# csiro-crop-informatics/biokanga

Hardware: AMD Instinct MI355X
Metric: aligned reads/s (SAM-identical) on 100 bp SE vs GRCh38, 1->8 MI355X (higher is better)
Workload: dtype u8

## Files before the change

### biokanga_amd/csrc/bk_ctx_int.h

```cpp
#pragma once
#include <atomic>
#include <thread>
#include <hip/hip_runtime.h>

#include <cstdio>
#include <string>
#include <vector>

#include "bk_device.h"
#include "bk_devbuf.h"

#define HIP_TRY(expr)                                                                              \
    do {                                                                                           \
        hipError_t e__ = (expr);                                                                   \
        if (e__ != hipSuccess) {                                                                   \
            fprintf(stderr, "biokanga_amd: %s failed: %s (%s:%d)\n", #expr, hipGetErrorString(e__), __FILE__, __LINE__); \
            return e__ == hipErrorOutOfMemory ? BK_ERR_MEM : BK_ERR_INTERNAL;                      \
        }                                                                                          \
    } while (0)

namespace bk {
struct BatchBufs {
    DevBuf<uint64_t> rd4, rd2, iv_first;
    DevBuf<uint2> iv2, iv32;
    DevBuf<uint32_t> iv_n, rmeta;
    DevBuf<uint32_t> act[2], heavy, wave, wave_work;
    DevBuf<uint32_t> stage[3], stripe_cnt;
    DevBuf<uint32_t> slist, slist_stage;
    DevBuf<uint32_t> sort[3];
    DevBuf<uint8_t> sort_tmp, scan_tmp;
    DevBuf<bk_seg2> seg2;
    DevBuf<uint8_t> in_bases;
    DevBuf<uint64_t> in_offs;
    DevBuf<uint32_t> in_lens;
    DevBuf<bk_hit> in_out;
    DevBuf<uint16_t> in_lens16;
    DevBuf<uint32_t> in_words;
    DevBuf<bk_nbase> in_exc;
    DevBuf<bk_snp_site> snp_sites;
    DevBuf<uint8_t> chrom_accept;
    DevBuf<unsigned long long> htab;
    DevBuf<uint32_t> slot_epoch;
};
struct ImageBufs {
    DevBuf<uint64_t> tgt4, tgt2, tgt2s;
    DevBuf<uint32_t> sa_lo, isa;
    DevBuf<uint8_t> sa_hi, nflag;
    DevBuf<uint64_t> ent_start, ent_end;
    DevBuf<uint32_t> ent_id, id2idx;
    DevBuf<uint8_t> ktab;
    DevBuf<uint64_t> ktab_hi;
    DevBuf<uint32_t> k2, kx[kMoreKeys];
    DevBuf<uint8_t> swin;
    DevBuf<uint32_t> swmap;
    DevBuf<uint32_t> grow_kx[kMoreKeys];
    DevBuf<uint8_t> grow_ktab2;
};
struct FixedBufs {
    DevBuf<uint32_t> small;
    DevBuf<PhaseCtl> ctl;
    DevBuf<unsigned long long> seq_counts, ctr, ctr_aux, snp_tot;
    DevBuf<unsigned long long> seq_global;
    DevBuf<uint32_t> snp_planes;
};
}

struct bk_ctx {
    int device = 0;
    hipStream_t stream = nullptr;
    bk_align_params params{};
    bk::DevAlignCfg cfg{};
    bk::DevIndex ix{};
    bk::ImageBufs image;
    bk::FixedBufs fixed;
    void release_image_buffers() { image = bk::ImageBufs{}; fixed = bk::FixedBufs{}; }
    uint64_t n_tgt4_words = 0;
    uint32_t cap_rd2w = 0;
    int use_tgt2 = 2;
    int sort_lists = 7;
    bool sort_lists_set = false;
    int sort_shift = 0;
    int use_k2 = 1;
    int use_k3 = bk::kMoreKeys;
    bool grow_enabled = false, grow_wait = false;
    uint64_t grow_after = 5 * BK_POLICY_MIN_READS, grow_seen = 0;
    std::atomic<int> grow_state{0};
    std::thread grow_thread;
    bk::DevIndex grow_ix{};
    bool grow_want_ktab2 = false;
    bool grow_elem = false, grow_want_elem = false;
    int use_ktab2 = 1;
    bool ktab_is2 = false;
    int use_iv32 = 1;
    uint32_t wave_waves = 256u * 8u * 4u;
    int use_isa = 1;
    int use_swin = 1;
    uint64_t swin_budget = 0;
    int swin_skip_short = 0;
    int swin_w = 0;
    uint64_t swin_bytes = 0;
    double swin_setup_s = 0;
    double swin_covered = 0;
    bool swin_denied = false;
    bool swin_rebuilt = false;
    int iv_poison = 0;
    int use_wave = 1;
    int lazy_search = 1;
    bool ktab64 = false;
    int ktab_wide = 0;
    int k_req = -1;
    int use_ktab = 1;
    uint32_t el_size = 4;
    uint64_t tot_seq_len = 0;
    std::string dataset;
    std::vector<bk_entry_info> entries;
    std::vector<bk_snp_site> snp_sites;

    bk::BatchBufs buf;
    void release_batch_buffers() { buf = bk::BatchBufs{}; }
    uint32_t cap_reads = 0, cap_wpr = 0, cap_iv_cores = 0;
    uint32_t *h_small = nullptr;
    bk::PhaseCtl *h_ctl = nullptr;
    hipEvent_t ev_ctl = nullptr;
    bool ctl_pending = false, hist_valid = false;
    uint32_t ctl_pending_reads = 0, ctl_pending_maxlen = 0;
    int ctl_pending_phases = 0;
    double hist_slist[bk::kMaxPhases] = {0}, hist_wave[bk::kMaxPhases] = {0};
    int async_error = 0;
    int async_phases = 1;
    bool force_rccl = false;
    uint64_t rccl_allreduces = 0;
    int rccl_ranks = 0;
    bk::HeavyScratch hs{};
    int max_read_len = 500;
    uint32_t last_maxlen = 0;
    int dbg_stop_phase = -1, dbg_phase = 0, dbg_cur = 0;
    uint32_t dbg_n = 0, dbg_ivc = 0;
    bool dbg_valid = false;
    bool debug = false;
    uint32_t chunk_reads = 64u << 20;

    hipEvent_t ev_wait = nullptr;
    bool entries_set = false, tgt2_built = false;
    bool tables_built = false;
    bool tables_under_way = false;
    void *sam_text[2] = {nullptr, nullptr};
    uint64_t sam_text_cap = 0;
    uint32_t n_chrom_accept = 0;
    bk_timing timing{};
    std::vector<hipEvent_t> ev_pool;
    std::vector<uint64_t> loci_offs;
    std::vector<bk_loci> loci;
    std::vector<bk_loci_trims> loci_trims;
    std::vector<bk_seg2> seg2;
};


namespace bk {
struct DevReads {
    const uint8_t *bases = nullptr;
    const uint64_t *offs = nullptr;
    const uint32_t *lens = nullptr;
    const uint32_t *words = nullptr;
    const bk_nbase *exc = nullptr;
    uint64_t n_exc = 0;
};
int engine_align_device(bk_ctx *c, const DevReads &in, uint32_t nreads, bk_hit *d_out, hipStream_t s, uint32_t maxlen_known = 0);
void release_swin(bk_ctx *c);
void drop_swin(bk_ctx *c);
int engine_pair_device(bk_ctx *c, const DevReads &in, uint32_t n_pairs, bk_hit *d_hits, uint32_t maxlen, const bk_pe_params *pe, hipStream_t s,
                       bk_seg2 *seg2_host = nullptr, bk_seg2 *seg2_dev = nullptr);
int engine_prepare_packed(bk_ctx *c, const uint16_t *d_lens16, uint32_t nreads, uint64_t n_words, const bk_nbase *d_exc, uint64_t n_exc,
                          uint32_t *d_lens32, uint64_t *d_offs, uint32_t *maxlen, hipStream_t s);
}

namespace bk {
hipError_t dev_malloc_bytes(void **p, size_t bytes);
hipError_t dev_zero_now(void *p, size_t bytes);
template <class T> inline hipError_t dev_malloc(T **p, size_t bytes) { return dev_malloc_bytes(reinterpret_cast<void **>(p), bytes); }
int upload_host(void *d_dst, const void *h_src, size_t bytes, int device);
int upload_file(void *d_dst, int fd, uint64_t file_ofs, size_t bytes, int device);
bool host_is_pinned(const void *p);
}
```

### biokanga_amd/csrc/bk_device.h

```cpp
#pragma once
#include <hip/hip_runtime.h>
#include <stdint.h>

#include "../../include/biokanga_amd.h"

namespace bk {

constexpr int kMoreKeys = 2;
constexpr int kK2Levels = 7;

__host__ __device__ __forceinline__ uint64_t k2s_pad(uint64_t words) { return (words + 15) & ~15ULL; }
__host__ __device__ __forceinline__ uint64_t k2s_count(uint64_t n, int j) { return (n + (1ULL << (4 * j)) - 1) >> (4 * j); }
__host__ __device__ __forceinline__ uint64_t k2s_start(uint64_t n, int j)
{
    uint64_t o = k2s_pad(n) + 16;
    for (int i = 1; i < j; i++) o += k2s_pad(k2s_count(n, i)) + 16;
    return o;
}


constexpr int kListStripes = 64;
struct StripeSet {
    uint32_t *cnt;
    uint32_t *stage[3];
    uint32_t cap;
};
constexpr int kCtrStripes = 64;
constexpr int kNwLong = 20;
constexpr int kNwLongest = 32;
constexpr int kPackedPadWords = 32;
constexpr int kMaxCoresFast = 16;
constexpr int kWave = 64;
constexpr int kMaxReadLenAbs = 2000;
constexpr uint32_t kNodeCap = 1024000;
constexpr uint64_t kEosWord = 0x7777777777777777ULL;
constexpr int kSwBases = 192, kSwPre = 92, kSwLen = 100;
template <int E> struct SwGeo { static constexpr int bases = 64 * E, pre = E == 3 ? 92 : 32 * E; };
template <int E> __host__ __device__ inline uint64_t sw_word_at(uint64_t idx, int q) { return (idx >> 5) * (32ULL * E) + (uint64_t)q * 32 + (idx & 31); }
constexpr int kSwBlkShift = 5;
constexpr uint32_t kSwNone = 0xFFFFFFFFu;
constexpr uint32_t kSwMinRun = 65, kSwHead = 192;
constexpr int kSwLevels = 8;
constexpr uint32_t kReadHasN = 1u << 15;
constexpr uint32_t kReadLenMask = kReadHasN - 1;

struct DevIndex {
    const uint64_t *tgt4;
    const uint64_t *tgt2;
    const uint64_t *tgt2s;
    const uint8_t *nflag;
    int flag_shift;
    uint32_t nflag_bytes;
    const uint32_t *sa_lo;
    const uint8_t *sa_hi;
    const uint64_t *ent_start;
    const uint64_t *ent_end;
    const uint32_t *ent_id;
    const uint32_t *id2idx;
    uint32_t max_id;
    const uint32_t *ktab32;
    const uint64_t *ktab64;
    const uint64_t *ktab_hi;
    const uint2 *ktab2;
    int ktab2_elem;
    const uint32_t *k2;
    const uint32_t *kx[kMoreKeys];
    const uint32_t *isa;
    const uint4 *swin;
    int sw_words;
    const uint32_t *swmap;
    uint64_t n;
    uint32_t n_ent;
    int k;
};

struct DevAlignCfg {
    int max_subs, mm_delta, align_strand, max_ns, max_hits;
    int min_core_len, slides_per100, max_iter;
    int heavy_thresh;
};

struct DevBatch {
    const uint8_t *bases;
    const uint64_t *offs;
    const uint32_t *lens;
    const uint32_t *pk_words;
    const bk_nbase *pk_exc;
    uint64_t pk_nexc;
    uint32_t pk_read0;
    uint64_t *rd4;
    uint64_t *rd2;
    uint32_t *rmeta;
    uint64_t *iv_first;
    uint32_t *iv_n;
    uint2 *iv2;
    uint32_t iv_stride;
    const uint32_t *act;
    uint32_t *wave_work;
    uint2 *iv32;
    bk_hit *out;
    unsigned long long *seq_counts;
    unsigned long long *ctr;
    uint32_t wpr;
    uint32_t n_reads;
    uint32_t nw;
    uint32_t iv_cores;
};

struct PhaseCtl {
    uint32_t n_act;
    uint32_t cmax;
    uint32_t n_slist;
    uint32_t n_wave;
    uint32_t n_heavy;
    uint32_t wave_cursor, heavy_cursor;
    uint32_t pad[9];
};
constexpr int kMaxPhases = 72;

struct HeavyScratch {
    unsigned long long *htab;
    uint32_t *slot_epoch;
    uint32_t tab_size;
    uint32_t n_slots;
};

struct ReadPlan {
    int len, max_tot_mm, core_len, core_delta, max_slides, n_loop, n_phases;
};

__host__ __device__ inline ReadPlan make_plan(int len, const DevAlignCfg &c)
{
    ReadPlan p;
    p.len = len;
    int m = c.max_subs == 0 ? 0 : (int)(0.5 + (double)(len * c.max_subs) / 100.0);
    if (c.max_subs != 0 && m < 1) m = 1;
    if (m > 63) m = 63;
    p.max_tot_mm = m;
    int cl = len / (c.mm_delta == 1 ? m + 1 : m + 2);
    p.core_len = cl > c.min_core_len ? cl : c.min_core_len;
    int ms = (c.slides_per100 * len + 99) / 100;
    p.max_slides = ms > 1 ? ms : 1;
    int cd = len / p.max_slides - 1;
    p.core_delta = cd > p.core_len ? cd : p.core_len;
    p.n_loop = 0;
    int has_final = 1;
    if (m > 0) {
        int a;
        for (a = 0; a <= m; a++) {
            if (len / (a + c.mm_delta) <= p.core_len) break;
            p.n_loop++;
        }
        has_final = a <= m;
    }
    p.n_phases = p.n_loop + has_final;
    return p;
}

__host__ __device__ inline void phase_params(const ReadPlan &p, const DevAlignCfg &c, int phase, int &mm, int &cl, int &cd)
{
    if (phase < p.n_loop) {
        mm = phase;
        cl = p.len / (phase + c.mm_delta);
        cd = cl;
    } else {
        mm = p.max_tot_mm;
        cl = p.core_len;
        cd = p.core_delta;
    }
}

__host__ __device__ inline int core_offsets(int plen, int cl, int cd, int max_slides, int *ofs, int maxn)
{
    int cur = cd, o = 0, n = 0;
    while (n < max_slides && o <= plen - cl && cur > cl / 3) {
        if (o + cl + cur > plen) cur = plen - (o + cl);
        n++;
        o += cur;
    }
    const int last = plen - cl;
    for (int i = 0; i < maxn; i++) {
        int v = i * cd;
        ofs[i] = v < last ? v : last;
    }
    return n;
}

}
```

### biokanga_amd/csrc/bk_engine.cpp

```cpp
#include "bk_engine_int.h"

namespace bk {
int size_heavy_scratch(bk_ctx *c)
{
    int slides = std::max(1, (c->cfg.slides_per100 * c->max_read_len + 99) / 100);
    uint64_t worst = c->cfg.max_iter ? (uint64_t)slides * (uint64_t)c->cfg.max_iter : kNodeCap;
    if (worst > kNodeCap) worst = kNodeCap;
    uint32_t ts = 1024;
    while (ts < 2 * worst) ts <<= 1;
    uint32_t slots = 4096;
    while ((uint64_t)slots * ts * 8 > (16ULL << 30) && slots > 64) slots >>= 1;
    if (c->hs.htab && c->hs.tab_size == ts && c->hs.n_slots == slots) return BK_OK;
    BatchBufs &m = c->buf;
    m.htab.reset();
    m.slot_epoch.reset();
    c->hs = HeavyScratch{};
    HIP_TRY(m.htab.ensure((size_t)slots * ts));
    HIP_TRY(m.slot_epoch.ensure(slots));
    launch_fill_u64(m.htab.get(), (uint64_t)slots * ts, 0ULL, c->stream);
    HIP_TRY(hipGetLastError());
    HIP_TRY(hipMemsetAsync(m.slot_epoch.get(), 0, (size_t)slots * 4, c->stream));
    HIP_TRY(hipStreamSynchronize(c->stream));
    c->hs = HeavyScratch{m.htab.get(), m.slot_epoch.get(), ts, slots};
    return BK_OK;
}


int ensure_batch_scratch(bk_ctx *c, uint32_t n_reads, uint32_t wpr, uint32_t rd2w, uint32_t iv_cores)
{
    if (n_reads <= c->cap_reads && wpr <= c->cap_wpr && rd2w <= c->cap_rd2w && iv_cores <= c->cap_iv_cores) return BK_OK;
    const size_t nr = std::max(n_reads, c->cap_reads), w = std::max(wpr, c->cap_wpr), w2 = std::max(rd2w, c->cap_rd2w);
    const size_t ivc = std::max(iv_cores, c->cap_iv_cores);
    BatchBufs &m = c->buf;
    m.rd4.reset(); m.iv_first.reset(); m.iv_n.reset(); m.rd2.reset(); m.iv2.reset(); m.rmeta.reset();
    m.act[0].reset(); m.act[1].reset(); m.heavy.reset(); m.wave.reset(); m.iv32.reset(); m.wave_work.reset();
    for (auto &st : m.stage) st.reset();
    c->cap_reads = 0;
    HIP_TRY(m.rd4.ensure(nr * 2 * w));
    if (w2) HIP_TRY(m.rd2.ensure(nr * 2 * w2 + 8));
    HIP_TRY(m.rmeta.ensure((nr + 2) / 2 * 2));
    if (c->image.sa_hi.get() == nullptr && c->ix.n < (1ULL << 32))
        HIP_TRY(m.iv2.ensure(nr * 2 * ivc));
    else {
        HIP_TRY(m.iv_first.ensure(nr * 2 * ivc));
        HIP_TRY(m.iv_n.ensure(nr * 2 * ivc));
    }
    HIP_TRY(m.act[0].ensure(nr));
    HIP_TRY(m.act[1].ensure(nr));
    HIP_TRY(m.heavy.ensure(nr));
    HIP_TRY(m.wave.ensure(nr));
    for (auto &st : m.stage) HIP_TRY(st.ensure(nr + (kListStripes + 2) * 1024));
    if (!m.stripe_cnt.get()) {
        HIP_TRY(m.stripe_cnt.ensure((size_t)2 * kListStripes * 16));
        HIP_TRY(dev_zero_now(m.stripe_cnt.get(), (size_t)2 * kListStripes * 16 * 4));
    }
    if (m.iv2.get()) HIP_TRY(m.iv32.ensure(nr * 2));
    HIP_TRY(m.wave_work.ensure(nr));
    c->cap_reads = (uint32_t)nr;
    c->cap_wpr = (uint32_t)w;
    c->cap_rd2w = (uint32_t)w2;
    c->cap_iv_cores = (uint32_t)ivc;
    return BK_OK;
}

int ensure_slist(bk_ctx *c, uint64_t lanes, hipStream_t s)
{
    BatchBufs &m = c->buf;
    if (m.slist_stage.get() && lanes <= m.slist.cap()) return BK_OK;
    HIP_TRY(hipStreamSynchronize(s));
    m.slist.reset();
    m.slist_stage.reset();
    HIP_TRY(m.slist.ensure(lanes));
    HIP_TRY(m.slist_stage.ensure(lanes + (kListStripes + 2) * 1024));
    return BK_OK;
}

int ensure_in_reads(bk_ctx *c, uint32_t n, bool packed)
{
    BatchBufs &m = c->buf;
    if (n > m.in_out.cap()) {
        m.in_offs.reset(); m.in_lens.reset(); m.in_out.reset(); m.in_lens16.reset();
        HIP_TRY(m.in_offs.ensure(n));
        HIP_TRY(m.in_lens.ensure(n));
        HIP_TRY(m.in_out.ensure(n));
    }
    if (packed) HIP_TRY(m.in_lens16.ensure(m.in_out.cap()));
    return BK_OK;
}

HostExtent host_extent(const uint64_t *offs, const uint32_t *lens, uint32_t nreads)
{
    HostExtent x;
    for (uint32_t i = 0; i < nreads; i++) {
        x.lo = std::min(x.lo, offs[i]);
        x.hi = std::max(x.hi, offs[i] + lens[i]);
        x.maxlen = std::max(x.maxlen, lens[i]);
    }
    x.rel.resize(nreads);
    for (uint32_t i = 0; i < nreads; i++) x.rel[i] = offs[i] - x.lo;
    return x;
}

static int stage_host_batch(bk_ctx *c, const uint8_t *bases, const uint64_t *offs, const uint32_t *lens, uint32_t nreads, HostExtent &x, DevReads &in)
{
    x = host_extent(offs, lens, nreads);
    if (x.maxlen > (uint32_t)kMaxReadLenAbs) return BK_ERR_PARAMS;
    const uint64_t nbytes = x.hi - x.lo;
    BatchBufs &m = c->buf;
    HIP_TRY(m.in_bases.ensure(nbytes + 16));
    int rc = ensure_in_reads(c, nreads, false);
    if (rc) return rc;
    HIP_TRY(hipMemcpyAsync(m.in_bases.get(), bases + x.lo, nbytes, hipMemcpyHostToDevice, c->stream));
    HIP_TRY(hipMemcpyAsync(m.in_offs.get(), x.rel.data(), (size_t)nreads * 8, hipMemcpyHostToDevice, c->stream));
    HIP_TRY(hipMemcpyAsync(m.in_lens.get(), lens, (size_t)nreads * 4, hipMemcpyHostToDevice, c->stream));
    in.bases = m.in_bases.get(); in.offs = m.in_offs.get(); in.lens = m.in_lens.get();
    return BK_OK;
}

static DevBatch make_batch(bk_ctx *c, const DevReads &in, uint32_t first, uint32_t n, uint32_t wpr, uint32_t iv_cores, bk_hit *d_out)
{
    const BatchBufs &m = c->buf;
    DevBatch b{};
    b.bases = in.bases; b.offs = in.offs + first; b.lens = in.lens + first;
    b.pk_words = in.words; b.pk_exc = in.exc; b.pk_nexc = in.words ? in.n_exc : 0; b.pk_read0 = first;
    b.rd4 = m.rd4.get(); b.iv_first = m.iv_first.get(); b.iv_n = m.iv_n.get(); b.iv2 = m.iv2.get();
    b.rmeta = m.rmeta.get();
    b.out = d_out; b.seq_counts = c->fixed.seq_counts.get(); b.ctr = c->fixed.ctr.get();
    b.wpr = wpr; b.n_reads = n; b.iv_cores = iv_cores;
    return b;
}

enum class Span { Search, Extend, Heavy, Other, SearchA, SearchSort, SearchB, Prep };

struct EvTimer {
    bk_ctx *c;
    bool on = true;
    std::vector<std::pair<Span, std::pair<hipEvent_t, hipEvent_t>>> spans;
    size_t next_ev = 0;
    hipEvent_t get()
    {
        if (!on) return nullptr;
        if (next_ev == c->ev_pool.size()) {
            hipEvent_t e;
            (void)hipEventCreate(&e);
            c->ev_pool.push_back(e);
        }
        return c->ev_pool[next_ev++];
    }
    hipEvent_t begin(hipStream_t s)
    {
        hipEvent_t e = get();
        if (e) (void)hipEventRecord(e, s);
        return e;
    }
    void end(Span kind, hipEvent_t b, hipStream_t s)
    {
        hipEvent_t e = get();
        if (!e) return;
        (void)hipEventRecord(e, s);
        spans.push_back({kind, {b, e}});
    }
};

int ensure_sort_scratch(bk_ctx *c, uint32_t n, hipStream_t s)
{
    BatchBufs &m = c->buf;
    if (m.sort_tmp.get() && n <= m.sort[2].cap()) return BK_OK;
    HIP_TRY(hipStreamSynchronize(s));
    for (auto &p : m.sort) p.reset();
    m.sort_tmp.reset();
    const uint64_t cap = (uint64_t)n + n / 4;
    for (auto &p : m.sort) HIP_TRY(p.ensure(cap));
    size_t tb = 0;
    if (sort_list_by_key(nullptr, nullptr, nullptr, nullptr, (uint32_t)cap, nullptr, &tb, s)) return BK_ERR_INTERNAL;
    HIP_TRY(m.sort_tmp.ensure(tb));
    return BK_OK;
}

int sort_work(bk_ctx *c, const uint32_t *list, uint32_t n, hipStream_t s, const uint32_t **out)
{
    const BatchBufs &m = c->buf;
    size_t tb = m.sort_tmp.cap();
    if (sort_list_by_key(m.sort[0].get(), m.sort[1].get(), list, m.sort[2].get(), n, m.sort_tmp.get(), &tb, s)) return BK_ERR_INTERNAL;
    *out = m.sort[2].get();
    return BK_OK;
}

struct LociChunk {
    bk_ctx *c;
    uint32_t n;
    hipStream_t s;
    DevBuf<unsigned long long> cnt, offs;
    DevBuf<uint8_t> tmp;
    DevBuf<bk_loci> loci;
    DevBuf<bk_loci_trims> trims;
    size_t base = 0;
    uint64_t loci_base = 0, total = 0;
    int begin()
    {
        HIP_TRY(cnt.ensure((size_t)n + 1));
        HIP_TRY(offs.ensure((size_t)n + 1));
        HIP_TRY(hipMemsetAsync(cnt.get(), 0, ((size_t)n + 1) * 8, s));
        return BK_OK;
    }
    int scan()
    {
        size_t tb = 0;
        if (scan_counts_u64(nullptr, nullptr, n + 1, nullptr, &tb, s)) return BK_ERR_INTERNAL;
        HIP_TRY(tmp.ensure(tb ? tb : 16));
        if (scan_counts_u64(cnt.get(), offs.get(), n + 1, tmp.get(), &tb, s)) return BK_ERR_INTERNAL;
        base = c->loci_offs.empty() ? 0 : c->loci_offs.size() - 1;
        loci_base = c->loci.size();
        if (c->loci_offs.empty()) c->loci_offs.push_back(0);
        c->loci_offs.resize(base + n + 1);
        HIP_TRY(hipMemcpyAsync(c->loci_offs.data() + base, offs.get(), ((size_t)n + 1) * 8, hipMemcpyDeviceToHost, s));
        HIP_TRY(hipStreamSynchronize(s));
        total = c->loci_offs[base + n];
        HIP_TRY(loci.ensure((size_t)total));
        return BK_OK;
    }
    int finish()
    {
        if (total) {
            c->loci.resize(loci_base + total);
            HIP_TRY(hipMemcpyAsync(c->loci.data() + loci_base, loci.get(), (size_t)total * sizeof(bk_loci), hipMemcpyDeviceToHost, s));
            if (trims.get()) {
                c->loci_trims.resize(loci_base + total);
                HIP_TRY(hipMemcpyAsync(c->loci_trims.data() + loci_base, trims.get(), (size_t)total * sizeof(bk_loci_trims), hipMemcpyDeviceToHost, s));
            }
            HIP_TRY(hipStreamSynchronize(s));
        }
        if (loci_base)
            for (size_t i = 0; i <= n; i++) c->loci_offs[base + i] += loci_base;
        return BK_OK;
    }
};

int collect_loci(bk_ctx *c, const DevBatch &b, uint32_t n, uint32_t maxlen, hipStream_t s)
{
    bk_seg2 *d_seg2 = c->params.min_chimeric_len > 0 ? c->buf.seg2.get() : nullptr;
    LociChunk lc{c, n, s};
    int rc = lc.begin();
    if (rc) return rc;
    launch_loci_count(b.out, n, c->params.clamp_ml ? c->cfg.max_hits : 0, lc.cnt.get(), s);
    rc = lc.scan();
    if (rc) return rc;
    uint32_t n_multi = 0;
    if (lc.total) {
        uint32_t *sm = c->fixed.small.get();
        if (d_seg2) {
            HIP_TRY(lc.trims.ensure((size_t)lc.total));
            HIP_TRY(clear_dev(lc.trims.get(), (size_t)lc.total * sizeof(bk_loci_trims), s));
        }
        HIP_TRY(hipMemsetAsync(sm, 0, 16 * 4, s));
        uint32_t *list = c->buf.act[0].get();
        launch_loci_single(b.out, n, lc.offs.get(), lc.loci.get(), list, sm + 0, d_seg2, lc.trims.get(), s);
        HIP_TRY(hipMemcpyAsync(c->h_small, sm, 16 * 4, hipMemcpyDeviceToHost, s));
        HIP_TRY(hipStreamSynchronize(s));
        n_multi = c->h_small[0];
        if (n_multi) {
            rc = size_heavy_scratch(c);
            if (rc) return rc;
            launch_loci_enum(c->ix, c->cfg, b, c->hs, list, n_multi, sm + 1, lc.offs.get(), lc.loci.get(), sm + 2, d_seg2 ? c->params.min_chimeric_len : 0,
                             maxlen > 512 ? 1 : 0, d_seg2, lc.trims.get(), s);
            HIP_TRY(hipGetLastError());
            HIP_TRY(hipMemcpyAsync(c->h_small, sm, 16 * 4, hipMemcpyDeviceToHost, s));
        }
    }
    rc = lc.finish();
    if (rc) return rc;
    if (n_multi && c->h_small[2] != 0) {
        fprintf(stderr, "bk: loci replay disagreed with LowHitInstances for %u reads\n", c->h_small[2]);
        return BK_ERR_INTERNAL;
    }
    return BK_OK;
}

int best_matches_chunk(bk_ctx *c, const DevBatch &b, uint32_t n, const uint32_t *d_list, uint32_t n_list, hipStream_t s)
{
    const uint32_t width = (uint32_t)c->cfg.max_hits;
    DevBuf<bk_loci> dense;
    LociChunk lc{c, n, s};
    int rc = lc.begin();
    if (rc) return rc;
    HIP_TRY(dense.ensure((size_t)n * width));
    rc = size_heavy_scratch(c);
    if (rc) return rc;
    uint32_t *sm = c->fixed.small.get();
    HIP_TRY(hipMemsetAsync(sm + 4, 0, 4, s));
    launch_best(c->ix, c->cfg, b, c->hs, d_list, n_list, sm + 4, lc.cnt.get(), dense.get(), s);
    HIP_TRY(hipGetLastError());
    rc = lc.scan();
    if (rc) return rc;
    if (lc.total) {
        launch_loci_compact(dense.get(), width, lc.offs.get(), n, lc.loci.get(), s);
        HIP_TRY(hipGetLastError());
    }
    return lc.finish();
}

int align_chunk(bk_ctx *c, const DevReads &in, uint32_t first, uint32_t n, uint32_t maxlen, bk_hit *d_out, hipStream_t s, EvTimer &tm)
{
    uint32_t *sm = c->fixed.small.get(), *hm = c->h_small;
    HIP_TRY(hipMemsetAsync(sm, 0, 16 * 4, s));
    const uint32_t wpr = words_per_read(maxlen);
    const bool reg_path = c->use_wave && maxlen <= 16u * (uint32_t)kNwLongest;
    const int nw16 = maxlen <= 128 ? 8 : (maxlen <= 256 ? 16 : (maxlen <= 16u * (uint32_t)kNwLong ? kNwLong : kNwLongest));
    const bool two_bit = reg_path && c->ix.tgt2 != nullptr;
    const uint32_t ivc = iv_cores_for(c, maxlen);
    int rc = ensure_batch_scratch(c, n, wpr, two_bit ? (uint32_t)(nw16 / 2) : 0u, ivc);
    if (rc && c->image.swin.get()) {
        (void)hipGetLastError();
        bk::release_swin(c);
        rc = ensure_batch_scratch(c, n, wpr, two_bit ? (uint32_t)(nw16 / 2) : 0u, ivc);
    }
    if (rc) return rc;

    BatchBufs &m = c->buf;
    uint32_t *const d_act[2] = {m.act[0].get(), m.act[1].get()}, *const d_heavy = m.heavy.get(), *const d_wave = m.wave.get();
    uint32_t *const d_stage[3] = {m.stage[0].get(), m.stage[1].get(), m.stage[2].get()}, *const d_stripe_cnt = m.stripe_cnt.get();
    DevBatch b = make_batch(c, in, first, n, wpr, ivc, d_out);
    b.rd2 = two_bit ? m.rd2.get() : nullptr;
    b.wave_work = (reg_path && c->cfg.heavy_thresh <= 100) ? m.wave_work.get() : nullptr;
    b.iv32 = (c->use_iv32 && c->ix.k2) ? m.iv32.get() : nullptr;
    b.nw = reg_path ? (uint32_t)nw16 : 0u;
    const int nstr = c->cfg.align_strand == 0 ? 2 : 1;

    PhaseCtl *ctl = c->fixed.ctl.get();
    HIP_TRY(hipMemsetAsync(ctl, 0, sizeof(PhaseCtl) * (kMaxPhases + 2), s));
    auto P = [&](int ph) { return reinterpret_cast<uint32_t *>(ctl + ph); };
    int max_phases = 0, cmax_bound[kMaxPhases + 1] = {0};
    bool cores_fit = true;
    for (uint32_t len = 1; len <= maxlen; len++) {
        const ReadPlan p = make_plan((int)len, c->cfg);
        max_phases = std::max(max_phases, p.n_phases);
        for (int ph = 0; ph < p.n_phases && ph <= kMaxPhases; ph++) {
            int mm, cl, cd, dummy[1];
            phase_params(p, c->cfg, ph, mm, cl, cd);
            const int nc = core_offsets((int)len, cl, cd, p.max_slides, dummy, 0);
            if (nc > kMaxCoresFast) cores_fit = false;
            cmax_bound[ph] = std::max(cmax_bound[ph], std::min(nc, (int)kMaxCoresFast));
        }
    }
    if (max_phases > kMaxPhases) return BK_ERR_INTERNAL;
    const bool no_readback = reg_path && c->cfg.heavy_thresh <= 100 && c->ix.k2 != nullptr && cores_fit && !c->params.best_matches &&
                             !c->debug && c->async_phases;
    const bool check_maxlen = !tm.on;
    if (check_maxlen) launch_max_len(b.lens, n, P(kMaxPhases + 1) + 0, s);
    hipEvent_t e0 = tm.begin(s);
    launch_prep(c->cfg, b, d_act[0], P(0) + 0, P(0) + 1, d_stage[0], d_stripe_cnt, s);
    HIP_TRY(hipGetLastError());
    tm.end(Span::Prep, e0, s);
    uint32_t n_act = n;
    int cmax = cmax_bound[0];
    auto read_ctl = [&](int ph) -> int {
        HIP_TRY(hipMemcpyAsync(hm, ctl + ph, 2 * sizeof(PhaseCtl), hipMemcpyDeviceToHost, s));
        HIP_TRY(hipStreamSynchronize(s));
        return BK_OK;
    };
    if (!no_readback) {
        int rr = read_ctl(0);
        if (rr) return rr;
        n_act = hm[0];
        cmax = (int)hm[1];
    }
    int cur = 0;
    if (c->params.best_matches) {
        hipEvent_t eb = tm.begin(s);
        int rb = best_matches_chunk(c, b, n, d_act[0], n_act, s);
        if (rb) return rb;
        tm.end(Span::Heavy, eb, s);
        n_act = 0;
    }
    b.iv_stride = n;
    if (no_readback && c->ix.isa == nullptr) { int rh = size_heavy_scratch(c); if (rh) return rh; }
    for (int phase = 0; no_readback ? phase < max_phases : n_act > 0; phase++) {
        const uint32_t *ext_list = d_act[cur];
        b.act = ext_list;
        if (no_readback) cmax = cmax_bound[phase];
        const uint32_t n_bound = n_act;
        uint32_t *ctl_p = P(phase), *ctl_n = P(phase + 1);
        const int lazy = (reg_path && c->lazy_search) ? 1 : 0;
        if (cmax > 0) {
            hipEvent_t e1 = tm.begin(s);
            if (c->ix.k2) {
                const uint64_t lanes = (uint64_t)n_bound * (uint64_t)(cmax * nstr);
                { int rs = ensure_slist(c, lanes, s); if (rs) return rs; }
                uint32_t *const d_slist = m.slist.get();
                if (c->iv_poison) launch_clear_iv(b, ctl_p + 0, n_bound, cmax, c->cfg.align_strand == 2 ? 1 : 0, c->cfg.align_strand == 1 ? 0 : 1, 0xFFFFFFFFu, s);
                hipEvent_t ea = tm.begin(s);
                launch_search_a(c->ix, c->cfg, b, d_act[cur], ctl_p + 0, n_bound, phase, cmax, nstr, lazy, d_slist, ctl_p + 2,
                                m.slist_stage.get(), d_stripe_cnt, s);
                HIP_TRY(hipGetLastError());
                tm.end(Span::SearchA, ea, s);
                uint64_t n_slist_bound = lanes;
                uint32_t n_sort = 0;
                if (!no_readback) {
                    HIP_TRY(hipMemcpyAsync(hm + 2, ctl_p + 2, 4, hipMemcpyDeviceToHost, s));
                    HIP_TRY(hipStreamSynchronize(s));
                    n_slist_bound = hm[2];
                    n_sort = hm[2];
                } else {
                    const double f = c->hist_valid ? c->hist_slist[phase] * 1.05 : 0.30;
                    n_sort = (uint32_t)std::min<uint64_t>({(uint64_t)(f * n) + 4096, lanes, (uint64_t)0x7FFFFFF0});
                }
                if (no_readback && m.sort[2].cap() >= 4096) n_sort = (uint32_t)std::min<uint64_t>(n_sort, m.sort[2].cap());
                const uint32_t *sorted = nullptr;
                if ((c->sort_lists & 1) && n_sort >= 4096) {
                    int rs = ensure_sort_scratch(c, n_sort, s);
                    if (rs) return rs;
                    hipEvent_t es = tm.begin(s);
                    launch_keys_search(b, d_slist, ctl_p + 2, n_sort, c->sort_shift, m.sort[0].get(), s);
                    rs = sort_work(c, d_slist, n_sort, s, &sorted);
                    if (rs) return rs;
                    tm.end(Span::SearchSort, es, s);
                } else
                    n_sort = 0;
                if (n_slist_bound) {
                    hipEvent_t eb = tm.begin(s);
                    launch_search_b(c->ix, c->cfg, b, phase, lazy, d_slist, sorted, n_sort, ctl_p + 2, n_slist_bound, s);
                    tm.end(Span::SearchB, eb, s);
                }
            } else
                launch_search(c->ix, c->cfg, b, d_act[cur], n_act, phase, cmax, nstr, lazy, s);
            HIP_TRY(hipGetLastError());
            tm.end(Span::Search, e1, s);
        }
        if (phase == c->dbg_stop_phase) {
            c->dbg_n = n; c->dbg_ivc = ivc; c->dbg_cur = cur; c->dbg_phase = phase; c->dbg_valid = true;
            break;
        }
        hipEvent_t e2 = tm.begin(s);
        DevAlignCfg cfg_lane = c->cfg;
        if (c->ix.n > (1ULL << 32)) cfg_lane.heavy_thresh = 0;
        if (n_bound == 0) {}
        else if (reg_path && c->cfg.heavy_thresh <= 100)
            launch_flat(c->ix, c->cfg, b, ext_list, ctl_p + 0, n_bound, phase, nstr * std::max(cmax, 1), d_act[cur ^ 1], ctl_n + 0, d_heavy, ctl_p + 4,
                        d_wave, ctl_p + 3, ctl_n + 1, d_stage, d_stripe_cnt, nw16, s);
        else
            launch_extend(c->ix, cfg_lane, b, ext_list, n_act, phase, d_act[cur ^ 1], ctl_n + 0, d_heavy, ctl_p + 4, ctl_n + 1, s);
        HIP_TRY(hipGetLastError());
        tm.end(Span::Extend, e2, s);
        uint32_t n_heavy = 0, n_wave = n_bound;
        if (!no_readback) {
            int rr = read_ctl(phase);
            if (rr) return rr;
            n_heavy = hm[4];
            n_wave = hm[3];
        }
        if (n_wave) {
            hipEvent_t e3 = tm.begin(s);
            const uint32_t *wsorted = nullptr;
            uint32_t n_sort = n_wave;
            if (no_readback) {
                const double f = c->hist_valid ? c->hist_wave[phase] * 1.05 : 0.25;
                n_sort = (uint32_t)std::min<uint64_t>((uint64_t)(f * n) + 4096, n_wave);
                if (m.sort[2].cap() >= 4096) n_sort = (uint32_t)std::min<uint64_t>(n_sort, m.sort[2].cap());
            }
            if ((c->sort_lists & 2) && n_sort >= 4096) {
                int rs = ensure_sort_scratch(c, n_sort, s);
                if (rs) return rs;
                launch_keys_wave(c->cfg, b, phase, d_wave, ctl_p + 3, n_sort, (c->sort_lists & 4) ? -1 : c->sort_shift, m.sort[0].get(), b.wave_work, s);
                rs = sort_work(c, d_wave, n_sort, s, &wsorted);
                if (rs) return rs;
            } else
                n_sort = 0;
            if (!no_readback && c->ix.isa == nullptr) { int rh = size_heavy_scratch(c); if (rh) return rh; }
            launch_wave(c->ix, c->cfg, b, c->hs, d_wave, wsorted, n_sort, ctl_p + 3, n_wave, phase, ctl_p + 5, d_act[cur ^ 1], ctl_n + 0, ctl_n + 1,
                        nw16, c->wave_waves, s);
            HIP_TRY(hipGetLastError());
            tm.end(Span::Heavy, e3, s);
        }
        if (n_heavy) {
            hipEvent_t e3 = tm.begin(s);
            { int rh = size_heavy_scratch(c); if (rh) return rh; }
            launch_heavy(c->ix, c->cfg, b, c->hs, d_heavy, n_heavy, phase, ctl_p + 6, d_act[cur ^ 1], ctl_n + 0, ctl_n + 1, s);
            HIP_TRY(hipGetLastError());
            tm.end(Span::Heavy, e3, s);
        }
        if (!no_readback) {
            if (n_wave || n_heavy) { int rr = read_ctl(phase); if (rr) return rr; }
            if (c->debug)
                fprintf(stderr, "bk: phase %d n_act %u cmax %d n_heavy %u n_wave %u -> next n_act %u cmax %u\n", phase, n_act, cmax, n_heavy, n_wave, hm[16], hm[17]);
            n_act = hm[16];
            cmax = (int)hm[17];
        }
        cur ^= 1;
        if (phase > 70) return BK_ERR_INTERNAL;
    }
    if (c->dbg_stop_phase >= 0 && !c->dbg_valid) {
        c->dbg_n = n; c->dbg_ivc = ivc; c->dbg_cur = cur; c->dbg_phase = kMaxPhases; c->dbg_valid = true;
    }
    if (no_readback) {
        HIP_TRY(hipMemcpyAsync(c->h_ctl, ctl, sizeof(PhaseCtl) * (kMaxPhases + 2), hipMemcpyDeviceToHost, s));
        HIP_TRY(hipEventRecord(c->ev_ctl, s));
        c->ctl_pending = true;
        c->ctl_pending_reads = n;
        c->ctl_pending_phases = max_phases;
        c->ctl_pending_maxlen = check_maxlen ? maxlen : 0;
    }
    if (c->params.micro_indel_len > 0 || c->params.splice_junct_len > 0 || c->params.min_chimeric_len > 0) {
        hipEvent_t ei = tm.begin(s);
        { int r2 = ensure_seg2(c, n); if (r2) return r2; }
        bk_seg2 *d_seg2 = m.seg2.get();
        hipError_t eh = clear_dev(d_seg2, (size_t)n * sizeof(bk_seg2), s);
        int rc2 = BK_OK;
        if (eh == hipSuccess && (c->params.micro_indel_len > 0 || c->params.splice_junct_len > 0)) {
            eh = hipMemsetAsync(sm, 0, 16 * 4, s);
            if (eh == hipSuccess) {
                launch_indel(c->ix, c->cfg, b, n, c->params.micro_indel_len, c->params.splice_junct_len, c->params.min_chimeric_len > 0 ? 1 : 0, d_act[0], sm + 0,
                             hm + 0, sm + 1, d_seg2, s);
                eh = hipGetLastError();
            }
        }
        if (eh == hipSuccess && c->params.min_chimeric_len > 0) {
            rc2 = size_heavy_scratch(c);
            if (rc2 == BK_OK) {
                eh = hipMemsetAsync(sm, 0, 16 * 4, s);
                if (eh == hipSuccess) {
                    launch_unaligned_list(b.out, n, d_act[0], sm + 0, s);
                    eh = hipMemcpyAsync(hm, sm, 4, hipMemcpyDeviceToHost, s);
                }
                if (eh == hipSuccess) eh = hipStreamSynchronize(s);
                if (eh == hipSuccess && hm[0]) {
                    launch_chimeric(c->ix, c->cfg, b, c->hs, d_act[0], hm[0], c->params.min_chimeric_len, maxlen > 512 ? 1 : 0, sm + 1, d_seg2, s);
                    eh = hipGetLastError();
                }
            }
        }
        const size_t at = c->seg2.size();
        c->seg2.resize(at + n);
        if (eh == hipSuccess && rc2 == BK_OK) eh = hipMemcpyAsync(c->seg2.data() + at, d_seg2, (size_t)n * sizeof(bk_seg2), hipMemcpyDeviceToHost, s);
        if (eh == hipSuccess) eh = hipStreamSynchronize(s);
        if (rc2 != BK_OK) return rc2;
        if (eh != hipSuccess) return BK_ERR_INTERNAL;
        if (c->params.min_chimeric_len > 0 && c->cfg.max_hits > 1)
            for (size_t i = at; i < at + n; i++)
                if (c->seg2[i].flags == 0x40) c->seg2[i] = bk_seg2{};
        tm.end(Span::Heavy, ei, s);
    }
    hipEvent_t e4 = tm.begin(s);
    launch_count_seqs(d_out, n, c->image.id2idx.get(), c->ix.n_ent, c->fixed.seq_counts.get(), s);
    HIP_TRY(hipGetLastError());
    tm.end(Span::Other, e4, s);
    if (c->cfg.max_hits > 1 && !c->params.best_matches) {
        int rl = collect_loci(c, b, n, maxlen, s);
        if (rl) return rl;
    }
    return BK_OK;
}


int take_phase_history(bk_ctx *c, bool wait)
{
    if (!c->ctl_pending) return BK_OK;
    if (wait) HIP_TRY(bk::wait_event(c->ev_ctl));
    else if (hipEventQuery(c->ev_ctl) != hipSuccess) { (void)hipGetLastError(); return BK_OK; }
    c->ctl_pending = false;
    const PhaseCtl *h = c->h_ctl;
    const double n = (double)std::max<uint32_t>(c->ctl_pending_reads, 1);
    for (int ph = 0; ph < kMaxPhases; ph++) {
        c->hist_slist[ph] = ph < c->ctl_pending_phases ? (double)h[ph].n_slist / n : 0.0;
        c->hist_wave[ph] = ph < c->ctl_pending_phases ? (double)h[ph].n_wave / n : 0.0;
        if (h[ph].n_heavy) {
            fprintf(stderr, "biokanga_amd: %u reads of phase %d were left for the general kernel by a schedule that does not run it\n", h[ph].n_heavy, ph);
            c->async_error = BK_ERR_INTERNAL;
        }
    }
    if (c->ctl_pending_maxlen && h[kMaxPhases + 1].n_act > c->ctl_pending_maxlen) {
        fprintf(stderr, "biokanga_amd: a batch held a read of %u bases, its caller had promised at most %u\n", h[kMaxPhases + 1].n_act, c->ctl_pending_maxlen);
        c->async_error = BK_ERR_PARAMS;
    }
    c->hist_valid = true;
    if (c->async_error && wait) { const int e = c->async_error; c->async_error = 0; return e; }
    return BK_OK;
}

int align_device(bk_ctx *c, const DevReads &in, uint32_t nreads, bk_hit *d_out, hipStream_t s, uint32_t maxlen_known, bool enqueue_only)
{
    grow_tick(c, nreads);
    const uint32_t *d_lens = in.lens;
    if (enqueue_only) {
        const uint32_t ml = maxlen_known;
        const bool plain = c->cfg.max_hits == 1 && !c->params.best_matches && !c->params.micro_indel_len && !c->params.splice_junct_len && !c->params.min_chimeric_len;
        const bool fits = ml >= 1 && ml <= 16u * (uint32_t)kNwLongest && nreads <= c->cap_reads && nreads <= c->chunk_reads && words_per_read(ml) <= c->cap_wpr &&
                          iv_cores_for(c, ml) <= c->cap_iv_cores && rd2w_for(ml) <= c->cap_rd2w &&
                          (uint64_t)nreads * iv_cores_for(c, ml) * (c->cfg.align_strand == 0 ? 2u : 1u) <= c->buf.slist.cap() && (c->ix.isa != nullptr || c->hs.htab != nullptr);
        const bool main_path = c->use_wave && c->cfg.heavy_thresh <= 100 && c->ix.k2 != nullptr && c->ix.tgt2 != nullptr && !c->debug && c->async_phases;
        if (!plain || !fits || !main_path) return BK_ERR_PARAMS;
    }
    EvTimer tm{c};
    tm.on = !enqueue_only;
    hipEvent_t t0 = tm.begin(s);
    c->loci_offs.clear();
    c->loci.clear();
    c->loci_trims.clear();
    c->seg2.clear();
    uint32_t maxlen = maxlen_known;
    if (!maxlen) {
        HIP_TRY(hipMemsetAsync(c->fixed.small.get(), 0, 16 * 4, s));
        launch_max_len(d_lens, nreads, c->fixed.small.get() + 5, s);
        HIP_TRY(hipMemcpyAsync(c->h_small, c->fixed.small.get(), 16 * 4, hipMemcpyDeviceToHost, s));
        HIP_TRY(hipStreamSynchronize(s));
        maxlen = c->h_small[5];
    }
    if (maxlen > (uint32_t)kMaxReadLenAbs) return BK_ERR_PARAMS;
    c->last_maxlen = maxlen;
    (void)take_phase_history(c, false);
    if ((int)maxlen > c->max_read_len) {
        c->max_read_len = (int)maxlen;
    }
    if (!enqueue_only) { int rw = maybe_build_swin(c, maxlen, nreads, s); if (rw) return rw; }
    uint32_t chunk = c->chunk_reads;
    if (!(std::min(chunk, nreads) <= c->cap_reads && words_per_read(maxlen) <= c->cap_wpr && iv_cores_for(c, maxlen) <= c->cap_iv_cores &&
          rd2w_for(maxlen) <= std::max(c->cap_rd2w, 1u) && !c->params.best_matches)) {
        const uint64_t per_read = scratch_bytes_per_read(words_per_read(maxlen), rd2w_for(maxlen), iv_cores_for(c, maxlen));
        size_t free_b = 0, total_b = 0;
        HIP_TRY(hipMemGetInfo(&free_b, &total_b));
        const uint64_t have = (uint64_t)c->cap_reads * scratch_bytes_per_read(c->cap_wpr, c->cap_rd2w, c->cap_iv_cores);
        uint64_t fit = ((uint64_t)free_b + have) / 4 * 3 / per_read;
        if (fit < 65536) fit = 65536;
        if (fit < chunk) chunk = (uint32_t)fit;
        if (chunk > (1u << 27)) chunk = 1u << 27;
        if (c->params.best_matches) {
            const uint64_t lim = std::max<uint64_t>(1024, (4ULL << 30) / (sizeof(bk_loci) * (uint64_t)c->cfg.max_hits));
            if (lim < chunk) chunk = (uint32_t)lim;
        }
    }
    for (uint32_t done = 0; done < nreads;) {
        uint32_t n = std::min(chunk, nreads - done);
        int rc = align_chunk(c, in, done, n, maxlen, d_out + done, s, tm);
        if (rc) return rc;
        done += n;
    }
    if (enqueue_only) return BK_OK;
    hipEvent_t t1 = tm.begin(s);
    HIP_TRY(bk::wait_stream(s, c->ev_wait));
    { int rh = take_phase_history(c, true); if (rh) return rh; }
    float ms = 0;
    (void)hipEventElapsedTime(&ms, t0, t1);
    c->timing.ms_total += ms;
    for (auto &sp : tm.spans) {
        float m = 0;
        (void)hipEventElapsedTime(&m, sp.second.first, sp.second.second);
        switch (sp.first) {
        case Span::Search: c->timing.ms_search += m; c->timing.n_search_launches++; break;
        case Span::Extend: c->timing.ms_extend += m; c->timing.n_extend_launches++; break;
        case Span::Heavy: c->timing.ms_heavy += m; c->timing.n_heavy_launches++; break;
        case Span::SearchA: c->timing.ms_search_a += m; break;
        case Span::SearchSort: c->timing.ms_search_sort += m; break;
        case Span::SearchB: c->timing.ms_search_b += m; c->timing.n_search_b_launches++; break;
        case Span::Prep: c->timing.ms_prep += m; c->timing.ms_other += m; break;
        case Span::Other: c->timing.ms_other += m; break;
        }
    }
    return BK_OK;
}


}

using namespace bk;

int bk::engine_align_device(bk_ctx *c, const DevReads &in, uint32_t nreads, bk_hit *d_out, hipStream_t s, uint32_t maxlen_known)
{
    return align_device(c, in, nreads, d_out, s, maxlen_known);
}

namespace {
struct CastU64 {
    __host__ __device__ unsigned long long operator()(const uint32_t &v) const { return (unsigned long long)v; }
};
}

int bk::engine_prepare_packed(bk_ctx *c, const uint16_t *d_lens16, uint32_t nreads, uint64_t n_words, const bk_nbase *d_exc, uint64_t n_exc,
                              uint32_t *d_lens32, uint64_t *d_offs, uint32_t *maxlen, hipStream_t s)
{
    launch_widen_lens(d_lens16, nreads, d_lens32, (unsigned long long *)d_offs, s);
    HIP_TRY(hipGetLastError());
    size_t need = 0;
    HIP_TRY(bk::prim::exclusive_sum(nullptr, need, (unsigned long long *)d_offs, (unsigned long long *)d_offs, (size_t)nreads, s));
    if (need > c->buf.scan_tmp.cap()) {
        HIP_TRY(hipStreamSynchronize(s));
        HIP_TRY(c->buf.scan_tmp.ensure(need + 256));
    }
    size_t tb = c->buf.scan_tmp.cap();
    HIP_TRY(bk::prim::exclusive_sum(c->buf.scan_tmp.get(), tb, (unsigned long long *)d_offs, (unsigned long long *)d_offs, (size_t)nreads, s));
    HIP_TRY(hipMemsetAsync(c->fixed.ctr_aux.get(), 0, 32, s));
    launch_packed_extent(d_offs, d_lens32, nreads, c->fixed.ctr_aux.get(), s);
    launch_check_exc(d_exc, n_exc, d_lens32, nreads, reinterpret_cast<uint32_t *>(c->fixed.ctr_aux.get() + 2), s);
    HIP_TRY(hipGetLastError());
    unsigned long long h[3] = {0, 0, 0};
    HIP_TRY(hipMemcpyAsync(h, c->fixed.ctr_aux.get(), 24, hipMemcpyDeviceToHost, s));
    HIP_TRY(hipStreamSynchronize(s));
    if (h[0] != n_words || h[1] > (unsigned long long)kMaxReadLenAbs || (uint32_t)h[2] != 0) return BK_ERR_PARAMS;
    *maxlen = (uint32_t)h[1];
    return BK_OK;
}

int bk::engine_pair_device(bk_ctx *c, const DevReads &in, uint32_t n_pairs, bk_hit *d_hits, uint32_t maxlen, const bk_pe_params *pe, hipStream_t s,
                           bk_seg2 *seg2_host, bk_seg2 *seg2_dev)
{
    const uint32_t nreads = 2 * n_pairs;
    const uint32_t wpr = words_per_read(maxlen);
    const uint32_t ivc = c->cap_iv_cores ? c->cap_iv_cores : iv_cores_for(c, maxlen);
    int rc = ensure_batch_scratch(c, nreads, wpr, 0, ivc);
    if (rc && c->image.swin.get()) {
        (void)hipGetLastError();
        bk::release_swin(c);
        rc = ensure_batch_scratch(c, nreads, wpr, 0, ivc);
    }
    if (rc) return rc;
    const DevBatch b = make_batch(c, in, 0, nreads, wpr, c->cap_iv_cores, d_hits);
    if (c->params.min_chimeric_len > 0 && !seg2_host && !seg2_dev) return BK_ERR_PARAMS;
    bk_seg2 *d_seg2 = seg2_dev;
    if (!d_seg2 && seg2_host) {
        rc = ensure_seg2(c, nreads);
        if (rc) return rc;
        d_seg2 = c->buf.seg2.get();
        HIP_TRY(hipMemcpyAsync(d_seg2, seg2_host, (size_t)nreads * sizeof(bk_seg2), hipMemcpyHostToDevice, s));
    }
    HIP_TRY(hipMemsetAsync(c->fixed.small.get(), 0, 16 * 4, s));
    launch_pe(c->ix, c->cfg, b, pe->pe_mode, pe->pair_min_len, pe->pair_max_len, pe->pair_strand ? 1 : 0, d_hits, n_pairs,
              c->buf.heavy.get(), c->fixed.small.get(), c->h_small, d_seg2, c->params.min_chimeric_len, maxlen > 512 ? 1 : 0, c->buf.chrom_accept.get(), c->n_chrom_accept, s);
    HIP_TRY(hipGetLastError());
    if (seg2_host && !seg2_dev) HIP_TRY(hipMemcpyAsync(seg2_host, d_seg2, (size_t)nreads * sizeof(bk_seg2), hipMemcpyDeviceToHost, s));
    HIP_TRY(hipStreamSynchronize(s));
    return BK_OK;
}


extern "C" {


int bk_batch_seg2(bk_ctx *c, const bk_seg2 **seg2, uint64_t *n)
{
    if (!c || !seg2 || !n) return BK_ERR_PARAMS;
    *seg2 = c->seg2.empty() ? nullptr : c->seg2.data();
    *n = c->seg2.size();
    return BK_OK;
// ... 355 lines not shown
```

### biokanga_amd/csrc/bk_engine_int.h

```cpp
#pragma once
#include <hip/hip_runtime.h>
#include <fcntl.h>
#include <unistd.h>
#include "bk_prim.h"

#include <algorithm>
#include <cstdio>
#include <cstdlib>
#include <ctime>
#include <cstring>
#include <map>
#include <mutex>
#include <string>
#include <atomic>
#include <thread>
#include <type_traits>
#include <vector>

#include <dlfcn.h>
#include <rccl/rccl.h>

#include "bk_ctx_int.h"
#include "bk_cpus.h"
#include "bk_wait.h"
#include "bk_env.h"
#include "sfx_file.h"


namespace bk {
void launch_pack_target(const uint8_t *seq, uint64_t n, uint64_t *tgt4, uint64_t nwords, hipStream_t s);
void launch_pack_target2(const uint64_t *tgt4, uint64_t nwords4, uint64_t *tgt2, unsigned int *nflag32, int flag_shift, hipStream_t s);
void launch_split_sa5(const uint8_t *sa5, uint64_t n, uint32_t *lo, uint8_t *hi, hipStream_t s);
void launch_build_ktab(const DevIndex &ix, void *tab, int k, bool tab64, hipStream_t s, uint64_t i0 = 0, uint64_t i1 = 0, unsigned long long *starts = nullptr, bool pairs = false);
void launch_fill_ktab2_y(void *tab2, const uint32_t *k2, uint64_t n_entries, hipStream_t s, const uint32_t *sa_elem = nullptr);
void launch_max_len(const uint32_t *lens, uint32_t n, uint32_t *out, hipStream_t s);
void launch_widen_lens(const uint16_t *lens16, uint32_t n, uint32_t *lens32, unsigned long long *nwords, hipStream_t s);
void launch_check_exc(const bk_nbase *exc, uint64_t n_exc, const uint32_t *lens, uint32_t n_reads, uint32_t *bad, hipStream_t s);
void launch_packed_extent(const uint64_t *offs, const uint32_t *lens, uint32_t n, unsigned long long *out, hipStream_t s);
void launch_snp_pileup(const DevIndex &ix, const uint8_t *bases, const uint64_t *offs, const uint32_t *id2idx, const bk_snp_aln *alns, uint64_t n_alns,
                       uint32_t *planes, hipStream_t s);
void launch_snp_gather(const DevIndex &ix, const uint32_t *planes, uint64_t g0, uint32_t n, uint32_t *out, hipStream_t s);
void launch_snp_centroids(const DevIndex &ix, const uint32_t *planes, uint64_t g0, uint32_t chrom_len, uint32_t min_reads, uint32_t *hist, hipStream_t s);
void launch_snp_sites(const DevIndex &ix, const uint32_t *planes, uint64_t g0, uint32_t chrom_len, uint32_t min_reads, double min_prop,
                      bk_snp_site *sites, uint32_t cap, uint32_t *n_sites, unsigned long long *totals, hipStream_t s);
void launch_count_seqs(const bk_hit *out, uint32_t n, const uint32_t *id2idx, uint32_t n_ent, unsigned long long *counts, hipStream_t s);
void launch_fill_u64(unsigned long long *p, uint64_t n, unsigned long long v, hipStream_t s);
void launch_prep(const DevAlignCfg &cfg, const DevBatch &b, uint32_t *act, uint32_t *act_cnt, uint32_t *cmax, uint32_t *stage,
                 uint32_t *stripe_cnt, hipStream_t s);
void launch_search(const DevIndex &ix, const DevAlignCfg &cfg, const DevBatch &b, const uint32_t *act, uint32_t n_act,
                   int phase, int cmax, int nstr, int lazy, hipStream_t s);
void launch_extend(const DevIndex &ix, const DevAlignCfg &cfg, const DevBatch &b, const uint32_t *act, uint32_t n_act,
                   int phase, uint32_t *next_act, uint32_t *next_cnt, uint32_t *heavy, uint32_t *heavy_cnt,
                   uint32_t *cmax_next, hipStream_t s);
void launch_build_isa(const uint32_t *sa, uint64_t n, uint32_t *isa, hipStream_t s, uint64_t i0 = 0, uint64_t i1 = 0);
void launch_build_swin(const DevIndex &ix, void *swin, int words, hipStream_t s);
void launch_swin_breaks(const DevIndex &ix, const int *w, int n_levels, unsigned long long *const *brk, uint64_t a, uint64_t e, uint64_t n_words,
                        const unsigned long long *starts, hipStream_t s);
void launch_swin_cover(const unsigned long long *brk, uint64_t n, uint32_t max_run, uint32_t min_run, uint32_t *flags, uint64_t n_blocks, int first_level, hipStream_t s);
void launch_pack_ktab64(const uint64_t *tab, uint64_t n_entries, uint32_t *off, uint64_t *hi, uint32_t *overflow, hipStream_t s);
void launch_count_nonzero(const uint32_t *flags, uint64_t n, unsigned long long *count, hipStream_t s);
void launch_swin_map(const uint32_t *flags, const uint32_t *incl, uint64_t n_blocks, uint32_t cap_blocks, uint32_t *used, uint32_t *map, hipStream_t s);
void launch_swin_fill(const DevIndex &ix, const uint32_t *map, void *swin, int words, uint64_t a, uint64_t e, hipStream_t s);
void launch_build_k2(const DevIndex &ix, uint32_t *k2, uint32_t *k3, uint32_t *k4, unsigned long long *bad, hipStream_t s, uint64_t i0 = 0, uint64_t i1 = 0, bool write_k2 = true);
void launch_build_k2_levels(uint32_t *k2, uint64_t n, hipStream_t s);
void launch_make_ktab2(const uint32_t *tab, const uint32_t *k2, uint64_t n_entries, uint64_t n, void *out, hipStream_t s, const uint32_t *sa_elem = nullptr);
void launch_search_a(const DevIndex &ix, const DevAlignCfg &cfg, const DevBatch &b, const uint32_t *act, const uint32_t *p_n_act, uint32_t n_act_bound,
                     int phase, int cmax, int nstr, int lazy, uint32_t *list, uint32_t *list_cnt, uint32_t *stage, uint32_t *stripe_cnt,
                     hipStream_t s);
void launch_search_b(const DevIndex &ix, const DevAlignCfg &cfg, const DevBatch &b, int phase, int lazy, const uint32_t *list, const uint32_t *sorted,
                     uint32_t n_sorted, const uint32_t *p_n_list, uint64_t n_bound, hipStream_t s);
void launch_clear_iv(const DevBatch &b, const uint32_t *p_n_act, uint32_t n_act_bound, int cmax, int st0, int st1, uint32_t word, hipStream_t s);
void launch_pe(const DevIndex &ix, const DevAlignCfg &cfg, const DevBatch &b, int pe_mode, int min_len, int max_len, int pair_strand,
               bk_hit *hits, uint32_t n_pairs, uint32_t *orphans, uint32_t *counters, uint32_t *h_count, bk_seg2 *seg2, int min_chim,
               int long_reads, const uint8_t *accept, uint32_t n_accept, hipStream_t s);
void launch_flat(const DevIndex &ix, const DevAlignCfg &cfg, const DevBatch &b, const uint32_t *act, const uint32_t *p_n_act, uint32_t n_act_bound, int phase,
                 int slots_max, uint32_t *next_act, uint32_t *next_cnt, uint32_t *heavy, uint32_t *heavy_cnt, uint32_t *wave,
                 uint32_t *wave_cnt, uint32_t *cmax_next, uint32_t *const *stage, uint32_t *stripe_cnt, int nw, hipStream_t s);
void launch_wave(const DevIndex &ix, const DevAlignCfg &cfg, const DevBatch &b, const HeavyScratch &hs, const uint32_t *list, const uint32_t *sorted,
                 uint32_t n_sorted, const uint32_t *p_n_list, uint32_t n_bound, int phase, uint32_t *cursor, uint32_t *next_act, uint32_t *next_cnt,
                 uint32_t *cmax_next, int nw, uint32_t max_waves, hipStream_t s);
void launch_heavy(const DevIndex &ix, const DevAlignCfg &cfg, const DevBatch &b, const HeavyScratch &hs, const uint32_t *list,
                  uint32_t n_list, int phase, uint32_t *cursor, uint32_t *next_act, uint32_t *next_cnt, uint32_t *cmax_next,
                  hipStream_t s);
int build_sa_device(const uint8_t *d_seq, uint64_t n, void *d_sa_out, int el_size, hipStream_t s);
int scan_counts_u64(const unsigned long long *in, unsigned long long *out, uint32_t n, void *tmp, size_t *tmp_bytes, hipStream_t s);
void launch_loci_count(const bk_hit *out, uint32_t n, int clamp_to, unsigned long long *cnt, hipStream_t s);
void launch_best(const DevIndex &ix, const DevAlignCfg &cfg, const DevBatch &b, const HeavyScratch &hs, const uint32_t *list,
                 uint32_t n_list, uint32_t *cursor, unsigned long long *cnt, bk_loci *dense, hipStream_t s);
void launch_indel(const DevIndex &ix, const DevAlignCfg &cfg, const DevBatch &b, uint32_t n, int max_indel, int max_junct, int keep_state, uint32_t *list,
                  uint32_t *list_cnt_dev, uint32_t *list_cnt_host, uint32_t *cursor, bk_seg2 *seg2, hipStream_t s);
void launch_unaligned_list(const bk_hit *out, uint32_t n, uint32_t *list, uint32_t *cnt, hipStream_t s);
void launch_chimeric(const DevIndex &ix, const DevAlignCfg &cfg, const DevBatch &b, const HeavyScratch &hs, const uint32_t *list, uint32_t n_list,
                     int min_pct, int long_reads, uint32_t *cursor, bk_seg2 *seg2, hipStream_t s);
void launch_loci_compact(const bk_loci *dense, uint32_t width, const unsigned long long *offs, uint32_t n, bk_loci *out, hipStream_t s);
void launch_loci_single(const bk_hit *out, uint32_t n, const unsigned long long *offs, bk_loci *loci, uint32_t *list, uint32_t *list_cnt,
                        const bk_seg2 *seg2, bk_loci_trims *trims, hipStream_t s);
void launch_loci_enum(const DevIndex &ix, const DevAlignCfg &cfg, const DevBatch &b, const HeavyScratch &hs, const uint32_t *list,
                      uint32_t n_list, uint32_t *cursor, const unsigned long long *offs, bk_loci *loci, uint32_t *err, int min_pct, int long_reads,
                      bk_seg2 *seg2, bk_loci_trims *trims, hipStream_t s);
int sort_list_by_key(const uint32_t *keys_in, uint32_t *keys_out, const uint32_t *vals_in, uint32_t *vals_out, uint32_t n,
                     void *tmp, size_t *tmp_bytes, hipStream_t s);
void launch_keys_search(const DevBatch &b, const uint32_t *list, const uint32_t *p_n, uint32_t n_sort, int shift, uint32_t *keys, hipStream_t s);
void launch_keys_wave(const DevAlignCfg &cfg, const DevBatch &b, int phase, const uint32_t *list, const uint32_t *p_n, uint32_t n_sort, int shift, uint32_t *keys,
                      const uint32_t *work_of, hipStream_t s);

struct StageClock {
    bool on = env::timing();
    double t0 = now();
    static double now() { timespec ts; clock_gettime(CLOCK_MONOTONIC, &ts); return (double)ts.tv_sec + 1e-9 * (double)ts.tv_nsec; }
    static double wall() { timespec ts; clock_gettime(CLOCK_REALTIME, &ts); return (double)(ts.tv_sec % 60) + 1e-9 * (double)ts.tv_nsec; }
    void lap(const char *what) { if (!on) return; const double t = now(); fprintf(stderr, "bk timing: %-28s %7.1f ms   (done at :%06.3f)\n", what, 1e3 * (t - t0), wall()); t0 = t; }
};


inline uint32_t words_per_read(uint32_t maxlen)
{
    return ((maxlen + 15) / 16 + 2) & ~1u;
}

inline uint32_t iv_cores_for(const bk_ctx *c, uint32_t maxlen)
{
    const uint32_t ms = std::max(1u, ((uint32_t)c->cfg.slides_per100 * maxlen + 99) / 100);
    return std::min<uint32_t>(ms, kMaxCoresFast);
}

inline uint32_t rd2w_for(uint32_t maxlen)
{
    return maxlen <= 128 ? 4u : (maxlen <= 256 ? 8u : (maxlen <= 16u * (uint32_t)kNwLong ? (uint32_t)kNwLong / 2 : (uint32_t)kNwLongest / 2));
}

inline uint64_t scratch_bytes_per_read(uint32_t wpr, uint32_t rd2w = 8, uint32_t iv_cores = kMaxCoresFast)
{
    return 2ULL * wpr * 8 + 2ULL * rd2w * 8 + 2ULL * iv_cores * (12 + 8) + 52 + 24;
}


int derive_cfg(bk_ctx *c);
hipError_t clear_dev(void *p, size_t bytes, hipStream_t s);
struct TablePlan {
    bool ktab = false, k2 = false, isa = false;
    bool ktab2 = false;
    int kx = 0;
    int k = 0;
    DevBuf<unsigned long long> d_bad;
};

int tables_begin(bk_ctx *c, TablePlan &tp);
int tables_range(bk_ctx *c, const TablePlan &tp, uint64_t i0, uint64_t i1, unsigned long long *bucket_starts = nullptr);
int tables_end(bk_ctx *c, TablePlan &tp);
int build_tables(bk_ctx *c);
int build_tgt2(bk_ctx *c);
void publish_index(bk_ctx *c);
void grow_take_in(bk_ctx *c);
void grow_drop(bk_ctx *c);
void grow_tick(bk_ctx *c, uint64_t nreads, bool now = false);
int setup_entries(bk_ctx *c, const bk_entry_info *entries, uint32_t n_entries);
int finish_ctx(bk_ctx *c, const bk_entry_info *entries, uint32_t n_entries);
int new_ctx(bk_ctx **out, int device_id, const bk_align_params *p, bk_ctx **pc);
int adopt_device_image(bk_ctx *c, const uint8_t *d_seq, uint64_t n, const uint8_t *d_sa, int el);
int maybe_build_swin(bk_ctx *c, uint32_t maxlen, uint32_t nreads, hipStream_t s);
int size_heavy_scratch(bk_ctx *c);
int ensure_batch_scratch(bk_ctx *c, uint32_t n_reads, uint32_t wpr, uint32_t rd2w = 0, uint32_t iv_cores = kMaxCoresFast);
int ensure_sort_scratch(bk_ctx *c, uint32_t n, hipStream_t s);
int ensure_slist(bk_ctx *c, uint64_t lanes, hipStream_t s);
inline int ensure_seg2(bk_ctx *c, uint32_t n) { HIP_TRY(c->buf.seg2.ensure(n)); return BK_OK; }
struct HostExtent {
    uint64_t lo = ~0ULL, hi = 0;
    uint32_t maxlen = 0;
    std::vector<uint64_t> rel;
};
HostExtent host_extent(const uint64_t *offs, const uint32_t *lens, uint32_t nreads);
int align_device(bk_ctx *c, const DevReads &in, uint32_t nreads, bk_hit *d_out, hipStream_t s, uint32_t maxlen_known = 0, bool enqueue_only = false);
}
```

### biokanga_amd/csrc/bk_extend.hip

```cpp
#include "bk_dev_window.h"
#include "bk_dev_prof.h"

namespace bk {


template <bool WIDE>
__global__ void __launch_bounds__(256) k_extend(DevIndex ix, DevAlignCfg cfg, DevBatch b, const uint32_t *__restrict__ act,
                                                uint32_t n_act, int phase, uint32_t *__restrict__ next_act,
                                                uint32_t *__restrict__ next_cnt, uint32_t *__restrict__ heavy,
                                                uint32_t *__restrict__ heavy_cnt, uint32_t *__restrict__ cmax_next)
{
    __shared__ LdsEntries s_le;
    lds_entries_load(s_le, ix);
    uint32_t a = blockIdx.x * blockDim.x + threadIdx.x;
    unsigned long long n_search = 0, n_cand = 0, n_lcm = 0;
    if (a < n_act) {
        uint32_t r = act[a];
        int len = (int)b.lens[r];
        ReadPlan p = make_plan(len, cfg);
        int mm, cl, cd, ofs[kMaxCoresFast];
        phase_params(p, cfg, phase, mm, cl, cd);
        int nc = core_offsets(len, cl, cd, p.max_slides, ofs, kMaxCoresFast);
        int s0 = cfg.align_strand == 2 ? 1 : 0, s1 = cfg.align_strand == 1 ? 0 : 1;
        bool is_heavy = nc > kMaxCoresFast;
        if (!is_heavy)
            for (int st = s0; st <= s1; st++)
                for (int c = 0; c < nc; c++)
                    if (iv_count(b, iv_slot(b, a, st, c)) > (uint32_t)cfg.heavy_thresh) is_heavy = true;
        if (is_heavy) {
            heavy[atomicAdd(heavy_cnt, 1u)] = r;
        } else {
            n_lcm = 1;
            const int init = mm + cfg.mm_delta + 1;
            int low_inst = 0, low_mm = init, nxt = init;
            uint64_t hit_left = 0;
            int hit_ent = -1, hit_strand = '?';
            bool done = false;
            for (int st = s0; st <= s1 && !done; st++) {
                const uint64_t *rdw = b.rd4 + ((uint64_t)r * 2 + st) * b.wpr;
                for (int c = 0; c < nc && !done; c++) {
                    n_search++;
                    uint64_t slot = iv_slot(b, a, st, c);
                    uint32_t n;
                    uint64_t first;
                    iv_get(b, slot, first, n);
                    for (uint32_t j = 0; j < n; j++) {
                        uint64_t loci = sa_get<WIDE>(ix, first + j);
                        if (loci < (uint64_t)ofs[c]) continue;
                        uint64_t t = loci - (uint64_t)ofs[c];
                        int e = find_entry_lds(s_le, ix, t);
                        if (e < 0 || t + (uint64_t)len - 1 > ix.ent_end[e]) continue;
                        bool dup = false;
                        for (int c2 = 0; c2 < c && !dup; c2++) {
                            uint64_t q0 = nib16(rdw, ofs[c2]) & top_mask(cl);
                            dup = cmp_core(rdw, ofs[c2], cl, q0, ix.tgt4, t + (uint64_t)ofs[c2]) == 0;
                        }
                        if (dup) continue;
                        n_cand++;
                        int lim = mm < nxt - 1 ? mm : nxt - 1;
                        int cm = hamming(rdw, len, ix.tgt4, t, lim);
                        if (cm > lim) continue;
                        if (cm < low_mm) {
                            low_inst = 1; nxt = low_mm; low_mm = cm;
                            hit_left = t; hit_ent = e; hit_strand = st ? '-' : '+';
                        } else if (cm == low_mm)
                            low_inst++;
                        else
                            nxt = cm;
                        if (low_inst > cfg.max_hits && low_mm == 0) { done = true; break; }
                    }
                }
            }
            int rslt = classify(low_inst, low_mm, nxt, init, cfg.mm_delta, cfg.max_hits);
            if (rslt != BK_HR_NONE)
                write_result(ix, cfg, b, r, len, rslt, low_inst, low_mm, nxt, hit_left, hit_ent, hit_strand, phase << 1);
            else if (phase + 1 < p.n_phases) {
                int mm2, cl2, cd2, dummy[1];
                phase_params(p, cfg, phase + 1, mm2, cl2, cd2);
                int nc2 = core_offsets(len, cl2, cd2, p.max_slides, dummy, 0);
                if (nc2 <= kMaxCoresFast) atomicMax(cmax_next, (uint32_t)nc2);
                next_act[atomicAdd(next_cnt, 1u)] = r;
            }
        }
    }
    for (int off = 32; off > 0; off >>= 1) {
        n_search += __shfl_down(n_search, off);
        n_cand += __shfl_down(n_cand, off);
        n_lcm += __shfl_down(n_lcm, off);
    }
    if ((threadIdx.x & 63) == 0) {
        if (n_search) atomicAdd(&b.ctr[ctr_stripe() + 0], n_search);
        if (n_cand) atomicAdd(&b.ctr[ctr_stripe() + 1], n_cand);
        if (n_lcm) atomicAdd(&b.ctr[ctr_stripe() + 2], n_lcm);
    }
}


constexpr uint32_t kLdsEntries = 128;
constexpr uint32_t kFlatCap = 8192;
constexpr uint8_t kRecSkip = 255;

template <bool WIDE> struct FlatEntT { typedef uint64_t type; };
template <> struct FlatEntT<false> { typedef uint32_t type; };
__host__ __device__ constexpr bool flat_caches_first(bool wide, int bs, int slots_max)
{
    return !wide && slots_max <= 16 && bs * slots_max * 6 <= 24576;
}

__host__ __device__ constexpr bool flat_rows_in_lds(bool wide, int nw, int bs) { return false; }
__host__ __device__ constexpr bool flat_small_pass(bool wide, int nw, int bs) { return !wide && nw <= 8 && bs <= 256; }

template <bool WIDE, int NW, int BS>
__global__ void __launch_bounds__(BS) k_flat(DevIndex ix, DevAlignCfg cfg, DevBatch b, const uint32_t *__restrict__ act,
                                              const uint32_t *__restrict__ p_n_act, int phase, int slots_max, StripeSet out, int have_wave)
{
    const uint32_t n_act = *p_n_act;
    if ((uint64_t)blockIdx.x * BS >= n_act) return;
    constexpr bool ROWS = flat_rows_in_lds(WIDE, NW, BS);
#ifdef BK_FLAT_KB
    constexpr int KB = BK_FLAT_KB;
#else
    constexpr int KB = 1;
#endif
    constexpr int NBLK = NW / 4 + 1;
    constexpr bool SMALL = flat_small_pass(WIDE, NW, BS);
    constexpr uint32_t CAP = (SMALL ? kFlatCap / 4 : kFlatCap) * BS / 256;
    constexpr int SPEC = 8;
    extern __shared__ uint32_t s_dyn[];
    const bool cf = flat_caches_first(WIDE, BS, slots_max);
    uint32_t *s_first = s_dyn;
    uint16_t *s_sp = reinterpret_cast<uint16_t *>(s_dyn + (cf ? BS * slots_max : 0));
    __shared__ uint32_t s_lazy[BS];
    __shared__ uint32_t s_off[BS + 1];
    __shared__ uint32_t s_r[BS];
    __shared__ uint32_t s_geo[BS];
    __shared__ uint8_t s_hasn[BS];
    __shared__ uint32_t s_k1[BS], s_c2[BS], s_nx[BS];
    __shared__ uint8_t s_mm[BS];
    __shared__ alignas(16) uint8_t s_rec[CAP];
    __shared__ uint4 s_row[ROWS ? BS * 2 * (NW / 4) : 1];
    __shared__ alignas(16) uint32_t s_key[WIDE ? CAP : 1];
    __shared__ uint32_t s_t[SMALL ? CAP : 1];
    __shared__ uint32_t s_wsum[BS / 64];
    __shared__ uint32_t s_cnt[4], s_base[4], s_cmax;
    __shared__ unsigned long long s_ctr[3];
    using EntT = typename FlatEntT<WIDE>::type;
    __shared__ EntT s_es[kLdsEntries], s_ee[kLdsEntries];
    const uint32_t t = threadIdx.x;
#if defined(BK_PROF) && BK_PROF == 1
    PROF_BEGIN;
#endif
    const int lane = t & 63, wid = t >> 6;
    if (t < 4) s_cnt[t] = 0;
    if (t == 4) s_cmax = 0;
    if (t >= 8 && t < 11) s_ctr[t - 8] = 0;
    const bool ent_lds = ix.n_ent <= kLdsEntries;
    uint64_t es_v = 0, ee_v = 0;
    if (ent_lds && t < ix.n_ent) { es_v = ix.ent_start[t]; ee_v = ix.ent_end[t]; }

    const uint32_t a = blockIdx.x * blockDim.x + t;
    const int s0 = cfg.align_strand == 2 ? 1 : 0, s1 = cfg.align_strand == 1 ? 0 : 1;
    const int cmaxs = slots_max / (s1 - s0 + 1);
    const bool two_bit = b.rd2 != nullptr;
    uint32_t n_search = 0, n_cand = 0, n_lcm = 0;
    int dest = 0;
    uint32_t r = 0, my_cmax = 0, my_total = 0;
    int len = 0, mm = 0, cl = 1, cd = 1, nc = 0, n_phases = 0;
    bool mine = false;
    if (a < n_act) {
        r = act[a];
        const uint32_t len_v = b.rmeta[r];
        const bool spec = !WIDE && slots_max <= SPEC;
        uint2 sv[SPEC];
        if (!WIDE) {
#pragma unroll
            for (int u = 0; u < SPEC; u++) {
                sv[u] = make_uint2(0, 0);
                if (spec && u < slots_max) {
                    const int sti = u >= cmaxs ? 1 : 0;
                    sv[u] = b.iv2[iv_slot(b, a, s0 + sti, u - sti * cmaxs)];
                }
            }
        }
        uint4 rb00 = make_uint4(0, 0, 0, 0), rb01 = rb00, rb10 = rb00, rb11 = rb00;
        if (ROWS && two_bit) {
            const uint4 *__restrict__ rp = reinterpret_cast<const uint4 *>(b.rd2 + (uint64_t)r * 2 * (NW / 2));
            rb00 = rp[0]; rb01 = rp[1]; rb10 = rp[2]; rb11 = rp[3];
        }
        len = (int)(len_v & kReadLenMask);
        ReadPlan p = make_plan(len, cfg);
        n_phases = p.n_phases;
        int dummy[1];
        phase_params(p, cfg, phase, mm, cl, cd);
        nc = core_offsets(len, cl, cd, p.max_slides, dummy, 0);
        const bool fits = nc <= kMaxCoresFast && len <= 16 * NW && nc <= cmaxs;
        bool is_heavy = !fits;
        if (fits) {
            uint32_t run = 0, lazy_bits = 0, work = 0;
            if (!WIDE && spec) {
#pragma unroll
                for (int u = 0; u < SPEC; u++)
                    if (u < slots_max) {
                        const int c = u >= cmaxs ? u - cmaxs : u;
                        const uint32_t raw = c < nc ? sv[u].y : 0u;
                        if (raw & kLazyFlag) lazy_bits |= 1u << u;
                        if (raw & kElemFlag) lazy_bits |= 0x10000u << u;
                        const uint32_t cnt = raw & ~kIvFlags;
                        if (cnt > (uint32_t)cfg.heavy_thresh) is_heavy = true;
                        run += is_heavy ? 0 : cnt;
                        work = work + cnt < work ? 0xFFFFFFFFu : work + cnt;
                        if (cf) s_first[t * slots_max + u] = sv[u].x;
                        s_sp[t * slots_max + u] = (uint16_t)run;
                    }
            } else
                for (int q = 0; q < slots_max; q++) {
                    const int sti = q >= cmaxs ? 1 : 0, c = q - sti * cmaxs;
                    uint64_t f64 = 0;
                    uint32_t cnt = 0;
                    if (c < nc) iv_get(b, iv_slot(b, a, s0 + sti, c), f64, cnt);
                    if (cnt & kLazyFlag) lazy_bits |= 1u << (q & 31);
                    if ((cnt & kElemFlag) && cf) lazy_bits |= 0x10000u << q;
                    cnt &= ~kIvFlags;
                    if (cnt > (uint32_t)cfg.heavy_thresh) is_heavy = true;
                    run += is_heavy ? 0 : cnt;
                    work = work + cnt < work ? 0xFFFFFFFFu : work + cnt;
                    if (cf) s_first[t * slots_max + q] = (uint32_t)f64;
                    s_sp[t * slots_max + q] = (uint16_t)run;
                }
            s_lazy[t] = lazy_bits;
            if (run > CAP) is_heavy = true;
            my_total = is_heavy ? 0 : run;
            if (is_heavy && have_wave && b.wave_work != nullptr) b.wave_work[a] = work;
        }
        if (is_heavy) dest = (fits && have_wave) ? 2 : 3;
        else { mine = true; n_lcm = 1; }
        if (ROWS && two_bit) { s_row[t * 4 + 0] = rb00; s_row[t * 4 + 1] = rb01; s_row[t * 4 + 2] = rb10; s_row[t * 4 + 3] = rb11; }
        s_hasn[t] = (len_v & kReadHasN) ? 1 : 0;
    }
    PROF(0);
    if (ent_lds && t < ix.n_ent) { s_es[t] = (EntT)es_v; s_ee[t] = (EntT)ee_v; }
    s_k1[t] = 0xFFFFFFFFu; s_c2[t] = 0; s_nx[t] = 0xFFFFFFFFu;
    s_mm[t] = (uint8_t)(mm < 255 ? mm : 255);
    s_r[t] = r; s_geo[t] = (uint32_t)len | ((uint32_t)cl << 10) | ((uint32_t)cd << 20);
    {
        uint32_t v = my_total;
        for (int off = 1; off < 64; off <<= 1) { uint32_t u = __shfl_up(v, off); if (lane >= off) v += u; }
        if (lane == 63) s_wsum[wid] = v;
        __syncthreads();
        uint32_t add = 0;
        for (int w = 0; w < wid; w++) add += s_wsum[w];
        s_off[t] = add + v - my_total;
        if (t == BS - 1) s_off[BS] = add + v;
    }
    __syncthreads();
    PROF(1);

    const int init = mm + cfg.mm_delta + 1;
    int low_inst = 0, low_mm = init, nxt = init;
    int best_q = -1;
    uint32_t best_j = 0, best_x = 0, my_hit_t = 0;
    constexpr uint32_t kNone = 0xFFFFFFFFu, kOffStart = 1u << 18, kLazyBit = 1u << 16;

    for (uint32_t start = 0; start < BS;) {
        const uint32_t base = s_off[start];
        uint32_t lo = start + 1, hi = BS;
        while (lo < hi) {
            uint32_t mid = (lo + hi + 1) >> 1;
            if (s_off[mid] - base <= CAP) lo = mid; else hi = mid - 1;
        }
        const uint32_t end = lo;
        const uint32_t total = s_off[end] - base;
        for (uint32_t f0 = 0; f0 < total; f0 += KB * BS) {
            uint64_t tv[KB];
            uint32_t meta[KB];
#pragma unroll
            for (int i = 0; i < KB; i++) {
                const uint32_t f = f0 + (uint32_t)i * BS + t;
                meta[i] = kNone;
                tv[i] = 0;
                if (f < total) {
                    const uint32_t g = base + f;
                    uint32_t l2 = start, h2 = end - 1;
                    while (l2 < h2) {
                        uint32_t mid = (l2 + h2 + 1) >> 1;
                        if (s_off[mid] <= g) l2 = mid; else h2 = mid - 1;
                    }
                    const uint32_t ri = l2;
                    const uint32_t local = g - s_off[ri];
                    const uint16_t *sp = s_sp + ri * slots_max;
                    int q = 0;
                    while (sp[q] <= local) q++;
                    const uint32_t j = local - (q ? sp[q - 1] : 0);
                    uint64_t iv_f;
                    bool lazy, elem;
                    if (cf) { iv_f = s_first[ri * slots_max + q]; lazy = ((s_lazy[ri] >> q) & 1) != 0; elem = ((s_lazy[ri] >> (16 + q)) & 1) != 0; }
                    else {
                        const int sti = q >= cmaxs ? 1 : 0;
                        uint32_t iv_c;
                        iv_get(b, iv_slot(b, blockIdx.x * blockDim.x + ri, s0 + sti, q - sti * cmaxs), iv_f, iv_c);
                        lazy = (iv_c & kLazyFlag) != 0;
                        elem = (iv_c & kElemFlag) != 0;
                    }
                    tv[i] = elem ? iv_f : sa_get<WIDE>(ix, iv_f + j);
                    meta[i] = ri | ((uint32_t)q << 10) | (lazy ? kLazyBit : 0u);
                }
            }
            uint4 wv[KB][NBLK];
            uint4 rowv[KB][NW / 4];
            uint8_t fb0[KB], fb1[KB];
#pragma unroll
            for (int i = 0; i < KB; i++) {
                fb0[i] = 0; fb1[i] = 0;
#pragma unroll
                for (int u = 0; u < NBLK; u++) wv[i][u] = make_uint4(0, 0, 0, 0);
                if (meta[i] != kNone) {
                    const uint32_t ri = meta[i] & 1023u;
                    const int q = (int)((meta[i] >> 10) & 63u);
                    const int c = q >= cmaxs ? q - cmaxs : q;
                    const uint32_t geo = s_geo[ri];
                    const int c_len = (int)(geo & 1023u), c_cl = (int)((geo >> 10) & 1023u), c_cd = (int)(geo >> 20);
                    const int last = c_len - c_cl;
                    const int ofs = c * c_cd < last ? c * c_cd : last;
                    if (tv[i] >= (uint64_t)ofs) {
                        const uint64_t t0 = tv[i] - (uint64_t)ofs;
                        tv[i] = t0;
                        if (two_bit) {
                            const uint64_t g0 = t0 >> ix.flag_shift, g1 = (t0 + (uint64_t)c_len - 1) >> ix.flag_shift;
                            fb0[i] = ix.nflag[g0 >> 3];
                            fb1[i] = ix.nflag[g1 >> 3];
                            window2_load<NW>(ix.tgt2, ix.tgt2s, t0, c_len, wv[i]);
                            if (!ROWS && NW <= 8) {
                                const int sti = q >= cmaxs ? 1 : 0;
                                const uint4 *__restrict__ rp = reinterpret_cast<const uint4 *>(b.rd2 + ((uint64_t)s_r[ri] * 2 + (uint64_t)(s0 + sti)) * (NW / 2));
#pragma unroll
                                for (int u = 0; u < NW / 4; u++) rowv[i][u] = rp[u];
                            }
                        }
                    } else
                        meta[i] |= kOffStart;
                }
            }
#pragma unroll
            for (int i = 0; i < KB; i++) {
                if (meta[i] == kNone) continue;
                const uint32_t f = f0 + (uint32_t)i * BS + t;
                uint8_t rec = kRecSkip;
                if (!(meta[i] & kOffStart)) {
// ... 17 lines not shown
                        if (ROWS) {
#pragma unroll
                            for (int u = 0; u < NW / 4; u++) {
                                const uint4 v = s_row[(ri * 2 + st) * (NW / 4) + u];
                                r2w[2 * u] = ((uint64_t)v.y << 32) | v.x;
                                r2w[2 * u + 1] = ((uint64_t)v.w << 32) | v.z;
                            }
                        } else if (NW <= 8) {
#pragma unroll
                            for (int u = 0; u < NW / 4; u++) {
                                r2w[2 * u] = ((uint64_t)rowv[i][u].y << 32) | rowv[i][u].x;
                                r2w[2 * u + 1] = ((uint64_t)rowv[i][u].w << 32) | rowv[i][u].z;
                            }
                        } else
                            load_read_words2<NW>(b.rd2 + ((uint64_t)cr * 2 + st) * (NW / 2), r2w);
#pragma unroll
                        for (int u = 0; u < NW / 4; u++) rnm[u] = 0;
                        window2_compare<NW>(r2w, rnm, c_len, t0, wv[i], w);
                    }
                    if (flg) eval_window_rare<NW>(read_row(b, cr, st, s_hasn[ri] != 0), c_len, ix.tgt4, t0, w);
                    bool skip = w.eos || (lazy && !core_clean<NW>(w, ofs, c_cl));
#pragma unroll 1
                    for (int c2 = 0; c2 < c; c2++) skip |= core_clean<NW>(w, c2 * c_cd, c_cl);
                    if (!skip) rec = (uint8_t)(w.mm < 127 ? w.mm : 127);
                    if (WIDE) s_key[f] = (uint32_t)t0;
                    if (SMALL) s_t[f] = (uint32_t)t0;
                    if (!WIDE && rec != kRecSkip) {
                        atomicAdd(&s_c2[ri], 1u << 16);
                        if (rec <= s_mm[ri]) atomicMin(&s_k1[ri], ((uint32_t)rec << 16) | (base + f - s_off[ri]));
                    }
                }
                s_rec[f] = rec;
            }
        }
        PROF(2);
        __syncthreads();
        PROF(3);
        auto replay_sequential = [&]() __attribute__((always_inline)) {
            const uint16_t *sp = s_sp + t * slots_max;
            const uint32_t rb = s_off[t] - base;
            bool done = false;
            uint32_t prev = 0;
            for (int q = 0; q < slots_max && !done; q++) {
                if ((q >= cmaxs ? q - cmaxs : q) >= nc) continue;
                n_search++;
                const uint32_t upto = sp[q];
                for (uint32_t x = prev; x < upto; x++) {
                    const int cm = s_rec[rb + x];
                    if (cm == kRecSkip) continue;
                    n_cand++;
                    if (cm > mm || cm >= nxt) continue;
                    if (cm < low_mm) {
                        low_inst = 1; nxt = low_mm; low_mm = cm;
                        best_q = q; best_j = x - prev; best_x = x;
                    } else if (cm == low_mm)
                        low_inst++;
                    else
                        nxt = cm;
                    if (low_inst > cfg.max_hits && low_mm == 0) { done = true; break; }
                }
                prev = upto;
            }
        };
        if (WIDE) {
            for (uint32_t f = t; f < total; f += BS) {
                if (s_rec[f] == kRecSkip) continue;
                const uint32_t g = base + f;
                uint32_t l2 = start, h2 = end - 1;
                while (l2 < h2) {
                    uint32_t mid = (l2 + h2 + 1) >> 1;
                    if (s_off[mid] <= g) l2 = mid; else h2 = mid - 1;
                }
                const uint32_t rb = s_off[l2] - base, local = f - rb;
                const uint32_t second = (s1 > s0) ? (uint32_t)s_sp[l2 * slots_max + cmaxs - 1] : 0xFFFFFFFFu;
                const uint32_t from = local >= second ? second : 0u;
                const uint32_t kx = s_key[f];
                bool seen = false;
                uint32_t i = rb + from;
                const uint32_t i1 = rb + local;
                for (; i < i1 && (i & 3) != 0; i++) seen |= s_rec[i] != kRecSkip && s_key[i] == kx;
                for (; i + 4 <= i1 && !seen; i += 4) {
                    const uint4 k4 = *reinterpret_cast<const uint4 *>(&s_key[i]);
                    const uint32_t r4 = *reinterpret_cast<const uint32_t *>(&s_rec[i]);
                    seen = (k4.x == kx && (r4 & 0xffu) != kRecSkip) || (k4.y == kx && ((r4 >> 8) & 0xffu) != kRecSkip) ||
                           (k4.z == kx && ((r4 >> 16) & 0xffu) != kRecSkip) || (k4.w == kx && (r4 >> 24) != kRecSkip);
                }
                for (; i < i1 && !seen; i++) seen = s_rec[i] != kRecSkip && s_key[i] == kx;
                if (seen) s_rec[f] = kRecSkip;
            }
            __syncthreads();
            for (uint32_t f = t; f < total; f += BS) {
                const uint8_t rec = s_rec[f];
                if (rec == kRecSkip) continue;
                const uint32_t g = base + f;
                uint32_t l2 = start, h2 = end - 1;
                while (l2 < h2) {
                    uint32_t mid = (l2 + h2 + 1) >> 1;
                    if (s_off[mid] <= g) l2 = mid; else h2 = mid - 1;
                }
                atomicAdd(&s_c2[l2], 1u << 16);
                if (rec <= s_mm[l2]) atomicMin(&s_k1[l2], ((uint32_t)rec << 16) | (g - s_off[l2]));
            }
            __syncthreads();
        }
        {
            for (uint32_t f = t; f < total; f += BS) {
                const int cm = s_rec[f];
                if (cm == kRecSkip) continue;
                const uint32_t g = base + f;
                uint32_t l2 = start, h2 = end - 1;
                while (l2 < h2) {
                    uint32_t mid = (l2 + h2 + 1) >> 1;
                    if (s_off[mid] <= g) l2 = mid; else h2 = mid - 1;
                }
                if (cm > (int)s_mm[l2]) continue;
                if ((uint32_t)cm == (s_k1[l2] >> 16)) atomicAdd(&s_c2[l2], 1u);
                else atomicMin(&s_nx[l2], (uint32_t)cm);
            }
            __syncthreads();
            if (mine && t >= start && t < end) {
                const uint32_t k1 = s_k1[t], c2 = s_c2[t];
                if (k1 != 0xFFFFFFFFu && (k1 >> 16) == 0 && (int)(c2 & 0xFFFFu) > cfg.max_hits)
                    replay_sequential();
                else {
                    n_search += (uint32_t)((s1 - s0 + 1) * nc);
                    n_cand += c2 >> 16;
                    if (k1 != 0xFFFFFFFFu) {
                        low_mm = (int)(k1 >> 16);
                        low_inst = (int)(c2 & 0xFFFFu);
                        const uint32_t nx = s_nx[t];
                        nxt = nx < (uint32_t)init ? (int)nx : init;
                        const uint32_t local = k1 & 0xFFFFu;
                        const uint16_t *sp = s_sp + t * slots_max;
                        int q = 0;
                        while (sp[q] <= local) q++;
                        best_q = q;
                        best_j = local - (q ? sp[q - 1] : 0);
                        best_x = local;
                    }
                }
                if (SMALL && best_q >= 0) my_hit_t = s_t[s_off[t] - base + best_x];
            }
        }
        PROF(4);
        __syncthreads();
        PROF(5);
        start = end;
    }

    int rslt = BK_HR_NONE;
    if (mine) {
        rslt = classify(low_inst, low_mm, nxt, init, cfg.mm_delta, cfg.max_hits);
        if (rslt == BK_HR_NONE && phase + 1 < n_phases) {
            ReadPlan p = make_plan(len, cfg);
            int mm2, cl2, cd2, dummy[1];
            phase_params(p, cfg, phase + 1, mm2, cl2, cd2);
            int nc2 = core_offsets(len, cl2, cd2, p.max_slides, dummy, 0);
            if (nc2 <= kMaxCoresFast) my_cmax = (uint32_t)nc2;
            dest = 1;
        }
    }
    const uint64_t lt_mask = (1ULL << lane) - 1;
    for (int off = 32; off > 0; off >>= 1) {
        n_search += __shfl_down(n_search, off);
        n_cand += __shfl_down(n_cand, off);
        n_lcm += __shfl_down(n_lcm, off);
        uint32_t m = __shfl_down(my_cmax, off);
        my_cmax = m > my_cmax ? m : my_cmax;
    }
    uint32_t my_off = 0;
#pragma unroll
    for (int d = 1; d <= 3; d++) {
        uint64_t m = __ballot(dest == d);
        if (m) {
            uint32_t w = 0;
            if (lane == 0) w = atomicAdd(&s_cnt[d], (uint32_t)__popcll(m));
            w = __builtin_amdgcn_readfirstlane(w);
            if (dest == d) my_off = w + (uint32_t)__popcll(m & lt_mask);
        }
    }
    if (lane == 0) {
        if (my_cmax) atomicMax(&s_cmax, my_cmax);
        if (n_search) atomicAdd(&s_ctr[0], (unsigned long long)n_search);
        if (n_cand) atomicAdd(&s_ctr[1], (unsigned long long)n_cand);
        if (n_lcm) atomicAdd(&s_ctr[2], (unsigned long long)n_lcm);
    }
    PROF(6);
    __syncthreads();
    PROF(7);
    if (t >= 1 && t <= 3 && s_cnt[t]) s_base[t] = stripe_reserve(out, (int)t - 1, s_cnt[t]);
    if (t == 4 && s_cmax) stripe_max(out, s_cmax);
    if (t >= 8 && t < 11 && s_ctr[t - 8]) atomicAdd(&b.ctr[ctr_stripe() + t - 8], s_ctr[t - 8]);
    __syncthreads();
    PROF(8);
    if (dest) stripe_put(out, dest - 1, s_base[dest] + my_off, dest == 2 ? a : r);
    if (mine && rslt != BK_HR_NONE) {
        uint64_t hit_left = 0;
        int hit_strand = '?', e = -1;
        if (low_inst >= 1) {
            const int sti = best_q >= cmaxs ? 1 : 0, c = best_q - sti * cmaxs, st = s0 + sti;
            const int last = len - cl;
            const int ofs = c * cd < last ? c * cd : last;
            const uint64_t bf = cf ? (uint64_t)s_first[t * slots_max + best_q] : iv_start(b, iv_slot(b, a, st, c));
            const bool belem = cf ? ((s_lazy[t] >> (16 + best_q)) & 1) != 0 : (iv_count(b, iv_slot(b, a, st, c)) & kElemFlag) != 0;
            hit_left = SMALL ? (uint64_t)my_hit_t : (belem ? bf : sa_get<WIDE>(ix, bf + best_j)) - (uint64_t)ofs;
            hit_strand = st ? '-' : '+';
            if (ent_lds) {
                int lo = 0, hi = (int)ix.n_ent - 1;
                while (lo <= hi) {
                    int mid = (lo + hi) >> 1;
                    if (hit_left < (uint64_t)s_es[mid]) hi = mid - 1;
                    else if (hit_left > (uint64_t)s_ee[mid]) lo = mid + 1;
                    else { e = mid; break; }
                }
            } else
                e = find_entry(ix, hit_left);
        }
        write_result(ix, cfg, b, r, len, rslt, low_inst, low_mm, nxt, hit_left, e, hit_strand, phase << 1);
    }
#if defined(BK_PROF) && BK_PROF == 1
    PROF(9);
    PROF_END;
#endif
}

void launch_extend(const DevIndex &ix, const DevAlignCfg &cfg, const DevBatch &b, const uint32_t *act, uint32_t n_act,
                   int phase, uint32_t *next_act, uint32_t *next_cnt, uint32_t *heavy, uint32_t *heavy_cnt,
                   uint32_t *cmax_next, hipStream_t s)
{
    unsigned blocks = (n_act + 255) / 256;
    if (ix.sa_hi) hipLaunchKernelGGL(k_extend<true>, dim3(blocks), dim3(256), 0, s, ix, cfg, b, act, n_act, phase, next_act, next_cnt, heavy, heavy_cnt, cmax_next);
    else hipLaunchKernelGGL(k_extend<false>, dim3(blocks), dim3(256), 0, s, ix, cfg, b, act, n_act, phase, next_act, next_cnt, heavy, heavy_cnt, cmax_next);
}

void launch_flat(const DevIndex &ix, const DevAlignCfg &cfg, const DevBatch &b, const uint32_t *act, const uint32_t *p_n_act, uint32_t n_act_bound, int phase,
                 int slots_max, uint32_t *next_act, uint32_t *next_cnt, uint32_t *heavy, uint32_t *heavy_cnt, uint32_t *wave,
                 uint32_t *wave_cnt, uint32_t *cmax_next, uint32_t *const *stage, uint32_t *stripe_cnt, int nw, hipStream_t s)
{
    constexpr int bs = 256;
    nw &= 0xff;
    bool wide = ix.sa_hi != nullptr;
    if (!n_act_bound) return;
    unsigned blocks = (n_act_bound + (unsigned)bs - 1) / (unsigned)bs;
    if (slots_max < 1) slots_max = 1;
    size_t lds = (size_t)bs * slots_max * (flat_caches_first(wide, bs, slots_max) ? 6 : 2);
    StripeSet out;
    out.cnt = stripe_cnt;
    for (int i = 0; i < 3; i++) out.stage[i] = stage[i];
    out.cap = stripe_cap(blocks, (unsigned)bs);
    const int have_wave = wave != nullptr;
#define BK_FLAT(W, N) hipLaunchKernelGGL((k_flat<W, N, 256>), dim3(blocks), dim3(256), lds, s, ix, cfg, b, act, p_n_act, phase, slots_max, out, have_wave)
    if (nw <= 8) { if (wide) BK_FLAT(true, 8); else BK_FLAT(false, 8); }
    else if (nw <= 16) { if (wide) BK_FLAT(true, 16); else BK_FLAT(false, 16); }
    else if (nw <= kNwLong) { if (wide) BK_FLAT(true, kNwLong); else BK_FLAT(false, kNwLong); }
    else { if (wide) BK_FLAT(true, kNwLongest); else BK_FLAT(false, kNwLongest); }
#undef BK_FLAT
    uint32_t *dense[3] = {next_act, have_wave ? wave : heavy, heavy}, *total[3] = {next_cnt, have_wave ? wave_cnt : heavy_cnt, heavy_cnt};
    launch_compact(out, dense, total, 3, cmax_next, s);
}

#ifdef BK_PROF
int prof_read_flat(unsigned long long *out16) { return prof_read(out16); }
#endif

}
```

### biokanga_amd/csrc/bk_image.cpp

```cpp
#include "bk_engine_int.h"

#define SW_TRY(x) do { hipError_t e_ = (x); if (e_ != hipSuccess) { (void)hipGetLastError(); return e_ == hipErrorOutOfMemory ? BK_ERR_MEM : BK_ERR_INTERNAL; } } while (0)

namespace bk {
hipError_t dev_zero_now(void *p, size_t bytes)
{
    hipError_t e = hipMemset(p, 0, bytes);
    if (e == hipSuccess) e = hipStreamSynchronize(nullptr);
    return e;
}

hipError_t dev_malloc_bytes(void **p, size_t bytes)
{
    const int poison = env::poison();
    const bool timing = env::timing();
    timespec ta, tb;
    if (timing) clock_gettime(CLOCK_MONOTONIC, &ta);
    hipError_t e = hipMalloc(p, bytes);
    if (timing) {
        clock_gettime(CLOCK_MONOTONIC, &tb);
        const double ms = 1e3 * (double)(tb.tv_sec - ta.tv_sec) + 1e-6 * (double)(tb.tv_nsec - ta.tv_nsec);
        if (ms > 2.0) fprintf(stderr, "bk timing: hipMalloc of %.2f GB took %.1f ms\n", (double)bytes / 1e9, ms);
    }
    if (e == hipSuccess && poison >= 0 && bytes) {
// ... 842 lines not shown
    const int fd = ::open(sfx_path, O_RDONLY);
    if (fd < 0) { bk_ctx_destroy(c); return BK_ERR_OPNFILE; }
    const uint64_t seq_ofs = (uint64_t)(f.seq - (const uint8_t *)f.map_base), sa_ofs = (uint64_t)(f.sa - (const uint8_t *)f.map_base);
    bool sent = upload_file(d_seq.get(), fd, seq_ofs, f.concat_len, device_id) == BK_OK;
    clk.lap("upload bases");
    if (sent && sa_in_place) {
        rc = adopt_device_image(c, d_seq.get(), f.concat_len, nullptr, 4);
        d_seq.reset();
        TablePlan tp;
        if (!rc) rc = tables_begin(c, tp);
        const uint64_t n = f.concat_len;
        uint64_t n_slices = std::max<uint64_t>(1, std::min<uint64_t>(16, n >> 26));
        if (const unsigned long long ts = env::table_slices()) n_slices = std::max<uint64_t>(1, std::min<uint64_t>(ts, n));
        bool swin_sliced = false;
        if (!rc && eager_swin && swin_ahead && tp.ktab && tp.k2 && tp.isa && !c->ktab64 && c->use_wave && c->use_tgt2) {
            rc = setup_entries(c, ents.data(), (uint32_t)ents.size());
            if (!rc) { c->entries_set = true; rc = build_tgt2(c); }
            if (!rc) {
                c->tgt2_built = true;
                clk.lap("entry table, 2-bit target");
                int w[kSwLevels];
                const int n_levels = swin_core_lens_k(c, 100, tp.k, w);
                sb.ent_state = 1;
                swin_sliced = swin_begin(c, sb, w, n_levels, 3, swin_ahead, n / n_slices + 128, 1, c->stream) == BK_OK;
                if (!swin_sliced) { (void)hipGetLastError(); sb.ent_state = 0; }
                else sb.alloc_ahead(device_id, swin_ahead);
            }
        }
        for (uint64_t k = 0; k < n_slices && !rc && sent; k++) {
            const uint64_t i0 = (n * k / n_slices) & ~63ULL, i1 = k + 1 == n_slices ? n : (n * (k + 1) / n_slices) & ~63ULL;
            if (i1 <= i0) continue;
            sent = upload_file(c->image.sa_lo.get() + i0, fd, sa_ofs + i0 * 4, (i1 - i0) * 4, device_id) == BK_OK;
            if (sent) rc = tables_range(c, tp, i0, i1, swin_sliced ? sb.d_starts.get() : nullptr);
            if (sent && !rc && swin_sliced) {
                DevIndex ix = c->ix;
                ix.k = tp.k;
                ix.k2 = c->image.k2.get();
                if (swin_range(c, sb, ix, i1, c->stream) != BK_OK) { (void)hipGetLastError(); swin_sliced = false; }
            }
        }
        clk.lap("upload suffix array, tables enqueued behind its slices");
        if (!rc && sent) rc = tables_end(c, tp);
        clk.lap("tables finished");
        if (!rc && sent && swin_sliced && c->ix.k2 != nullptr) {
            const int re = swin_end(c, sb, c->stream);
            if (re == BK_ERR_INTERNAL) rc = re;
            clk.lap("window array finished");
            if (clk.on && c->image.swin.get()) fprintf(stderr, "biokanga_amd: window array for %.1f %% of the suffix array, %.2f GB, made behind the upload\n", 100.0 * c->swin_covered, c->swin_bytes / 1e9);
        }
    } else if (sent) {
        sent = upload_file(d_sa.get(), fd, sa_ofs, f.concat_len * f.el_size, device_id) == BK_OK;
        clk.lap("upload suffix array");
        if (sent) rc = adopt_device_image(c, d_seq.get(), f.concat_len, d_sa.get(), (int)f.el_size);
        clk.lap("pack target, adopt");
    }
    ::close(fd);
    d_seq.reset(); d_sa.reset();
    if (!sent) { bk_ctx_destroy(c); return BK_ERR_INTERNAL; }
    if (rc) { bk_ctx_destroy(c); return rc; }
    rc = finish_ctx(c, ents.data(), (uint32_t)ents.size());
    if (rc) { bk_ctx_destroy(c); return rc; }
    clk.lap("(rest of bk_ctx_create)");
    if (eager_swin) {
        rc = maybe_build_swin(c, 100, c->chunk_reads, c->stream);
        if (rc) { bk_ctx_destroy(c); return rc; }
    }
    *out = c;
    return BK_OK;
}

int bk_ctx_create_from_device(bk_ctx **out, const void *d_seq, uint64_t concat_len, const void *d_sa, int sfx_el_size,
                              const bk_entry_info *entries, uint32_t n_entries, int device_id, const bk_align_params *p)
{
    if (!d_seq || !d_sa || !entries || !n_entries || !concat_len || (sfx_el_size != 4 && sfx_el_size != 5)) return BK_ERR_PARAMS;
    bk_ctx *c = nullptr;
    int rc = new_ctx(out, device_id, p, &c);
    if (rc) return rc;
    c->dataset = "device";
    rc = adopt_device_image(c, (const uint8_t *)d_seq, concat_len, (const uint8_t *)d_sa, sfx_el_size);
    if (!rc) rc = finish_ctx(c, entries, n_entries);
    if (rc) { bk_ctx_destroy(c); return rc; }
    *out = c;
    return BK_OK;
}

int bk_ctx_clone(bk_ctx **out, const bk_ctx *src, int device_id)
{
    if (!src) return BK_ERR_PARAMS;
    bk_ctx *c = nullptr;
    int rc = new_ctx(out, device_id, &src->params, &c);
    if (rc) return rc;
    StageClock clk;
    c->dataset = src->dataset;
    c->el_size = src->el_size;
    c->n_tgt4_words = src->n_tgt4_words;
    c->sort_shift = src->sort_shift;
    c->ktab64 = src->ktab64;
    c->ktab_wide = src->ktab_wide;
    c->ktab_is2 = src->ktab_is2;
    c->use_ktab2 = src->use_ktab2;
    c->grow_elem = src->grow_elem;
    c->use_k3 = src->use_k3;
    c->sort_lists = src->sort_lists; c->sort_lists_set = src->sort_lists_set;
    c->grow_enabled = src->grow_enabled && src->grow_state.load() != 4; c->grow_after = src->grow_after; c->grow_wait = src->grow_wait;
    c->use_ktab = src->use_ktab; c->k_req = src->k_req; c->use_k2 = src->use_k2; c->use_isa = src->use_isa; c->use_wave = src->use_wave; c->use_tgt2 = src->use_tgt2;
    c->ix.n = src->ix.n;
    c->ix.k = src->ix.k;
    c->ix.flag_shift = src->ix.flag_shift;
    c->ix.nflag_bytes = src->ix.nflag_bytes;
    bool ok = true;
    auto dup = [&](auto &dst, const auto &from) {
        if (!ok || !from.get()) return;
        if (dst.ensure(from.cap()) != hipSuccess) { ok = false; rc = BK_ERR_MEM; return; }
        const size_t bytes = from.cap() * sizeof(*from.get());
        hipError_t e = c->device == src->device ? hipMemcpyAsync(dst.get(), from.get(), bytes, hipMemcpyDeviceToDevice, c->stream)
                                                : hipMemcpyPeerAsync(dst.get(), c->device, from.get(), src->device, bytes, c->stream);
        if (e != hipSuccess) { ok = false; rc = BK_ERR_INTERNAL; }
    };
    ImageBufs &im = c->image;
    const ImageBufs &sim = src->image;
    dup(im.tgt4, sim.tgt4);
    dup(im.sa_lo, sim.sa_lo);
    dup(im.sa_hi, sim.sa_hi);
    dup(im.ktab, sim.ktab);
    dup(im.ktab_hi, sim.ktab_hi);
    dup(im.k2, sim.k2);
    for (int i = 0; i < kMoreKeys; i++) dup(im.kx[i], sim.kx[i]);
    dup(im.isa, sim.isa);
    dup(im.tgt2, sim.tgt2);
    dup(im.tgt2s, sim.tgt2s);
    dup(im.nflag, sim.nflag);
    c->use_swin = src->use_swin;
    if (ok && hipStreamSynchronize(c->stream) != hipSuccess) { ok = false; rc = BK_ERR_INTERNAL; }
    if (!ok) { bk_ctx_destroy(c); return rc; }
    publish_index(c);
    clk.lap("index image copied from the first device");
    rc = setup_entries(c, src->entries.data(), (uint32_t)src->entries.size());
    if (rc) { bk_ctx_destroy(c); return rc; }
    *out = c;
    return BK_OK;
}

void bk_ctx_destroy(bk_ctx *c)
{
    if (!c) return;
    (void)hipSetDevice(c->device);
    grow_drop(c);
    if (c->stream) (void)hipStreamSynchronize(c->stream);
    c->release_image_buffers();
    c->release_batch_buffers();
    if (c->h_small) (void)hipHostFree(c->h_small);
    for (void *&t : c->sam_text) if (t) { (void)hipHostFree(t); t = nullptr; }
    if (c->h_ctl) (void)hipHostFree(c->h_ctl);
    if (c->ev_ctl) (void)hipEventDestroy(c->ev_ctl);
    if (c->ev_wait) (void)hipEventDestroy(c->ev_wait);
    for (hipEvent_t e : c->ev_pool) (void)hipEventDestroy(e);
    if (c->stream) (void)hipStreamDestroy(c->stream);
    bk::live_contexts()--;
    delete c;
}


}
```

### biokanga_amd/csrc/bk_prep.hip

```cpp
#include "bk_dev_util.h"

namespace bk {


__global__ void __launch_bounds__(256) k_compact_lists(CompactJobs J)
{
    const int li = blockIdx.y;
    __shared__ uint32_t s_pre[kListStripes + 1];
    if (threadIdx.x < 64) {
        uint32_t run = 0;
        for (int s0 = 0; s0 < kListStripes; s0 += 64) {
            uint32_t v = J.set.cnt[(s0 + threadIdx.x) * 16 + li];
            for (int off = 1; off < 64; off <<= 1) { uint32_t u = __shfl_up(v, off); if ((int)threadIdx.x >= off) v += u; }
            s_pre[s0 + threadIdx.x + 1] = run + v;
            run += __shfl(v, 63);
        }
        if (threadIdx.x == 0) s_pre[0] = 0;
    }
    __syncthreads();
    const uint32_t tot = s_pre[kListStripes], old = *J.total[li];
    const uint32_t *__restrict__ stage = J.set.stage[li];
    uint32_t *__restrict__ dense = J.dense[li];
    for (uint32_t i = blockIdx.x * 256 + threadIdx.x; i < tot; i += gridDim.x * 256) {
        int lo = 0, hi = kListStripes - 1;
        while (lo < hi) {
            const int mid = (lo + hi + 1) >> 1;
            if (s_pre[mid] <= i) lo = mid; else hi = mid - 1;
        }
        dense[old + i] = stage[(uint64_t)lo * J.set.cap + (i - s_pre[lo])];
    }
}

__global__ void k_finish_lists(CompactJobs J)
{
    uint32_t sum[3] = {0, 0, 0}, mx = 0;
    for (int s0 = threadIdx.x; s0 < kListStripes; s0 += 64) {
        uint32_t *line = J.set.cnt + s0 * 16;
#pragma unroll
        for (int li = 0; li < 3; li++) { sum[li] += line[li]; line[li] = 0; }
        uint32_t *mline = J.set.cnt + (kListStripes + s0) * 16;
        mx = mline[0] > mx ? mline[0] : mx;
        mline[0] = 0;
    }
    for (int off = 32; off > 0; off >>= 1) {
#pragma unroll
        for (int li = 0; li < 3; li++) sum[li] += __shfl_down(sum[li], off);
        const uint32_t q = __shfl_down(mx, off);
        mx = q > mx ? q : mx;
    }
    if (threadIdx.x == 0) {
        for (int li = 0; li < J.n; li++) if (sum[li]) *J.total[li] += sum[li];
        if (J.max_out && mx > *J.max_out) *J.max_out = mx;
    }
}


struct __attribute__((packed)) Bytes16 { uint64_t lo, hi; };

__device__ __forceinline__ uint64_t pack8_msb(uint64_t y)
{
    y &= 0x0707070707070707ULL;
    y = (y | (y >> 4)) & 0x00FF00FF00FF00FFULL;
    y = (y | (y >> 8)) & 0x0000FFFF0000FFFFULL;
    y = (y | (y >> 16)) & 0x00000000FFFFFFFFULL;
    return y;
}

__device__ __forceinline__ uint64_t complement8(uint64_t x)
{
    x &= 0x0707070707070707ULL;
    return x ^ (((~x >> 2) & 0x0101010101010101ULL) * 3);
}


__device__ __forceinline__ uint32_t rev2_32(uint32_t x)
{
    x = __brev(x);
    return ((x >> 1) & 0x55555555u) | ((x & 0x55555555u) << 1);
}
__device__ __forceinline__ uint64_t rev2_64(uint64_t x)
{
    x = __brevll(x);
    return ((x >> 1) & 0x5555555555555555ULL) | ((x & 0x5555555555555555ULL) << 1);
}

__device__ __forceinline__ uint32_t packed_word16(const uint32_t *__restrict__ W, int len, int w, bool rc)
{
    const int rem = len - 16 * w;
    if (rem <= 0) return 0;
    const uint32_t keep = rem >= 16 ? 0xFFFFFFFFu : ~0u << (32 - 2 * rem);
    if (!rc) return W[w] & keep;
    const int p = len - 16 * w - 16;
    uint32_t x;
    if (p >= 0) {
        const int i = p >> 4;
        const unsigned s = (unsigned)(p & 15) << 1;
        const uint64_t c = ((uint64_t)W[i] << 32) | W[i + 1];
        x = (uint32_t)(c >> (32 - s));
    } else
        x = W[0] >> (unsigned)(2 * (-p));
    return ~rev2_32(x) & keep;
}

template <int W>
__device__ __forceinline__ void revcomp2(const uint64_t (&f)[W], int len, uint64_t (&r)[W])
{
    uint64_t v[W + 1];
#pragma unroll
    for (int i = 0; i < W; i++) v[i] = ~rev2_64(f[W - 1 - i]);
    v[W] = 0;
    const int sh = 2 * (32 * W - len), q = sh >> 6;
    const unsigned bsh = (unsigned)(sh & 63);
#pragma unroll
    for (int step = 1; step <= W; step <<= 1) {
        const bool on = (q & step) != 0;
        uint64_t nv[W + 1];
#pragma unroll
        for (int i = 0; i <= W; i++) nv[i] = on ? (i + step <= W ? v[i + step <= W ? i + step : W] : 0ULL) : v[i];
#pragma unroll
        for (int i = 0; i <= W; i++) v[i] = nv[i];
    }
#pragma unroll
    for (int i = 0; i < W; i++) r[i] = bsh ? ((v[i] << bsh) | (v[i + 1] >> (64 - bsh))) : v[i];
}

__global__ void __launch_bounds__(256) k_mark_exc(DevBatch b)
{
    const uint64_t i = (uint64_t)blockIdx.x * blockDim.x + threadIdx.x;
    if (i >= b.pk_nexc) return;
    const bk_nbase e = b.pk_exc[i];
    const uint32_t rr = e.read - b.pk_read0;
    if (rr >= b.n_reads) return;
    if (e.code == 4) atomicAdd(&b.rmeta[rr], ((uint32_t)e.run + 1u) << 16);
    else atomicOr(&b.rmeta[rr], 1u << 31);
}

__global__ void __launch_bounds__(256) k_exc_rows(DevBatch b)
{
    const uint64_t i = (uint64_t)blockIdx.x * blockDim.x + threadIdx.x;
    if (i >= b.pk_nexc) return;
    const uint32_t rd = b.pk_exc[i].read;
    const uint32_t rr = rd - b.pk_read0;
    if (rr >= b.n_reads || (i > 0 && b.pk_exc[i - 1].read == rd)) return;
    for (uint32_t st = 0; st < 2; st++)
        for (uint32_t w = 0; w < b.wpr; w++) {
            uint64_t v = 0;
            if (w < b.nw) {
                const uint64_t x = b.rd2[((uint64_t)rr * 2 + st) * (b.nw / 2) + (w >> 1)];
                v = spread2to4((w & 1) ? (uint32_t)x : (uint32_t)(x >> 32));
            }
            b.rd4[((uint64_t)rr * 2 + st) * b.wpr + w] = v;
        }
}

__global__ void __launch_bounds__(256) k_apply_exc(DevBatch b)
{
    const uint64_t i = (uint64_t)blockIdx.x * blockDim.x + threadIdx.x;
    if (i >= b.pk_nexc) return;
    const bk_nbase e = b.pk_exc[i];
    const uint32_t rr = e.read - b.pk_read0;
    if (rr >= b.n_reads) return;
    const int len = (int)b.lens[rr];
    const int lo2[2] = {(int)e.pos, len - 1 - (int)e.pos - (int)e.run}, hi2[2] = {(int)e.pos + (int)e.run, len - 1 - (int)e.pos};
    const unsigned long long code16 = 0x1111111111111111ULL * (unsigned long long)(e.code & 7);
    for (int st = 0; st < 2; st++) {
        for (int w = lo2[st] >> 4; w <= (hi2[st] >> 4); w++) {
            const int a = lo2[st] > 16 * w ? lo2[st] - 16 * w : 0, z = hi2[st] < 16 * w + 15 ? hi2[st] - 16 * w : 15;
            const unsigned long long m = (~0ULL >> (4 * a)) & (~0ULL << (60 - 4 * z));
            unsigned long long *p = reinterpret_cast<unsigned long long *>(b.rd4 + ((uint64_t)rr * 2 + st) * b.wpr + w);
            atomicAnd(p, ~m);
            atomicOr(p, code16 & m);
        }
    }
}

__global__ void __launch_bounds__(256) k_check_exc(const bk_nbase *__restrict__ exc, uint64_t n_exc, const uint32_t *__restrict__ lens, uint32_t n_reads,
                                                   uint32_t *__restrict__ bad)
{
    const uint64_t i = (uint64_t)blockIdx.x * blockDim.x + threadIdx.x;
    if (i >= n_exc) return;
    const bk_nbase e = exc[i];
    bool ok = e.read < n_reads && e.code >= 4 && e.code <= 7;
    if (ok) ok = (uint32_t)e.pos + e.run < lens[e.read];
    if (ok && i > 0) {
        const bk_nbase q = exc[i - 1];
        ok = q.read < e.read || (q.read == e.read && (uint32_t)q.pos + q.run < e.pos);
    }
    if (!ok) atomicAdd(bad, 1u);
}

__global__ void __launch_bounds__(256) k_widen_lens(const uint16_t *__restrict__ lens16, uint32_t n, uint32_t *__restrict__ lens32,
                                                    unsigned long long *__restrict__ nwords)
{
    const uint32_t i = blockIdx.x * blockDim.x + threadIdx.x;
    if (i >= n) return;
    const uint32_t l = lens16[i];
    lens32[i] = l;
    nwords[i] = (l + 15) >> 4;
}

__global__ void __launch_bounds__(256) k_packed_extent(const uint64_t *__restrict__ offs, const uint32_t *__restrict__ lens, uint32_t n,
                                                       unsigned long long *__restrict__ out)
{
    unsigned long long e = 0, l = 0;
    for (uint64_t i = (uint64_t)blockIdx.x * blockDim.x + threadIdx.x; i < n; i += (uint64_t)gridDim.x * blockDim.x) {
        const unsigned long long len = lens[i], end = offs[i] + ((len + 15) >> 4);
        e = end > e ? end : e;
        l = len > l ? len : l;
    }
    for (int off = 32; off > 0; off >>= 1) {
        const unsigned long long e2 = __shfl_down(e, off), l2 = __shfl_down(l, off);
        e = e2 > e ? e2 : e;
        l = l2 > l ? l2 : l;
    }
    if ((threadIdx.x & 63) == 0) {
        if (e) atomicMax(out + 0, e);
        if (l) atomicMax(out + 1, l);
    }
}

void launch_packed_extent(const uint64_t *offs, const uint32_t *lens, uint32_t n, unsigned long long *out, hipStream_t s)
{
    unsigned blocks = (n + 255) / 256;
    if (blocks > 2048) blocks = 2048;
    if (n) hipLaunchKernelGGL(k_packed_extent, dim3(blocks), dim3(256), 0, s, offs, lens, n, out);
}

void launch_widen_lens(const uint16_t *lens16, uint32_t n, uint32_t *lens32, unsigned long long *nwords, hipStream_t s)
{
    if (n) hipLaunchKernelGGL(k_widen_lens, dim3((n + 255) / 256), dim3(256), 0, s, lens16, n, lens32, nwords);
}

void launch_check_exc(const bk_nbase *exc, uint64_t n_exc, const uint32_t *lens, uint32_t n_reads, uint32_t *bad, hipStream_t s)
{
    if (n_exc) hipLaunchKernelGGL(k_check_exc, dim3((unsigned)((n_exc + 255) / 256)), dim3(256), 0, s, exc, n_exc, lens, n_reads, bad);
}

__global__ void __launch_bounds__(256) k_pack_reads(DevBatch b, const uint32_t *__restrict__ pairs, uint32_t n_pairs)
{
    const uint32_t wpr = b.wpr;
    const uint32_t per_read = 2 * wpr;
    const uint32_t rpb = 256 / per_read;
    const uint32_t lr = threadIdx.x / per_read;
    if (lr >= rpb) return;
    uint64_t r = (uint64_t)blockIdx.x * rpb + lr;
    if (pairs != nullptr) {
        if (r >= 2ULL * n_pairs) return;
        r = 2ULL * pairs[r >> 1] + (r & 1);
    }
    if (r >= b.n_reads) return;
    const uint32_t rem = threadIdx.x - lr * per_read;
    const uint32_t st = rem >= wpr ? 1 : 0, w = rem - st * wpr;
    int len = (int)b.lens[r];
    if (b.pk_words != nullptr) {
        b.rd4[r * per_read + rem] = spread2to4(packed_word16(b.pk_words + b.offs[r], len, (int)w, st != 0));
        return;
    }
    const uint8_t *s = b.bases + b.offs[r];
    uint64_t v = 0;
    int base0 = 16 * (int)w;
    if (base0 + 16 <= len) {
        if (st == 0) {
            Bytes16 q = *reinterpret_cast<const Bytes16 *>(s + base0);
            v = (pack8_msb(__builtin_bswap64(q.lo)) << 32) | pack8_msb(__builtin_bswap64(q.hi));
        } else {
            Bytes16 q = *reinterpret_cast<const Bytes16 *>(s + (len - 16 - base0));
            v = (pack8_msb(complement8(q.hi)) << 32) | pack8_msb(complement8(q.lo));
        }
    } else if (base0 < len) {
        int cnt = len - base0;
        if (st == 0) {
            for (int k = 0; k < cnt; k++) v |= (uint64_t)(s[base0 + k] & 7) << (60 - 4 * k);
        } else {
            for (int k = 0; k < cnt; k++) {
                uint8_t x = s[len - 1 - base0 - k] & 7;
                x = x < 4 ? (uint8_t)(3 - x) : x;
                v |= (uint64_t)x << (60 - 4 * k);
            }
        }
    }
    b.rd4[r * per_read + rem] = v;
}

#ifndef BK_PREP_TRANSPOSE
#define BK_PREP_TRANSPOSE 1
#endif
template <int NW, bool PACKED>
__global__ void __launch_bounds__(256) k_prep_fused(DevAlignCfg cfg, DevBatch b, StripeSet out)
{
    __shared__ uint32_t s_cnt, s_base, s_cmax;
    constexpr bool TR = NW == 8 && BK_PREP_TRANSPOSE;
    __shared__ uint4 s_tr[TR ? 4 : 1][TR ? 64 * (NW / 2) : 1];
    if (threadIdx.x == 0) { s_cnt = 0; s_cmax = 0; }
    __syncthreads();
    const uint32_t r = blockIdx.x * blockDim.x + threadIdx.x;
    const bool lean = b.rd2 != nullptr;
    const int wv = threadIdx.x >> 6;
    const bool wave_full = (r | 63u) < b.n_reads;
    bool go = false, has_n = false;
    uint32_t my_cmax = 0;
    int len = 0;
    uint64_t fw[PACKED ? 1 : NW], rv[PACKED ? 1 : NW];
    uint64_t f2[NW / 2], r2[NW / 2];
    bk_hit h;
    if (r < b.n_reads) {
        len = (int)b.lens[r];
        int num_ns = 0;
        bool bad = false;
        if (PACKED) {
            const uint32_t *__restrict__ W = b.pk_words + b.offs[r];
            uint32_t wv[NW];
#pragma unroll
            for (int k = 0; k < NW; k++) wv[k] = W[k];
#pragma unroll
            for (int k = 0; k < NW / 2; k++) {
                uint64_t v = ((uint64_t)wv[2 * k] << 32) | wv[2 * k + 1];
                const int rem = len - 32 * k;
                if (rem < 32) v = rem <= 0 ? 0ULL : (v & (~0ULL << (64 - 2 * rem)));
                f2[k] = v;
            }
            revcomp2<NW / 2>(f2, len, r2);
            const uint32_t pre = b.rmeta[r];
            num_ns = (int)((pre >> 16) & 0x7FFFu);
            bad = (pre >> 31) != 0;
        } else {
            const uint8_t *s = b.bases + b.offs[r];
#pragma unroll
            for (int w = 0; w < NW; w++) {
                const int base0 = 16 * w;
                uint64_t f = 0;
                if (base0 + 16 <= len) {
                    Bytes16 q = *reinterpret_cast<const Bytes16 *>(s + base0);
                    f = (pack8_msb(__builtin_bswap64(q.lo)) << 32) | pack8_msb(__builtin_bswap64(q.hi));
                } else if (base0 < len) {
                    const int cnt = len - base0;
                    for (int k = 0; k < cnt; k++) f |= (uint64_t)(s[base0 + k] & 7) << (60 - 4 * k);
                }
                fw[w] = f;
                rv[w] = 0;
            }
#pragma unroll
            for (int w = 0; w < NW; w++) {
                if (16 * w < len) {
                    uint64_t x = fw[w] & top_mask(len - 16 * w);
                    uint64_t hi = x & 0x4444444444444444ULL;
                    uint64_t lo = (x | (x >> 1)) & 0x1111111111111111ULL;
                    bad |= ((hi >> 2) & lo) != 0;
                    num_ns += __popcll(hi);
                }
            }
#pragma unroll
            for (int k = 0; k < NW / 2; k++) f2[k] = ((uint64_t)squeeze2(fw[2 * k]) << 32) | squeeze2(fw[2 * k + 1]);
            if (lean && !bad && num_ns == 0) revcomp2<NW / 2>(f2, len, r2);
            else {
#pragma unroll
                for (int w = 0; w < NW; w++) {
                    const int base0 = 16 * w;
                    uint64_t v = 0;
                    if (base0 + 16 <= len) {
                        Bytes16 p = *reinterpret_cast<const Bytes16 *>(s + (len - 16 - base0));
                        v = (pack8_msb(complement8(p.hi)) << 32) | pack8_msb(complement8(p.lo));
                    } else if (base0 < len) {
                        const int cnt = len - base0;
                        for (int k = 0; k < cnt; k++) {
                            uint8_t x = s[len - 1 - base0 - k] & 7;
                            x = x < 4 ? (uint8_t)(3 - x) : x;
                            v |= (uint64_t)x << (60 - 4 * k);
                        }
                    }
                    rv[w] = v;
                }
#pragma unroll
                for (int k = 0; k < NW / 2; k++) r2[k] = ((uint64_t)squeeze2(rv[2 * k]) << 32) | squeeze2(rv[2 * k + 1]);
            }
        }
        h.chrom_id = 0; h.match_loci = 0; h.match_len = 0; h.low_hit_instances = 0; h.rslt = 0;
        h.nar = BK_NAR_NOHIT; h.strand = '?'; h.low_mm = 0; h.nxt_low_mm = 0; h.num_hits = 0; h.mismatches = 0; h.flags = 0;
        int max_ns_seq = 0;
        if (cfg.max_ns) {
            max_ns_seq = (len * cfg.max_ns) / 100;
            if (max_ns_seq < cfg.max_ns) max_ns_seq = cfg.max_ns;
        }
        if (bad || num_ns > max_ns_seq) h.nar = BK_NAR_NS;
        has_n = bad || num_ns > 0;
        if (h.nar != BK_NAR_NS) {
            ReadPlan p = make_plan(len, cfg);
            if (p.n_phases > 0) {
                int mm, cl, cd, ofs[1];
                phase_params(p, cfg, 0, mm, cl, cd);
                int nc = core_offsets(len, cl, cd, p.max_slides, ofs, 0);
                if (nc <= kMaxCoresFast) my_cmax = (uint32_t)nc;
                go = true;
            }
        }
    }
    const int lane = threadIdx.x & 63;
    uint64_t m = __ballot(go);
    uint32_t my_off = 0;
    for (int off = 32; off > 0; off >>= 1) { uint32_t q = __shfl_down(my_cmax, off); my_cmax = q > my_cmax ? q : my_cmax; }
    if (m) {
        uint32_t w = 0;
        if (lane == 0) { w = atomicAdd(&s_cnt, (uint32_t)__popcll(m)); if (my_cmax) atomicMax(&s_cmax, my_cmax); }
        w = __builtin_amdgcn_readfirstlane(w);
        my_off = w + (uint32_t)__popcll(m & ((1ULL << lane) - 1));
    }
    __syncthreads();
    if (threadIdx.x == 0 && s_cnt) s_base = stripe_reserve(out, 0, s_cnt);
    if (threadIdx.x == 64 && s_cmax) stripe_max(out, s_cmax);
    __syncthreads();
    if (go) stripe_put(out, 0, s_base + my_off, r);
    if (r < b.n_reads) {
        b.rmeta[r] = (uint32_t)len | (has_n ? kReadHasN : 0u);
        if (PACKED ? !lean : (!lean || has_n)) {
            const uint32_t wpr = b.wpr;
            uint4 *row0 = reinterpret_cast<uint4 *>(b.rd4 + (uint64_t)r * 2 * wpr);
            uint4 *row1 = reinterpret_cast<uint4 *>(b.rd4 + ((uint64_t)r * 2 + 1) * wpr);
#pragma unroll
            for (int q = 0; q < NW / 2; q++) {
                if (2 * q < (int)wpr) {
                    uint64_t a0, a1, c0, c1;
                    if (PACKED) {
                        a0 = spread2to4((uint32_t)(f2[q] >> 32)); a1 = spread2to4((uint32_t)f2[q]);
                        c0 = spread2to4((uint32_t)(r2[q] >> 32)); c1 = spread2to4((uint32_t)r2[q]);
                    } else { a0 = fw[PACKED ? 0 : 2 * q]; a1 = fw[PACKED ? 0 : 2 * q + 1]; c0 = rv[PACKED ? 0 : 2 * q]; c1 = rv[PACKED ? 0 : 2 * q + 1]; }
                    row0[q] = make_uint4((uint32_t)a0, (uint32_t)(a0 >> 32), (uint32_t)a1, (uint32_t)(a1 >> 32));
                    row1[q] = make_uint4((uint32_t)c0, (uint32_t)(c0 >> 32), (uint32_t)c1, (uint32_t)(c1 >> 32));
                }
            }
            for (uint32_t q = NW / 2; 2 * q < wpr; q++) { row0[q] = make_uint4(0, 0, 0, 0); row1[q] = make_uint4(0, 0, 0, 0); }
        }
        if (lean && !(TR && wave_full)) {
            uint4 *t0 = reinterpret_cast<uint4 *>(b.rd2 + (uint64_t)r * 2 * (NW / 2));
            uint4 *t1 = reinterpret_cast<uint4 *>(b.rd2 + ((uint64_t)r * 2 + 1) * (NW / 2));
#pragma unroll
            for (int q = 0; q < NW / 4; q++) {
                t0[q] = make_uint4((uint32_t)f2[2 * q], (uint32_t)(f2[2 * q] >> 32), (uint32_t)f2[2 * q + 1], (uint32_t)(f2[2 * q + 1] >> 32));
                t1[q] = make_uint4((uint32_t)r2[2 * q], (uint32_t)(r2[2 * q] >> 32), (uint32_t)r2[2 * q + 1], (uint32_t)(r2[2 * q + 1] >> 32));
            }
        }
        if (!(TR && wave_full)) b.out[r] = h;
    }
    if (TR && wave_full) {
        constexpr int RW = NW / 2;
        uint4 *sr = s_tr[wv];
        if (lean) {
#pragma unroll
            for (int q = 0; q < NW / 4; q++) {
                sr[lane * RW + q] = make_uint4((uint32_t)f2[2 * q], (uint32_t)(f2[2 * q] >> 32), (uint32_t)f2[2 * q + 1], (uint32_t)(f2[2 * q + 1] >> 32));
                sr[lane * RW + NW / 4 + q] = make_uint4((uint32_t)r2[2 * q], (uint32_t)(r2[2 * q] >> 32), (uint32_t)r2[2 * q + 1], (uint32_t)(r2[2 * q + 1] >> 32));
            }
            __builtin_amdgcn_wave_barrier();
            uint4 *dst = reinterpret_cast<uint4 *>(b.rd2 + (uint64_t)(r - (uint32_t)lane) * 2 * (NW / 2));
#pragma unroll
            for (int k = 0; k < RW; k++) dst[k * 64 + lane] = sr[k * 64 + lane];
            __builtin_amdgcn_wave_barrier();
        }
        uint32_t *sh = reinterpret_cast<uint32_t *>(sr);
        const uint32_t *hw = reinterpret_cast<const uint32_t *>(&h);
#pragma unroll
        for (int k = 0; k < 5; k++) sh[lane * 5 + k] = hw[k];
        __builtin_amdgcn_wave_barrier();
        uint32_t *od = reinterpret_cast<uint32_t *>(b.out + (r - (uint32_t)lane));
#pragma unroll
        for (int k = 0; k < 5; k++) od[k * 64 + lane] = sh[k * 64 + lane];
    }
}

__global__ void __launch_bounds__(1024) k_init_reads(DevAlignCfg cfg, DevBatch b, uint32_t *__restrict__ act,
                                                      uint32_t *__restrict__ act_cnt, uint32_t *__restrict__ cmax)
{
    __shared__ uint32_t s_cnt, s_base, s_cmax;
    if (threadIdx.x == 0) { s_cnt = 0; s_cmax = 0; }
    __syncthreads();
    uint32_t r = blockIdx.x * blockDim.x + threadIdx.x;
    bool go = false;
    uint32_t my_cmax = 0;
    if (r < b.n_reads) {
        int len = (int)b.lens[r];
        bk_hit h;
        h.chrom_id = 0; h.match_loci = 0; h.match_len = 0; h.low_hit_instances = 0; h.rslt = 0;
        h.nar = BK_NAR_NOHIT; h.strand = '?'; h.low_mm = 0; h.nxt_low_mm = 0; h.num_hits = 0; h.mismatches = 0; h.flags = 0;
        int max_ns_seq = 0;
        if (cfg.max_ns) {
            max_ns_seq = (len * cfg.max_ns) / 100;
            if (max_ns_seq < cfg.max_ns) max_ns_seq = cfg.max_ns;
        }
        const uint64_t *fw = b.rd4 + (uint64_t)r * 2 * b.wpr;
        int num_ns = 0;
        bool bad = false;
        for (int w = 0; 16 * w < len; w++) {
            uint64_t x = fw[w] & top_mask(len - 16 * w);
            uint64_t hi = x & 0x4444444444444444ULL;
            uint64_t lo = (x | (x >> 1)) & 0x1111111111111111ULL;
            bad |= ((hi >> 2) & lo) != 0;
            num_ns += __popcll(hi);
        }
        if (bad || num_ns > max_ns_seq) h.nar = BK_NAR_NS;
        b.out[r] = h;
        b.rmeta[r] = (uint32_t)len | ((bad || num_ns > 0) ? kReadHasN : 0u);
        if (h.nar != BK_NAR_NS) {
            ReadPlan p = make_plan(len, cfg);
            if (p.n_phases > 0) {
                int mm, cl, cd, ofs[1];
                phase_params(p, cfg, 0, mm, cl, cd);
                int nc = core_offsets(len, cl, cd, p.max_slides, ofs, 0);
                if (nc <= kMaxCoresFast) my_cmax = (uint32_t)nc;
                go = true;
            }
        }
    }
    const int lane = threadIdx.x & 63;
    uint64_t m = __ballot(go);
    uint32_t my_off = 0;
    for (int off = 32; off > 0; off >>= 1) { uint32_t q = __shfl_down(my_cmax, off); my_cmax = q > my_cmax ? q : my_cmax; }
    if (m) {
        uint32_t w = 0;
        if (lane == 0) { w = atomicAdd(&s_cnt, (uint32_t)__popcll(m)); if (my_cmax) atomicMax(&s_cmax, my_cmax); }
        w = __builtin_amdgcn_readfirstlane(w);
        my_off = w + (uint32_t)__popcll(m & ((1ULL << lane) - 1));
    }
    __syncthreads();
    if (threadIdx.x == 0 && s_cnt) s_base = atomicAdd(act_cnt, s_cnt);
    if (threadIdx.x == 64 && s_cmax) atomicMax(cmax, s_cmax);
    __syncthreads();
    if (go) act[s_base + my_off] = r;
}

__global__ void __launch_bounds__(256) k_expand_rd4(DevBatch b, const uint32_t *__restrict__ list, uint32_t n_list)
{
    const uint32_t per_read = 2 * b.wpr;
    const uint64_t tid = (uint64_t)blockIdx.x * blockDim.x + threadIdx.x;
    const uint64_t item = tid / per_read;
    if (item >= n_list) return;
    const uint32_t rem = (uint32_t)(tid - item * per_read);
    const uint32_t r = list ? list[item] : (uint32_t)item;
    if (b.rmeta[r] & kReadHasN) return;
    const uint32_t st = rem >= b.wpr ? 1 : 0, w = rem - st * b.wpr;
    uint64_t v = 0;
    if (w < b.nw) {
        const uint64_t x = b.rd2[((uint64_t)r * 2 + st) * (b.nw / 2) + (w >> 1)];
        v = spread2to4((w & 1) ? (uint32_t)x : (uint32_t)(x >> 32));
    }
    b.rd4[((uint64_t)r * 2 + st) * b.wpr + w] = v;
}

void expand_rd4(const DevBatch &b, const uint32_t *list, uint32_t n_list, hipStream_t s)
{
    if (b.rd2 == nullptr || !n_list) return;
    const uint64_t threads = (uint64_t)n_list * 2 * b.wpr;
    hipLaunchKernelGGL(k_expand_rd4, dim3((unsigned)((threads + 255) / 256)), dim3(256), 0, s, b, list, n_list);
}

__global__ void __launch_bounds__(256) k_max_len(const uint32_t *__restrict__ lens, uint32_t n, uint32_t *__restrict__ out)
{
    __shared__ uint32_t s_max;
    if (threadIdx.x == 0) s_max = 0;
    __syncthreads();
    uint32_t v = 0;
    for (uint64_t i = (uint64_t)blockIdx.x * blockDim.x + threadIdx.x; i < n; i += (uint64_t)gridDim.x * blockDim.x) {
        uint32_t w = lens[i];
        v = w > v ? w : v;
    }
    for (int off = 32; off > 0; off >>= 1) { uint32_t w = __shfl_down(v, off); v = w > v ? w : v; }
    if ((threadIdx.x & 63) == 0 && v) atomicMax(&s_max, v);
    __syncthreads();
    if (threadIdx.x == 0 && s_max) atomicMax(out, s_max);
}

void launch_max_len(const uint32_t *lens, uint32_t n, uint32_t *out, hipStream_t s)
{
    uint32_t blocks = (n + 255) / 256;
    if (blocks > 2048) blocks = 2048;
    if (n) hipLaunchKernelGGL(k_max_len, dim3(blocks), dim3(256), 0, s, lens, n, out);
}

void launch_compact(const StripeSet &set, uint32_t *const *dense, uint32_t *const *total, int n, uint32_t *max_out, hipStream_t s)
{
    CompactJobs J;
    J.set = set;
    for (int i = 0; i < 3; i++) { J.dense[i] = dense[i < n ? i : 0]; J.total[i] = total[i < n ? i : 0]; }
    J.max_out = max_out;
    J.n = n;
    hipLaunchKernelGGL(k_compact_lists, dim3(1024, (unsigned)n), dim3(256), 0, s, J);
    hipLaunchKernelGGL(k_finish_lists, dim3(1), dim3(64), 0, s, J);
}

void launch_pack_rows(const DevBatch &b, hipStream_t s, const uint32_t *pairs, uint32_t n_pairs)
{
    const uint32_t rpb = 256 / (2 * b.wpr);
    const uint64_t n = pairs != nullptr ? 2ULL * n_pairs : b.n_reads;
    if (!n) return;
    hipLaunchKernelGGL(k_pack_reads, dim3((unsigned)((n + rpb - 1) / rpb)), dim3(256), 0, s, b, pairs, n_pairs);
    if (b.pk_words != nullptr && b.pk_nexc) hipLaunchKernelGGL(k_apply_exc, dim3((unsigned)((b.pk_nexc + 255) / 256)), dim3(256), 0, s, b);
}

void launch_prep(const DevAlignCfg &cfg, const DevBatch &b, uint32_t *act, uint32_t *act_cnt, uint32_t *cmax, uint32_t *stage,
                 uint32_t *stripe_cnt, hipStream_t s)
{
    const bool packed = b.pk_words != nullptr;
    const unsigned eblocks = (unsigned)((b.pk_nexc + 255) / 256);
    if (b.nw == 8 || b.nw == 16 || b.nw == kNwLong || b.nw == kNwLongest) {
        const unsigned blocks = (b.n_reads + 255) / 256;
        StripeSet out;
        out.cnt = stripe_cnt;
        out.stage[0] = out.stage[1] = out.stage[2] = stage;
        out.cap = stripe_cap(blocks, 256);
        if (packed) {
            launch_fill_u64(reinterpret_cast<unsigned long long *>(b.rmeta), ((uint64_t)b.n_reads + 1) / 2, 0ULL, s);
            if (eblocks) hipLaunchKernelGGL(k_mark_exc, dim3(eblocks), dim3(256), 0, s, b);
            if (b.nw == 8) hipLaunchKernelGGL((k_prep_fused<8, true>), dim3(blocks), dim3(256), 0, s, cfg, b, out);
            else if (b.nw == 16) hipLaunchKernelGGL((k_prep_fused<16, true>), dim3(blocks), dim3(256), 0, s, cfg, b, out);
            else if (b.nw == kNwLong) hipLaunchKernelGGL((k_prep_fused<kNwLong, true>), dim3(blocks), dim3(256), 0, s, cfg, b, out);
            else hipLaunchKernelGGL((k_prep_fused<kNwLongest, true>), dim3(blocks), dim3(256), 0, s, cfg, b, out);
            if (eblocks && b.rd2 != nullptr) hipLaunchKernelGGL(k_exc_rows, dim3(eblocks), dim3(256), 0, s, b);
            if (eblocks) hipLaunchKernelGGL(k_apply_exc, dim3(eblocks), dim3(256), 0, s, b);
        } else if (b.nw == 8) hipLaunchKernelGGL((k_prep_fused<8, false>), dim3(blocks), dim3(256), 0, s, cfg, b, out);
        else if (b.nw == 16) hipLaunchKernelGGL((k_prep_fused<16, false>), dim3(blocks), dim3(256), 0, s, cfg, b, out);
        else if (b.nw == kNwLong) hipLaunchKernelGGL((k_prep_fused<kNwLong, false>), dim3(blocks), dim3(256), 0, s, cfg, b, out);
        else hipLaunchKernelGGL((k_prep_fused<kNwLongest, false>), dim3(blocks), dim3(256), 0, s, cfg, b, out);
        launch_compact(out, &act, &act_cnt, 1, cmax, s);
        return;
    }
    launch_pack_rows(b, s);
    hipLaunchKernelGGL(k_init_reads, dim3((b.n_reads + 1023) / 1024), dim3(1024), 0, s, cfg, b, act, act_cnt, cmax);
}

}
```

### biokanga_amd/csrc/bk_search.hip

```cpp
#include <algorithm>

#include "bk_dev_k2.h"
#include "bk_dev_prof.h"

namespace bk {



template <bool WIDE>
__global__ void __launch_bounds__(256) k_search(DevIndex ix, DevAlignCfg cfg, DevBatch b, const uint32_t *__restrict__ act,
                                                uint32_t n_act, int phase, int cmax, int nstr, int lazy)
{
    uint64_t tid = (uint64_t)blockIdx.x * blockDim.x + threadIdx.x;
    uint32_t per_read = (uint32_t)(nstr * cmax);
    uint64_t a = tid / per_read;
    if (a >= n_act) return;
    uint32_t rem = (uint32_t)(tid - a * per_read);
    int si = (int)(rem / (uint32_t)cmax), c = (int)(rem % (uint32_t)cmax);
    uint32_t r = act[a];
    const uint32_t meta = b.rmeta[r];
    int len = (int)(meta & kReadLenMask);
    ReadPlan p = make_plan(len, cfg);
    int mm, cl, cd;
    phase_params(p, cfg, phase, mm, cl, cd);
    int cur = cd, o = 0, n = 0, my_ofs = -1;
    while (n < p.max_slides && o <= len - cl && cur > cl / 3) {
        if (o + cl + cur > len) cur = len - (o + cl);
        if (n == c) my_ofs = o;
        n++;
        o += cur;
    }
    if (my_ofs < 0 || n > kMaxCoresFast) return;
    int strand = cfg.align_strand == 2 ? 1 : si;
    const RdRow rdw = read_row(b, r, strand, (meta & kReadHasN) != 0);
    uint64_t first, count;
    uint64_t slot = iv_slot(b, (uint32_t)a, strand, c);
    if (lazy && ix.k > 0 && cl >= ix.k) {
        uint64_t p0 = rdw.nib16(my_ofs) & top_mask(cl);
        uint64_t lo, hi;
        core_range(ix, p0, cl, lo, hi);
        if (hi - lo <= kLazyBucket && !(lo == 0 && hi == ix.n)) {
            iv_put(b, slot, lo, (uint32_t)(hi - lo) | (hi > lo ? kLazyFlag : 0u));
            return;
        }
    }
    search_core<WIDE>(ix, rdw, my_ofs, cl, ~0ULL >> 1, first, count);
    iv_put(b, slot, first, count > 0x7FFFFFFFULL ? 0x7FFFFFFFu : (uint32_t)count);
}


template <int ILP>
__global__ void __launch_bounds__(256) k_search_a_ilp(DevIndex ix, DevAlignCfg cfg, DevBatch b, const uint32_t *__restrict__ act,
                                                      const uint32_t *__restrict__ p_n_act, int phase, int cmax, int nstr, int lazy,
                                                      StripeSet out)
{
    __shared__ uint32_t s_cnt, s_base;
#if defined(BK_PROF) && BK_PROF == 2
    PROF_BEGIN;
#endif
    const uint32_t n_act = *p_n_act;
    const uint32_t per_read = (uint32_t)(nstr * cmax);
    const uint64_t total = (uint64_t)n_act * per_read;
    constexpr uint64_t stride = 256;
    const int k = ix.k;
  for (uint64_t tile0 = (uint64_t)blockIdx.x * (256 * ILP); tile0 < total; tile0 += (uint64_t)gridDim.x * (256 * ILP)) {
    if (threadIdx.x == 0) s_cnt = 0;
    __syncthreads();
    bool on[ILP], push[ILP], have_code[ILP];
    uint64_t slot[ILP], p0[ILP], first[ILP], lo[ILP], hi[ILP];
    uint32_t nval[ILP], q2raw[ILP];
    int cl[ILP];
    constexpr uint32_t kNoIv32 = 0xFFFFFFFFu;
    uint32_t cix[ILP];
    uint2 cv[ILP];
    bool cached[ILP];
    uint32_t key0[ILP];
#pragma unroll
    for (int u = 0; u < ILP; u++) {
        const uint64_t tid = tile0 + threadIdx.x + (uint64_t)u * stride;
        on[u] = false; push[u] = false; have_code[u] = false; slot[u] = 0; p0[u] = 0; q2raw[u] = 0; first[u] = 0; nval[u] = 0; cl[u] = 1; lo[u] = hi[u] = 0;
        cix[u] = kNoIv32; cv[u] = make_uint2(0, kNoIv32); cached[u] = false;
        if (tid < total) {
            const uint64_t a = tid / per_read;
            const uint32_t rem = (uint32_t)(tid - a * per_read);
            const int si = (int)(rem / (uint32_t)cmax), c = (int)(rem % (uint32_t)cmax);
            const uint32_t r = act[a];
            const uint32_t meta = b.rmeta[r];
            const int len = (int)(meta & kReadLenMask);
            const int strand_c = cfg.align_strand == 2 ? 1 : si;
            if (b.iv32 != nullptr && c == 0 && phase > 0) cv[u] = b.iv32[(uint32_t)strand_c * b.n_reads + r];
            ReadPlan p = make_plan(len, cfg);
            int mm, cd, dummy[1];
            phase_params(p, cfg, phase, mm, cl[u], cd);
            const int nc = core_offsets(len, cl[u], cd, p.max_slides, dummy, 0);
            if (c < nc && nc <= kMaxCoresFast) {
                on[u] = true;
                if (b.iv32 != nullptr && c == 0 && cl[u] >= k + kK2Bases) {
                    cix[u] = (uint32_t)strand_c * b.n_reads + r;
                    cached[u] = phase > 0 && cv[u].y != kNoIv32 && (cv[u].y < (1u << kKindShift) || (lazy && (cv[u].y & kIvFlags) == kIvFlags));
                }
                const int my_ofs = c * cd < len - cl[u] ? c * cd : len - cl[u];
                const int strand = cfg.align_strand == 2 ? 1 : si;
                slot[u] = iv_slot(b, (uint32_t)a, strand, c);
                if (b.rd2 != nullptr && !(meta & kReadHasN)) {
                    const uint64_t *row = b.rd2 + ((uint64_t)r * 2 + strand) * (b.nw / 2);
                    const uint64_t x = bits64_2(row, my_ofs);
                    p0[u] = spread2to4((uint32_t)(x >> 32)) & top_mask(cl[u]);
                    q2raw[u] = k == 16 ? (uint32_t)x : (uint32_t)(bits64_2(row, my_ofs + k) >> 32);
                } else {
                    const uint64_t *rdw = b.rd4 + ((uint64_t)r * 2 + strand) * b.wpr;
                    p0[u] = nib16(rdw, my_ofs) & top_mask(cl[u]);
                    const uint64_t q4 = nib16(rdw, my_ofs + k);
                    q2raw[u] = squeeze2(q4);
                    const int rem2 = cl[u] - k;
                    if (rem2 > 0 && (q4 & 0x4444444444444444ULL & top_mask(rem2 < kK2Bases ? rem2 : kK2Bases))) p0[u] |= 0x4000000000000000ULL;
                }
            }
        }
    }
    PROFS(0);
#pragma unroll
    for (int u = 0; u < ILP; u++) {
        nval[u] = kKindFull << kKindShift;
        push[u] = on[u];
        have_code[u] = on[u] && !cached[u] && cl[u] >= k && !(p0[u] & 0x4444444444444444ULL & top_mask(k));
        key0[u] = kK2Above;
        if (have_code[u]) {
            const uint64_t code = (uint64_t)(squeeze2(p0[u]) >> (32 - 2 * k));
            if (ix.ktab2 != nullptr) {
                const uint2 e0 = ix.ktab2[code], e1 = ix.ktab2[code + 1];
                lo[u] = e0.x; hi[u] = e1.x; key0[u] = e0.y;
            } else {
                ktab_get_pair(ix, code, lo[u], hi[u]);
            }
        }
    }
    PROFS(1);
    uint32_t key[ILP][kInlineBucket];
    bool absent[ILP];
    bool carry[ILP];
#pragma unroll
    for (int u = 0; u < ILP; u++) {
        const uint64_t size = hi[u] - lo[u];
        const uint32_t m = k2_mask(cl[u] - k);
        absent[u] = have_code[u] && ix.ktab2 != nullptr && size >= 2 && ktab2_absent(key0[u], m, q2raw[u] & m);
        carry[u] = have_code[u] && lazy && ix.ktab2 != nullptr && ix.ktab2_elem && size == 1;
        const bool key_in_entry = size == 1 && ix.ktab2 != nullptr && !ix.ktab2_elem;
#pragma unroll
        for (uint32_t j = 0; j < kInlineBucket; j++)
            key[u][j] = (have_code[u] && !absent[u] && !carry[u] && size <= kInlineBucket && j < size) ? (key_in_entry ? key0[u] : ix.k2[lo[u] + j]) : kK2Above;
    }
    PROFS(2);
#pragma unroll
    for (int u = 0; u < ILP; u++) {
        uint2 leave = make_uint2(0, kNoIv32);
        if (cached[u] && (cv[u].y & kElemFlag)) {
            first[u] = cv[u].x;
            nval[u] = cv[u].y;
            push[u] = false;
        } else if (cached[u]) {
            first[u] = cv[u].x;
            const uint32_t cnt = cv[u].y;
            if (cnt == 0 || cl[u] <= k + kK2Bases) { nval[u] = cnt; push[u] = false; }
            else if (lazy && cnt <= kLazyBucket) { nval[u] = cnt | kLazyFlag; push[u] = false; }
            else nval[u] = cnt | (kKindDeep << kKindShift);
        }
        if (carry[u]) {
            first[u] = key0[u];
            nval[u] = 1u | kIvFlags;
            push[u] = false;
            leave = make_uint2(key0[u], 1u | kIvFlags);
        } else if (have_code[u]) {
            const uint64_t size = hi[u] - lo[u];
            if (size == 0 || absent[u]) { first[u] = lo[u]; nval[u] = 0; push[u] = false; leave = make_uint2((uint32_t)lo[u], 0u); }
            else if (size <= kInlineBucket) {
                const uint32_t m = k2_mask(cl[u] - k), q2 = q2raw[u] & m;
                uint32_t lb = 0, ub = 0;
                bool suspect = false;
#pragma unroll
                for (uint32_t j = 0; j < kInlineBucket; j++) {
                    const int cm = k2_cmp(key[u][j], m, q2);
                    lb += cm < 0;
                    ub += cm <= 0;
                    suspect |= cm == 0 && k2_nkind(key[u][j]);
                }
                if (suspect) {
                    first[u] = lo[u];
                    nval[u] = (uint32_t)size | (kKindK2 << kKindShift);
                } else {
                    first[u] = lo[u] + lb;
                    const uint32_t cnt = ub - lb;
                    leave = make_uint2((uint32_t)first[u], cnt);
                    if (cnt == 0 || cl[u] <= k + kK2Bases) { nval[u] = cnt; push[u] = false; }
                    else if (lazy && cnt <= kLazyBucket) { nval[u] = cnt | kLazyFlag; push[u] = false; }
                    else nval[u] = cnt | (kKindDeep << kKindShift);
                }
            } else if (size < (1ULL << kKindShift)) {
                first[u] = lo[u];
                nval[u] = (uint32_t)size | (kKindK2 << kKindShift);
            }
        }
        if (phase == 0 && cix[u] != kNoIv32) b.iv32[cix[u]] = leave;
    }
    PROFS(3);
    const int lane = threadIdx.x & 63;
    uint32_t my_off[ILP];
#pragma unroll
    for (int u = 0; u < ILP; u++) {
        my_off[u] = 0;
        const uint64_t m = __ballot(push[u]);
        if (m) {
            uint32_t w = 0;
            if (lane == 0) w = atomicAdd(&s_cnt, (uint32_t)__popcll(m));
            w = __builtin_amdgcn_readfirstlane(w);
            my_off[u] = w + (uint32_t)__popcll(m & ((1ULL << lane) - 1));
        }
    }
    PROFS(4);
    __syncthreads();
    const uint64_t tile = tile0 / (256 * ILP);
    if (threadIdx.x == 0 && s_cnt) s_base = stripe_reserve_tile(out, 0, s_cnt, tile);
    __syncthreads();
    PROFS(5);
#pragma unroll
    for (int u = 0; u < ILP; u++) {
        if (push[u]) stripe_put_tile(out, 0, s_base + my_off[u], (uint32_t)slot[u], tile);
        if (on[u]) iv_put(b, slot[u], first[u], nval[u]);
    }
    __syncthreads();
  }
#if defined(BK_PROF) && BK_PROF == 2
    PROFS(6);
    PROF_END;
#endif
}

template <bool WIDE>
__global__ void __launch_bounds__(256) k_search_b(DevIndex ix, DevAlignCfg cfg, DevBatch b, int phase, int lazy,
                                                  const uint32_t *__restrict__ list, const uint32_t *__restrict__ sorted, uint32_t n_sorted,
                                                  const uint32_t *__restrict__ p_n_list)
{
    __shared__ uint64_t s_lv[kK2Levels + 1];
    if (threadIdx.x <= (unsigned)kK2Levels) s_lv[threadIdx.x] = threadIdx.x ? k2s_start(ix.n, (int)threadIdx.x) : 0;
    __syncthreads();
    const uint32_t n_list = *p_n_list;
    const uint32_t n_grouped = sorted != nullptr ? (n_list < n_sorted ? n_list : n_sorted) : 0u;
  for (uint32_t i = blockIdx.x * blockDim.x + threadIdx.x; i < n_list; i += gridDim.x * blockDim.x) {
#ifdef BK_DIAG_B
    unsigned long long d_k2 = 0, d_deep = 0, d_sa = 0;
    struct Fin { unsigned long long &a, &b, &c; DevBatch &bb; __device__ ~Fin() { if (a + b) atomicAdd(&bb.ctr[ctr_stripe() + 5], a + b); if (c) atomicAdd(&bb.ctr[ctr_stripe() + 6], c); } } fin{d_k2, d_deep, d_sa, b};
#endif
    const uint64_t slot = i < n_grouped ? sorted[i] : list[i];
    const uint32_t r = b.act[(uint32_t)(slot % b.iv_stride)], sc = (uint32_t)(slot / b.iv_stride);
    const int strand = (int)(sc / b.iv_cores), c = (int)(sc % b.iv_cores);
    const uint32_t meta = b.rmeta[r];
    const int len = (int)(meta & kReadLenMask);
    ReadPlan p = make_plan(len, cfg);
    int mm, cl, cd;
    phase_params(p, cfg, phase, mm, cl, cd);
    const int my_ofs = c * cd < len - cl ? c * cd : len - cl;
    const RdRow rdw = read_row(b, r, strand, (meta & kReadHasN) != 0);
    uint64_t first;
    uint32_t raw;
    iv_get(b, slot, first, raw);
    const uint32_t kind = raw >> kKindShift;
    uint64_t cnt = raw & ((1u << kKindShift) - 1);
    const int k = ix.k;
    if (kind == kKindFull) {
        search_core<WIDE>(ix, rdw, my_ofs, cl, ~0ULL >> 1, first, cnt);
        iv_put(b, slot, first, cnt > 0x7FFFFFFFULL ? 0x7FFFFFFFu : (uint32_t)cnt);
        continue;
    }
    if (kind == kKindK2) {
        const uint32_t m = k2_mask(cl - k);
        const uint32_t q2 = squeeze2(rdw.nib16(my_ofs + k)) & m;
        uint64_t l1, l2;
        unsigned long long k2_lines = 0;
        k2_bounds(ix.k2, s_lv, first, cnt, m, q2, l1, l2, k2_lines);
#ifdef BK_DIAG_B
        d_k2 += 1 + (k2_lines << 32);
#endif
        {
            const int upto = cl < k + kK2Bases ? cl : k + kK2Bases;
            while (l2 > l1) {
                const uint32_t kv = ix.k2[l2 - 1];
                if (!k2_nkind(kv) || cmp_core_from(rdw, my_ofs, upto, k, ix.tgt4, sa_get<WIDE>(ix, l2 - 1)) == 0) break;
                l2--;
            }
        }
        first = l1;
        cnt = l2 - l1;
        if (!WIDE && b.iv32 != nullptr && phase == 0 && c == 0 && cl >= k + kK2Bases)
            b.iv32[(uint32_t)strand * b.n_reads + r] = make_uint2((uint32_t)first, (uint32_t)cnt);
        if (cnt == 0 || cl <= k + kK2Bases) {
            iv_put(b, slot, first, cnt > 0x7FFFFFFFULL ? 0x7FFFFFFFu : (uint32_t)cnt);
            continue;
        }
    }
    if (lazy && cnt <= kLazyBucket) {
        iv_put(b, slot, first, (uint32_t)cnt | kLazyFlag);
        continue;
    }
    int start = k + kK2Bases;
    bool settled = false;
    for (int lv = 0; lv < kMoreKeys && ix.kx[lv] != nullptr; lv++) {
        const uint32_t *__restrict__ kx = ix.kx[lv];
        const uint64_t p3 = rdw.nib16(my_ofs + start);
        if (p3 & 0x4444444444444444ULL & top_mask(cl - start < kK2Bases ? cl - start : kK2Bases)) break;
        const uint32_t m3 = k2_mask(cl - start);
        const uint32_t q3 = squeeze2(p3) & m3;
        uint64_t l1, l2;
        unsigned long long k3_lines = 0;
        k2_bounds(kx, s_lv, first, cnt, m3, q3, l1, l2, k3_lines);
#ifdef BK_DIAG_B
        d_deep += 1 + (k3_lines << 32);
#endif
        {
            const int upto = cl < start + kK2Bases ? cl : start + kK2Bases;
            while (l2 > l1) {
                const uint32_t kv = kx[l2 - 1];
                if (!k2_nkind(kv) || cmp_core_from(rdw, my_ofs, upto, start, ix.tgt4, sa_get<WIDE>(ix, l2 - 1)) == 0) break;
                l2--;
            }
        }
        first = l1;
        cnt = l2 - l1;
        start += kK2Bases;
        if (cnt == 0 || cl <= start) {
            iv_put(b, slot, first, cnt > 0x7FFFFFFFULL ? 0x7FFFFFFFu : (uint32_t)cnt);
            settled = true;
            break;
        }
        if (lazy && cnt <= kLazyBucket) {
            iv_put(b, slot, first, (uint32_t)cnt | kLazyFlag);
            settled = true;
            break;
        }
    }
    if (settled) continue;
    {
        uint64_t l1 = first, h1 = first + cnt, l2 = first, h2 = first + cnt;
        while (l1 < h1 || l2 < h2) {
            const bool a1 = l1 < h1, a2 = l2 < h2;
            const uint64_t m1 = l1 + ((h1 - l1) >> 1), m2 = l2 + ((h2 - l2) >> 1);
#ifdef BK_DIAG_B
            d_sa += (2ULL << 32) * (a1 + (a2 && m1 != m2));
#endif
            const uint64_t s1 = a1 ? sa_get<WIDE>(ix, m1) : 0, s2 = a2 ? sa_get<WIDE>(ix, m2) : 0;
            const int c1 = a1 ? cmp_core_from(rdw, my_ofs, cl, start, ix.tgt4, s1) : 0;
            const int c2 = a2 ? cmp_core_from(rdw, my_ofs, cl, start, ix.tgt4, s2) : 0;
            if (a1) { if (c1 > 0) l1 = m1 + 1; else h1 = m1; }
            if (a2) { if (c2 >= 0) l2 = m2 + 1; else h2 = m2; }
        }
        first = l1;
#ifdef BK_DIAG_B
        d_sa += 1;
#endif
        cnt = l2 - l1;
    }
    iv_put(b, slot, first, cnt > 0x7FFFFFFFULL ? 0x7FFFFFFFu : (uint32_t)cnt);
  }
}

void launch_search(const DevIndex &ix, const DevAlignCfg &cfg, const DevBatch &b, const uint32_t *act, uint32_t n_act,
                   int phase, int cmax, int nstr, int lazy, hipStream_t s)
{
    uint64_t threads = (uint64_t)n_act * (uint64_t)(cmax * nstr);
    unsigned blocks = (unsigned)((threads + 255) / 256);
    if (ix.sa_hi) hipLaunchKernelGGL(k_search<true>, dim3(blocks), dim3(256), 0, s, ix, cfg, b, act, n_act, phase, cmax, nstr, lazy);
    else hipLaunchKernelGGL(k_search<false>, dim3(blocks), dim3(256), 0, s, ix, cfg, b, act, n_act, phase, cmax, nstr, lazy);
}

__global__ void __launch_bounds__(256) k_keys_search(DevBatch b, const uint32_t *__restrict__ list, const uint32_t *__restrict__ p_n, uint32_t n_sort, int shift,
                                                     uint32_t *__restrict__ keys)
{
    const uint32_t n = *p_n;
    for (uint32_t i = blockIdx.x * blockDim.x + threadIdx.x; i < n_sort; i += gridDim.x * blockDim.x)
        keys[i] = i < n ? (uint32_t)(iv_start(b, list[i]) >> shift) : 0xFFFFFFFFu;
}

void launch_keys_search(const DevBatch &b, const uint32_t *list, const uint32_t *p_n, uint32_t n_sort, int shift, uint32_t *keys, hipStream_t s)
{
    if (!n_sort) return;
    unsigned blocks = (n_sort + 255) / 256;
    if (blocks > 16384) blocks = 16384;
    hipLaunchKernelGGL(k_keys_search, dim3(blocks), dim3(256), 0, s, b, list, p_n, n_sort, shift, keys);
}

void launch_search_a(const DevIndex &ix, const DevAlignCfg &cfg, const DevBatch &b, const uint32_t *act, const uint32_t *p_n_act, uint32_t n_act_bound,
                     int phase, int cmax, int nstr, int lazy, uint32_t *list, uint32_t *list_cnt, uint32_t *stage, uint32_t *stripe_cnt,
                     hipStream_t s)
{
    uint64_t threads = (uint64_t)n_act_bound * (uint64_t)(cmax * nstr);
    if (!threads) return;
    lazy &= 0xff;
    constexpr int ilp = 2;
    const uint64_t per = (uint64_t)256 * (uint64_t)ilp;
    const uint64_t tiles = (threads + per - 1) / per;
    const unsigned blocks = (unsigned)std::min<uint64_t>(tiles, 16384);
    StripeSet out;
    out.cnt = stripe_cnt;
    out.stage[0] = out.stage[1] = out.stage[2] = stage;
    out.cap = stripe_cap((unsigned)tiles, (unsigned)per);
    hipLaunchKernelGGL(k_search_a_ilp<2>, dim3(blocks), dim3(256), 0, s, ix, cfg, b, act, p_n_act, phase, cmax, nstr, lazy, out);
    launch_compact(out, &list, &list_cnt, 1, nullptr, s);
}

void launch_search_b(const DevIndex &ix, const DevAlignCfg &cfg, const DevBatch &b, int phase, int lazy, const uint32_t *list, const uint32_t *sorted,
                     uint32_t n_sorted, const uint32_t *p_n_list, uint64_t n_bound, hipStream_t s)
{
    if (!n_bound) return;
    unsigned blocks = (unsigned)std::min<uint64_t>((n_bound + 255) / 256, 32768);
    if (ix.sa_hi) hipLaunchKernelGGL(k_search_b<true>, dim3(blocks), dim3(256), 0, s, ix, cfg, b, phase, lazy, list, sorted, n_sorted, p_n_list);
    else hipLaunchKernelGGL(k_search_b<false>, dim3(blocks), dim3(256), 0, s, ix, cfg, b, phase, lazy, list, sorted, n_sorted, p_n_list);
}

__global__ void __launch_bounds__(256) k_clear_iv(DevBatch b, const uint32_t *__restrict__ p_n_act, int cmax, int st0, int st1, uint32_t word)
{
    const uint32_t n_act = *p_n_act;
    const uint64_t per_strand = (uint64_t)cmax * n_act, total = per_strand * (uint64_t)(st1 - st0 + 1);
    for (uint64_t i = (uint64_t)blockIdx.x * blockDim.x + threadIdx.x; i < total; i += (uint64_t)gridDim.x * blockDim.x) {
        const int st = st0 + (int)(i / per_strand);
        const uint64_t q = i % per_strand;
        const uint64_t slot = iv_slot(b, (uint32_t)(q % n_act), st, (int)(q / n_act));
        if (b.iv2) b.iv2[slot] = make_uint2(word, word);
        else { b.iv_first[slot] = word ? ~0ULL : 0ULL; b.iv_n[slot] = word; }
    }
}

void launch_clear_iv(const DevBatch &b, const uint32_t *p_n_act, uint32_t n_act_bound, int cmax, int st0, int st1, uint32_t word, hipStream_t s)
{
    const uint64_t total = (uint64_t)n_act_bound * (uint64_t)cmax * (uint64_t)(st1 - st0 + 1);
    if (!total) return;
    const unsigned blocks = (unsigned)std::min<uint64_t>((total + 255) / 256, 16384);
    hipLaunchKernelGGL(k_clear_iv, dim3(blocks), dim3(256), 0, s, b, p_n_act, cmax, st0, st1, word);
}

}

namespace bk { int prof_read_flat(unsigned long long *out16); }
extern "C" int bk_debug_prof(unsigned long long *out16)
{
#if defined(BK_PROF) && BK_PROF == 2
    return bk::prof_read(out16);
#elif defined(BK_PROF)
    return bk::prof_read_flat(out16);
#else
    (void)out16;
    return 1;
#endif
}
```

### biokanga_amd/csrc/bk_tune.cpp

```cpp
#include "bk_engine_int.h"

using namespace bk;

extern "C" {

int bk_ctx_reserve(bk_ctx *c, uint32_t max_batch_reads, uint32_t max_read_len)
{
    if (!c || !max_batch_reads || !max_read_len || max_read_len > (uint32_t)kMaxReadLenAbs) return BK_ERR_PARAMS;
    HIP_TRY(hipSetDevice(c->device));
    const uint32_t n = std::min(max_batch_reads, c->chunk_reads);
    const uint32_t wpr = words_per_read(max_read_len);
    const bool reg_path = c->use_wave && max_read_len <= 16u * (uint32_t)kNwLongest;
    const bool two_bit = reg_path && c->ix.tgt2 != nullptr;
    const uint32_t ivc = iv_cores_for(c, max_read_len);
    int rc = ensure_batch_scratch(c, n, wpr, two_bit ? rd2w_for(max_read_len) : 0u, ivc);
    if (rc) return rc;
    if (c->ix.k2) {
        const uint64_t lanes = (uint64_t)n * ivc * (c->cfg.align_strand == 0 ? 2u : 1u);
        rc = ensure_slist(c, lanes, c->stream);
        if (rc) return rc;
    }
    if (c->sort_lists) { rc = ensure_sort_scratch(c, n, c->stream); if (rc) return rc; }
    if (c->use_wave && c->ix.isa == nullptr) { rc = size_heavy_scratch(c); if (rc) return rc; }
    return BK_OK;
}

int bk_ctx_set_chrom_filter(bk_ctx *c, const uint8_t *accept, uint32_t n)
{
    if (!c || (n && !accept)) return BK_ERR_PARAMS;
    HIP_TRY(hipSetDevice(c->device));
    HIP_TRY(hipStreamSynchronize(c->stream));
    c->buf.chrom_accept.reset();
    c->n_chrom_accept = 0;
    if (!n) return BK_OK;
    HIP_TRY(c->buf.chrom_accept.ensure(n));
    HIP_TRY(hipMemcpy(c->buf.chrom_accept.get(), accept, n, hipMemcpyHostToDevice));
    c->n_chrom_accept = n;
    return BK_OK;
}

int bk_ctx_set_params(bk_ctx *c, const bk_align_params *p)
{
    if (!c || !p) return BK_ERR_PARAMS;
    bk_align_params old = c->params;
    c->params = *p;
    if (c->params.max_ml == 0) c->params.max_ml = 1;
    int rc = derive_cfg(c);
    if (rc) { c->params = old; derive_cfg(c); return rc; }
    (void)hipSetDevice(c->device);
    return BK_OK;
}

int64_t bk_ctx_tune(bk_ctx *c, const char *name, int64_t value)
{
    if (!c || !name) return BK_ERR_PARAMS;
    (void)hipSetDevice(c->device);
    std::string n(name);
    if (n == "heavy_thresh") {
        int64_t old = c->cfg.heavy_thresh;
        if (value < 0 || value > 100) return BK_ERR_PARAMS;
        c->cfg.heavy_thresh = (int)value;
        return old;
    }
    if (n == "chunk_reads") {
        int64_t old = c->chunk_reads;
        if (value < 1 || value > (1LL << 30)) return BK_ERR_PARAMS;
        c->chunk_reads = (uint32_t)value;
        return old;
    }
    if (n == "kmer_bits" || n == "use_ktab") {
        int64_t old = n == "use_ktab" ? c->use_ktab : c->ix.k;
        if (n == "use_ktab") c->use_ktab = value ? 1 : 0;
        else { if (value < 2 || value > 16) return BK_ERR_PARAMS; c->k_req = (int)value; }
        int rc = build_tables(c);
        return rc ? rc : old;
    }
    if (n == "ktab_wide") {
        int64_t old = c->ktab_wide;
        c->ktab_wide = value < 0 ? 0 : (value > 2 ? 2 : (int)value);
        int rc = build_tables(c);
        return rc ? rc : old;
    }
    if (n == "ktab_packed") return c->ix.ktab_hi != nullptr;
    if (n == "use_k3") {
        int64_t old = c->use_k3;
        c->use_k3 = value < 0 ? 0 : (value > kMoreKeys ? kMoreKeys : (int)value);
        int rc = build_tables(c);
        return rc ? rc : old;
    }
    if (n == "k3_resident") return (c->ix.kx[0] != nullptr) + (c->ix.kx[1] != nullptr);
    if (n == "ktab2_resident") return c->ix.ktab2 != nullptr;
    if (n == "ktab2_elem") return c->ix.ktab2 != nullptr && c->ix.ktab2_elem;
    if (n == "grow_after_reads") { int64_t old = (int64_t)c->grow_after; if (value > 0) c->grow_after = (uint64_t)value; return old; }
    if (n == "grow_state") return c->grow_enabled ? c->grow_state.load() : 5;
    if (n == "image_wait") {
        if (c->grow_enabled) {
            grow_tick(c, 0, true);
            if (c->grow_state.load() != 4 && c->grow_state.load() != 0) grow_take_in(c);
        }
        return (c->ix.kx[0] != nullptr) + (c->ix.kx[1] != nullptr) + (c->ix.ktab2 != nullptr ? 4 : 0);
    }
    if (n == "use_ktab2") {
        int64_t old = c->use_ktab2;
        c->use_ktab2 = value < 0 ? 0 : (value > 2 ? 2 : (int)value);
        c->grow_elem = c->use_ktab2 == 2;
        int rc = build_tables(c);
        return rc ? rc : old;
    }
    if (n == "sort_lists") {
        int64_t old = c->sort_lists;
        c->sort_lists = (int)value & 7;
        c->sort_lists_set = true;
        return old;
    }
    if (n == "use_tgt2") {
        int64_t old = c->use_tgt2;
        c->use_tgt2 = value < 0 ? 0 : (value > 2 ? 2 : (int)value);
        int rc = build_tgt2(c);
        return rc ? rc : old;
    }
    if (n == "wave_waves") {
        int64_t old = c->wave_waves;
        if (value < 64 || value > 65536) return BK_ERR_PARAMS;
        c->wave_waves = (uint32_t)value;
        return old;
    }
    if (n == "async_phases") {
        int64_t old = c->async_phases;
        c->async_phases = value ? 1 : 0;
        return old;
    }
    if (n == "swin_resident") return c->image.swin.get() != nullptr ? 1 : 0;
    if (n == "use_swin") {
        int64_t old = c->use_swin;
        c->use_swin = value < 0 ? 0 : (value > 3 ? 3 : (int)value);
        c->swin_denied = false;
        if (c->image.swin.get() && (!c->use_swin || (c->use_swin == 3) != (c->image.swmap.get() == nullptr))) {
            if (c->stream) (void)hipStreamSynchronize(c->stream);
            drop_swin(c);
        }
        return old;
    }
    if (n == "swin_skip_short") {
        int64_t old = c->swin_skip_short;
        c->swin_skip_short = value < 0 ? 0 : (int)std::min<int64_t>(value, kSwLevels - 1);
        return old;
    }
    if (n == "swin_budget_kb") {
        int64_t old = (int64_t)(c->swin_budget >> 10);
        c->swin_budget = value > 0 ? (uint64_t)value << 10 : 0;
        return old;
    }
    if (n == "swin_mbytes") return (int64_t)(c->swin_bytes >> 20);
    if (n == "swin_setup_us") return (int64_t)(c->swin_setup_s * 1e6);
    if (n == "swin_covered_ppm") return c->image.swin.get() ? (int64_t)(c->swin_covered * 1e6) : 0;
    if (n == "swin_core_lens") return c->image.swmap.get() ? c->swin_w : 0;
    if (n == "use_isa") {
        int64_t old = c->use_isa;
        c->use_isa = value ? 1 : 0;
        int rc = build_tables(c);
        return rc ? rc : old;
    }
    if (n == "use_k2") {
        int64_t old = c->use_k2;
        c->use_k2 = value ? 1 : 0;
        int rc = build_tables(c);
        return rc ? rc : old;
    }
    if (n == "use_iv32") {
        int64_t old = c->use_iv32;
        c->use_iv32 = value ? 1 : 0;
        return old;
    }
    if (n == "lazy_search") {
        int64_t old = c->lazy_search;
        c->lazy_search = value ? 1 : 0;
// ... 51 lines not shown
```

Measured before the change: 708.8 million.

## Precompute per-length read plan table and replace per-thread divisions with reciprocals

```diff
diff --git a/biokanga_amd/csrc/bk_ctx_int.h b/biokanga_amd/csrc/bk_ctx_int.h
--- a/biokanga_amd/csrc/bk_ctx_int.h
+++ b/biokanga_amd/csrc/bk_ctx_int.h
@@ -41,6 +41,7 @@
     DevBuf<uint8_t> chrom_accept;
     DevBuf<unsigned long long> htab;
     DevBuf<uint32_t> slot_epoch;
+    DevBuf<uint2> plan;
 };
 struct ImageBufs {
     DevBuf<uint64_t> tgt4, tgt2, tgt2s;
@@ -131,6 +132,11 @@
     bool force_rccl = false;
     uint64_t rccl_allreduces = 0;
     int rccl_ranks = 0;
+    uint2 *h_plan = nullptr;
+    size_t h_plan_cap = 0;
+    uint32_t plan_maxlen = 0;
+    int plan_key[4] = {-1, -1, -1, -1};
+    hipEvent_t ev_plan = nullptr;
     bk::HeavyScratch hs{};
     int max_read_len = 500;
     uint32_t last_maxlen = 0;
diff --git a/biokanga_amd/csrc/bk_device.h b/biokanga_amd/csrc/bk_device.h
--- a/biokanga_amd/csrc/bk_device.h
+++ b/biokanga_amd/csrc/bk_device.h
@@ -105,6 +105,9 @@
     uint32_t n_reads;
     uint32_t nw;
     uint32_t iv_cores;
+    const uint2 *plan;
+    uint32_t plan_stride;
+    uint32_t plan_n;
 };
 
 struct PhaseCtl {
diff --git a/biokanga_amd/csrc/bk_engine.cpp b/biokanga_amd/csrc/bk_engine.cpp
--- a/biokanga_amd/csrc/bk_engine.cpp
+++ b/biokanga_amd/csrc/bk_engine.cpp
@@ -1,4 +1,5 @@
 #include "bk_engine_int.h"
+#include "bk_plan_table.h"
 
 namespace bk {
 int size_heavy_scratch(bk_ctx *c)
@@ -75,6 +76,41 @@
     return BK_OK;
 }
 
+bool plan_table_covers(const bk_ctx *c, uint32_t maxlen)
+{
+    const int key[4] = {c->cfg.max_subs, c->cfg.mm_delta, c->cfg.min_core_len, c->cfg.slides_per100};
+    return c->buf.plan.get() != nullptr && maxlen <= c->plan_maxlen && std::equal(key, key + 4, c->plan_key);
+}
+
+int plan_table_for(bk_ctx *c, uint32_t maxlen, hipStream_t s)
+{
+    const int key[4] = {c->cfg.max_subs, c->cfg.mm_delta, c->cfg.min_core_len, c->cfg.slides_per100};
+    if (plan_table_covers(c, maxlen)) return BK_OK;
+    if (c->cfg.mm_delta < 1 || maxlen > (uint32_t)kMaxReadLenAbs) return BK_ERR_PARAMS;
+    const uint32_t cover = std::max(maxlen, std::equal(key, key + 4, c->plan_key) ? c->plan_maxlen : 0u);
+    const int rows = plan_table_rows(c->cfg, (int)cover);
+    if (rows > kMaxPhases + 1) return BK_ERR_INTERNAL;
+    const size_t n = (size_t)rows * (cover + 1);
+    if (!c->ev_plan) HIP_TRY(hipEventCreateWithFlags(&c->ev_plan, hipEventDisableTiming));
+    else HIP_TRY(hipEventSynchronize(c->ev_plan));
+    c->plan_maxlen = 0;
+    if (n > c->h_plan_cap) {
+        if (c->h_plan) { (void)hipHostFree(c->h_plan); c->h_plan = nullptr; c->h_plan_cap = 0; }
+        HIP_TRY(hipHostMalloc(&c->h_plan, n * sizeof(uint2)));
+        c->h_plan_cap = n;
+    }
+    if (n > c->buf.plan.cap()) {
+        HIP_TRY(hipStreamSynchronize(s));
+        HIP_TRY(c->buf.plan.ensure(n));
+    }
+    if (!plan_table_fill(c->cfg, (int)cover, rows, c->h_plan)) return BK_ERR_INTERNAL;
+    HIP_TRY(hipMemcpyAsync(c->buf.plan.get(), c->h_plan, n * sizeof(uint2), hipMemcpyHostToDevice, s));
+    HIP_TRY(hipEventRecord(c->ev_plan, s));
+    std::copy(key, key + 4, c->plan_key);
+    c->plan_maxlen = cover;
+    return BK_OK;
+}
+
 int ensure_in_reads(bk_ctx *c, uint32_t n, bool packed)
 {
     BatchBufs &m = c->buf;
@@ -331,13 +367,15 @@
     auto P = [&](int ph) { return reinterpret_cast<uint32_t *>(ctl + ph); };
     int max_phases = 0, cmax_bound[kMaxPhases + 1] = {0};
     bool cores_fit = true;
+    { int rp = plan_table_for(c, maxlen, s); if (rp) return rp; }
+    b.plan = c->buf.plan.get();
+    b.plan_stride = c->plan_maxlen + 1;
+    b.plan_n = maxlen + 1;
     for (uint32_t len = 1; len <= maxlen; len++) {
-        const ReadPlan p = make_plan((int)len, c->cfg);
-        max_phases = std::max(max_phases, p.n_phases);
-        for (int ph = 0; ph < p.n_phases && ph <= kMaxPhases; ph++) {
-            int mm, cl, cd, dummy[1];
-            phase_params(p, c->cfg, ph, mm, cl, cd);
-            const int nc = core_offsets((int)len, cl, cd, p.max_slides, dummy, 0);
+        const int n_phases = plan_unpack(c->h_plan[len]).n_phases;
+        max_phases = std::max(max_phases, n_phases);
+        for (int ph = 0; ph < n_phases && ph <= kMaxPhases; ph++) {
+            const int nc = plan_unpack(c->h_plan[(size_t)ph * b.plan_stride + len]).nc;
             if (nc > kMaxCoresFast) cores_fit = false;
             cmax_bound[ph] = std::max(cmax_bound[ph], std::min(nc, (int)kMaxCoresFast));
         }
@@ -585,7 +623,8 @@
         const bool plain = c->cfg.max_hits == 1 && !c->params.best_matches && !c->params.micro_indel_len && !c->params.splice_junct_len && !c->params.min_chimeric_len;
         const bool fits = ml >= 1 && ml <= 16u * (uint32_t)kNwLongest && nreads <= c->cap_reads && nreads <= c->chunk_reads && words_per_read(ml) <= c->cap_wpr &&
                           iv_cores_for(c, ml) <= c->cap_iv_cores && rd2w_for(ml) <= c->cap_rd2w &&
-                          (uint64_t)nreads * iv_cores_for(c, ml) * (c->cfg.align_strand == 0 ? 2u : 1u) <= c->buf.slist.cap() && (c->ix.isa != nullptr || c->hs.htab != nullptr);
+                          (uint64_t)nreads * iv_cores_for(c, ml) * (c->cfg.align_strand == 0 ? 2u : 1u) <= c->buf.slist.cap() && (c->ix.isa != nullptr || c->hs.htab != nullptr) &&
+                          plan_table_covers(c, ml);
         const bool main_path = c->use_wave && c->cfg.heavy_thresh <= 100 && c->ix.k2 != nullptr && c->ix.tgt2 != nullptr && !c->debug && c->async_phases;
         if (!plain || !fits || !main_path) return BK_ERR_PARAMS;
     }
diff --git a/biokanga_amd/csrc/bk_engine_int.h b/biokanga_amd/csrc/bk_engine_int.h
--- a/biokanga_amd/csrc/bk_engine_int.h
+++ b/biokanga_amd/csrc/bk_engine_int.h
@@ -163,6 +163,8 @@
 int ensure_batch_scratch(bk_ctx *c, uint32_t n_reads, uint32_t wpr, uint32_t rd2w = 0, uint32_t iv_cores = kMaxCoresFast);
 int ensure_sort_scratch(bk_ctx *c, uint32_t n, hipStream_t s);
 int ensure_slist(bk_ctx *c, uint64_t lanes, hipStream_t s);
+int plan_table_for(bk_ctx *c, uint32_t maxlen, hipStream_t s);
+bool plan_table_covers(const bk_ctx *c, uint32_t maxlen);
 inline int ensure_seg2(bk_ctx *c, uint32_t n) { HIP_TRY(c->buf.seg2.ensure(n)); return BK_OK; }
 struct HostExtent {
     uint64_t lo = ~0ULL, hi = 0;
diff --git a/biokanga_amd/csrc/bk_extend.hip b/biokanga_amd/csrc/bk_extend.hip
--- a/biokanga_amd/csrc/bk_extend.hip
+++ b/biokanga_amd/csrc/bk_extend.hip
@@ -1,5 +1,6 @@
 #include "bk_dev_window.h"
 #include "bk_dev_prof.h"
+#include "bk_plan_table.h"
 
 namespace bk {
 
@@ -109,6 +110,7 @@
 
 __host__ __device__ constexpr bool flat_rows_in_lds(bool wide, int nw, int bs) { return false; }
 __host__ __device__ constexpr bool flat_small_pass(bool wide, int nw, int bs) { return !wide && nw <= 8 && bs <= 256; }
+__host__ __device__ constexpr bool flat_plan_in_lds(int nw) { return nw <= 16; }
 
 template <bool WIDE, int NW, int BS>
 __global__ void __launch_bounds__(BS) k_flat(DevIndex ix, DevAlignCfg cfg, DevBatch b, const uint32_t *__restrict__ act,
@@ -144,6 +146,9 @@
     __shared__ uint32_t s_wsum[BS / 64];
     __shared__ uint32_t s_cnt[4], s_base[4], s_cmax;
     __shared__ unsigned long long s_ctr[3];
+    constexpr bool PLAN_LDS = flat_plan_in_lds(NW);
+    uint2 *s_plan = reinterpret_cast<uint2 *>(reinterpret_cast<uint8_t *>(s_dyn) + (size_t)BS * slots_max * (cf ? 6 : 2));
+    const uint2 *plan0 = PLAN_LDS ? s_plan : b.plan + (size_t)phase * b.plan_stride, *plan1 = PLAN_LDS ? s_plan + b.plan_n : plan0 + b.plan_stride;
     using EntT = typename FlatEntT<WIDE>::type;
     __shared__ EntT s_es[kLdsEntries], s_ee[kLdsEntries];
     const uint32_t t = threadIdx.x;
@@ -159,6 +164,13 @@
     if (ent_lds && t < ix.n_ent) { es_v = ix.ent_start[t]; ee_v = ix.ent_end[t]; }
 
     const uint32_t a = blockIdx.x * blockDim.x + t;
+    uint32_t r_first = 0;
+    if (a < n_act) r_first = act[a];
+    if (PLAN_LDS) {
+        plan_stage(s_plan, b, phase, t, BS);
+        plan_stage(s_plan + b.plan_n, b, phase + 1, t, BS);
+        __syncthreads();
+    }
     const int s0 = cfg.align_strand == 2 ? 1 : 0, s1 = cfg.align_strand == 1 ? 0 : 1;
     const int cmaxs = slots_max / (s1 - s0 + 1);
     const bool two_bit = b.rd2 != nullptr;
@@ -168,7 +180,7 @@
     int len = 0, mm = 0, cl = 1, cd = 1, nc = 0, n_phases = 0;
     bool mine = false;
     if (a < n_act) {
-        r = act[a];
+        r = r_first;
         const uint32_t len_v = b.rmeta[r];
         const bool spec = !WIDE && slots_max <= SPEC;
         uint2 sv[SPEC];
@@ -188,11 +200,9 @@
             rb00 = rp[0]; rb01 = rp[1]; rb10 = rp[2]; rb11 = rp[3];
         }
         len = (int)(len_v & kReadLenMask);
-        ReadPlan p = make_plan(len, cfg);
-        n_phases = p.n_phases;
-        int dummy[1];
-        phase_params(p, cfg, phase, mm, cl, cd);
-        nc = core_offsets(len, cl, cd, p.max_slides, dummy, 0);
+        const PlanGeo g = plan_lookup(plan0, b.plan_n, len);
+        n_phases = g.n_phases;
+        mm = g.mm; cl = g.cl; cd = g.cd; nc = g.nc;
         const bool fits = nc <= kMaxCoresFast && len <= 16 * NW && nc <= cmaxs;
         bool is_heavy = !fits;
         if (fits) {
@@ -516,10 +526,7 @@
     if (mine) {
         rslt = classify(low_inst, low_mm, nxt, init, cfg.mm_delta, cfg.max_hits);
         if (rslt == BK_HR_NONE && phase + 1 < n_phases) {
-            ReadPlan p = make_plan(len, cfg);
-            int mm2, cl2, cd2, dummy[1];
-            phase_params(p, cfg, phase + 1, mm2, cl2, cd2);
-            int nc2 = core_offsets(len, cl2, cd2, p.max_slides, dummy, 0);
+            const int nc2 = plan_lookup(plan1, b.plan_n, len).nc;
             if (nc2 <= kMaxCoresFast) my_cmax = (uint32_t)nc2;
             dest = 1;
         }
@@ -608,6 +615,7 @@
     unsigned blocks = (n_act_bound + (unsigned)bs - 1) / (unsigned)bs;
     if (slots_max < 1) slots_max = 1;
     size_t lds = (size_t)bs * slots_max * (flat_caches_first(wide, bs, slots_max) ? 6 : 2);
+    if (flat_plan_in_lds(nw)) lds += 2 * (size_t)b.plan_n * sizeof(uint2);
     StripeSet out;
     out.cnt = stripe_cnt;
     for (int i = 0; i < 3; i++) out.stage[i] = stage[i];
diff --git a/biokanga_amd/csrc/bk_image.cpp b/biokanga_amd/csrc/bk_image.cpp
--- a/biokanga_amd/csrc/bk_image.cpp
+++ b/biokanga_amd/csrc/bk_image.cpp
@@ -1018,6 +1018,8 @@
     if (c->h_small) (void)hipHostFree(c->h_small);
     for (void *&t : c->sam_text) if (t) { (void)hipHostFree(t); t = nullptr; }
     if (c->h_ctl) (void)hipHostFree(c->h_ctl);
+    if (c->h_plan) (void)hipHostFree(c->h_plan);
+    if (c->ev_plan) (void)hipEventDestroy(c->ev_plan);
     if (c->ev_ctl) (void)hipEventDestroy(c->ev_ctl);
     if (c->ev_wait) (void)hipEventDestroy(c->ev_wait);
     for (hipEvent_t e : c->ev_pool) (void)hipEventDestroy(e);
diff --git a/biokanga_amd/csrc/bk_plan_table.h b/biokanga_amd/csrc/bk_plan_table.h
--- /dev/null
+++ b/biokanga_amd/csrc/bk_plan_table.h
@@ -0,0 +1,133 @@
+#pragma once
+#include "bk_device.h"
+
+namespace bk {
+
+struct PlanGeo {
+    int cl, cd, nc;
+    int mm, n_phases, max_slides;
+};
+
+__host__ __device__ inline PlanGeo plan_geo_direct(int len, int phase, const DevAlignCfg &c)
+{
+    const ReadPlan p = make_plan(len, c);
+    PlanGeo g;
+    int dummy[1];
+    phase_params(p, c, phase, g.mm, g.cl, g.cd);
+    g.nc = core_offsets(len, g.cl, g.cd, p.max_slides, dummy, 0);
+    g.n_phases = p.n_phases;
+    g.max_slides = p.max_slides;
+    return g;
+}
+
+constexpr int kPlanLenBits = 11, kPlanNcBits = 10, kPlanMmBits = 6, kPlanPhBits = 7;
+static_assert(kMaxReadLenAbs < (1 << kPlanLenBits), "core length and step must fit their fields");
+__host__ __device__ inline uint2 plan_pack(const PlanGeo &g)
+{
+    uint2 e;
+    e.x = (uint32_t)g.cl | (uint32_t)g.cd << kPlanLenBits | (uint32_t)g.nc << (2 * kPlanLenBits);
+    e.y = (uint32_t)g.mm | (uint32_t)g.n_phases << kPlanMmBits | (uint32_t)g.max_slides << (kPlanMmBits + kPlanPhBits);
+    return e;
+}
+__host__ __device__ inline PlanGeo plan_unpack(uint2 e)
+{
+    PlanGeo g;
+    g.cl = (int)(e.x & ((1u << kPlanLenBits) - 1));
+    g.cd = (int)(e.x >> kPlanLenBits & ((1u << kPlanLenBits) - 1));
+    g.nc = (int)(e.x >> (2 * kPlanLenBits));
+    g.mm = (int)(e.y & ((1u << kPlanMmBits) - 1));
+    g.n_phases = (int)(e.y >> kPlanMmBits & ((1u << kPlanPhBits) - 1));
+    g.max_slides = (int)(e.y >> (kPlanMmBits + kPlanPhBits));
+    return g;
+}
+__host__ __device__ inline bool plan_fits(const PlanGeo &g)
+{
+    return g.cl >= 0 && g.cl < (1 << kPlanLenBits) && g.cd >= 0 && g.cd < (1 << kPlanLenBits) && g.nc >= 0 && g.nc < (1 << kPlanNcBits) &&
+           g.mm >= 0 && g.mm < (1 << kPlanMmBits) && g.n_phases >= 0 && g.n_phases < (1 << kPlanPhBits) && g.max_slides >= 0 &&
+           g.max_slides < (1 << (32 - kPlanMmBits - kPlanPhBits));
+}
+
+inline int plan_table_rows(const DevAlignCfg &c, int maxlen)
+{
+    int rows = 0;
+    for (int len = 1; len <= maxlen; len++) {
+        const int n = make_plan(len, c).n_phases;
+        rows = n > rows ? n : rows;
+    }
+    return rows + 1;
+}
+inline bool plan_table_fill(const DevAlignCfg &c, int maxlen, int rows, uint2 *out)
+{
+    const size_t stride = (size_t)maxlen + 1;
+    for (int ph = 0; ph < rows; ph++)
+        for (int len = 0; len <= maxlen; len++) {
+            const PlanGeo g = plan_geo_direct(len, ph, c);
+            if (!plan_fits(g)) return false;
+            out[ph * stride + len] = plan_pack(g);
+        }
+    return true;
+}
+
+__device__ __forceinline__ PlanGeo plan_lookup(const uint2 *row, uint32_t n, int len)
+{
+    const uint32_t i = (uint32_t)len < n ? (uint32_t)len : n - 1;
+    return plan_unpack(row[i]);
+}
+__device__ __forceinline__ void plan_stage(uint2 *dst, const DevBatch &b, int phase, uint32_t t, uint32_t threads)
+{
+    const uint2 *__restrict__ row = b.plan + (size_t)phase * b.plan_stride;
+    for (uint32_t i = t; i < b.plan_n; i += threads) dst[i] = row[i];
+}
+
+struct SmallDiv { uint32_t d, m; };
+constexpr uint32_t kSmallDivMaxD = 32, kSmallDivMaxX = 2048;
+__host__ __device__ inline SmallDiv small_div_make(uint32_t d) { return SmallDiv{d, 65536u / d + 1}; }
+__host__ __device__ inline uint32_t small_div(uint32_t x, SmallDiv v) { return (x * v.m) >> 16; }
+
+struct Div32 { uint64_t m; uint32_t d; };
+__host__ __device__ inline Div32 div32_make(uint32_t d) { return Div32{d > 1 ? ~0ULL / d + 1 : 0ULL, d}; }
+__host__ __device__ inline uint32_t div32(uint32_t n, Div32 v)
+{
+    const uint64_t hi = v.m >> 32, lo = v.m & 0xFFFFFFFFu;
+    const uint32_t q = (uint32_t)((hi * n + ((lo * n) >> 32)) >> 32);
+    return v.d == 1 ? n : q;
+}
+
+struct ItemCursor { uint64_t a0; uint32_t rem0; };
+struct ItemGeo { SmallDiv per_read, cmax; uint32_t step_q, step_r; };
+constexpr uint32_t kItemMaxLaneOfs = kSmallDivMaxX - kSmallDivMaxD;
+inline ItemGeo item_geo_make(uint32_t per_read, uint32_t cmax, uint64_t step)
+{
+    return ItemGeo{small_div_make(per_read), small_div_make(cmax), (uint32_t)(step / per_read), (uint32_t)(step % per_read)};
+}
+__host__ __device__ inline ItemCursor item_cursor(uint64_t item, uint32_t per_read)
+{
+    return ItemCursor{item / per_read, (uint32_t)(item % per_read)};
+}
+__host__ __device__ inline void item_advance(ItemCursor &t, const ItemGeo &g)
+{
+    t.a0 += g.step_q;
+    t.rem0 += g.step_r;
+    if (t.rem0 >= g.per_read.d) { t.rem0 -= g.per_read.d; t.a0++; }
+}
+__host__ __device__ inline void item_decode(const ItemCursor &t, uint32_t lane_ofs, const ItemGeo &g, uint64_t &a, int &si, int &c)
+{
+    const uint32_t x = t.rem0 + lane_ofs, q = small_div(x, g.per_read), rem = x - q * g.per_read.d;
+    const uint32_t s = small_div(rem, g.cmax);
+    a = t.a0 + q;
+    si = (int)s;
+    c = (int)(rem - s * g.cmax.d);
+}
+
+struct SlotGeo { Div32 stride; SmallDiv cores; };
+inline SlotGeo slot_geo_make(uint32_t iv_stride, uint32_t iv_cores) { return SlotGeo{div32_make(iv_stride), small_div_make(iv_cores)}; }
+__host__ __device__ inline void slot_decode(uint32_t slot, const SlotGeo &g, uint32_t &a, int &strand, int &c)
+{
+    const uint32_t sc = div32(slot, g.stride);
+    a = slot - sc * g.stride.d;
+    const uint32_t s = small_div(sc, g.cores);
+    strand = (int)s;
+    c = (int)(sc - s * g.cores.d);
+}
+
+}
diff --git a/biokanga_amd/csrc/bk_prep.hip b/biokanga_amd/csrc/bk_prep.hip
--- a/biokanga_amd/csrc/bk_prep.hip
+++ b/biokanga_amd/csrc/bk_prep.hip
@@ -1,4 +1,5 @@
 #include "bk_dev_util.h"
+#include "bk_plan_table.h"
 
 namespace bk {
 
@@ -291,6 +292,8 @@
     __shared__ uint32_t s_cnt, s_base, s_cmax;
     constexpr bool TR = NW == 8 && BK_PREP_TRANSPOSE;
     __shared__ uint4 s_tr[TR ? 4 : 1][TR ? 64 * (NW / 2) : 1];
+    extern __shared__ uint2 s_plan[];
+    plan_stage(s_plan, b, 0, threadIdx.x, 256);
     if (threadIdx.x == 0) { s_cnt = 0; s_cmax = 0; }
     __syncthreads();
     const uint32_t r = blockIdx.x * blockDim.x + threadIdx.x;
@@ -384,12 +387,9 @@
         if (bad || num_ns > max_ns_seq) h.nar = BK_NAR_NS;
         has_n = bad || num_ns > 0;
         if (h.nar != BK_NAR_NS) {
-            ReadPlan p = make_plan(len, cfg);
-            if (p.n_phases > 0) {
-                int mm, cl, cd, ofs[1];
-                phase_params(p, cfg, 0, mm, cl, cd);
-                int nc = core_offsets(len, cl, cd, p.max_slides, ofs, 0);
-                if (nc <= kMaxCoresFast) my_cmax = (uint32_t)nc;
+            const PlanGeo g = plan_lookup(s_plan, b.plan_n, len);
+            if (g.n_phases > 0) {
+                if (g.nc <= kMaxCoresFast) my_cmax = (uint32_t)g.nc;
                 go = true;
             }
         }
@@ -605,19 +605,20 @@
         out.cnt = stripe_cnt;
         out.stage[0] = out.stage[1] = out.stage[2] = stage;
         out.cap = stripe_cap(blocks, 256);
+        const size_t plan_lds = (size_t)b.plan_n * sizeof(uint2);
         if (packed) {
             launch_fill_u64(reinterpret_cast<unsigned long long *>(b.rmeta), ((uint64_t)b.n_reads + 1) / 2, 0ULL, s);
             if (eblocks) hipLaunchKernelGGL(k_mark_exc, dim3(eblocks), dim3(256), 0, s, b);
-            if (b.nw == 8) hipLaunchKernelGGL((k_prep_fused<8, true>), dim3(blocks), dim3(256), 0, s, cfg, b, out);
-            else if (b.nw == 16) hipLaunchKernelGGL((k_prep_fused<16, true>), dim3(blocks), dim3(256), 0, s, cfg, b, out);
-            else if (b.nw == kNwLong) hipLaunchKernelGGL((k_prep_fused<kNwLong, true>), dim3(blocks), dim3(256), 0, s, cfg, b, out);
-            else hipLaunchKernelGGL((k_prep_fused<kNwLongest, true>), dim3(blocks), dim3(256), 0, s, cfg, b, out);
+            if (b.nw == 8) hipLaunchKernelGGL((k_prep_fused<8, true>), dim3(blocks), dim3(256), plan_lds, s, cfg, b, out);
+            else if (b.nw == 16) hipLaunchKernelGGL((k_prep_fused<16, true>), dim3(blocks), dim3(256), plan_lds, s, cfg, b, out);
+            else if (b.nw == kNwLong) hipLaunchKernelGGL((k_prep_fused<kNwLong, true>), dim3(blocks), dim3(256), plan_lds, s, cfg, b, out);
+            else hipLaunchKernelGGL((k_prep_fused<kNwLongest, true>), dim3(blocks), dim3(256), plan_lds, s, cfg, b, out);
             if (eblocks && b.rd2 != nullptr) hipLaunchKernelGGL(k_exc_rows, dim3(eblocks), dim3(256), 0, s, b);
             if (eblocks) hipLaunchKernelGGL(k_apply_exc, dim3(eblocks), dim3(256), 0, s, b);
-        } else if (b.nw == 8) hipLaunchKernelGGL((k_prep_fused<8, false>), dim3(blocks), dim3(256), 0, s, cfg, b, out);
-        else if (b.nw == 16) hipLaunchKernelGGL((k_prep_fused<16, false>), dim3(blocks), dim3(256), 0, s, cfg, b, out);
-        else if (b.nw == kNwLong) hipLaunchKernelGGL((k_prep_fused<kNwLong, false>), dim3(blocks), dim3(256), 0, s, cfg, b, out);
-        else hipLaunchKernelGGL((k_prep_fused<kNwLongest, false>), dim3(blocks), dim3(256), 0, s, cfg, b, out);
+        } else if (b.nw == 8) hipLaunchKernelGGL((k_prep_fused<8, false>), dim3(blocks), dim3(256), plan_lds, s, cfg, b, out);
+        else if (b.nw == 16) hipLaunchKernelGGL((k_prep_fused<16, false>), dim3(blocks), dim3(256), plan_lds, s, cfg, b, out);
+        else if (b.nw == kNwLong) hipLaunchKernelGGL((k_prep_fused<kNwLong, false>), dim3(blocks), dim3(256), plan_lds, s, cfg, b, out);
+        else hipLaunchKernelGGL((k_prep_fused<kNwLongest, false>), dim3(blocks), dim3(256), plan_lds, s, cfg, b, out);
         launch_compact(out, &act, &act_cnt, 1, cmax, s);
         return;
     }
diff --git a/biokanga_amd/csrc/bk_search.hip b/biokanga_amd/csrc/bk_search.hip
--- a/biokanga_amd/csrc/bk_search.hip
+++ b/biokanga_amd/csrc/bk_search.hip
@@ -2,6 +2,7 @@
 
 #include "bk_dev_k2.h"
 #include "bk_dev_prof.h"
+#include "bk_plan_table.h"
 
 namespace bk {
 
@@ -52,9 +53,11 @@
 template <int ILP>
 __global__ void __launch_bounds__(256) k_search_a_ilp(DevIndex ix, DevAlignCfg cfg, DevBatch b, const uint32_t *__restrict__ act,
                                                       const uint32_t *__restrict__ p_n_act, int phase, int cmax, int nstr, int lazy,
-                                                      StripeSet out)
+                                                      StripeSet out, ItemGeo ig)
 {
     __shared__ uint32_t s_cnt, s_base;
+    extern __shared__ uint2 s_plan[];
+    plan_stage(s_plan, b, phase, threadIdx.x, 256);
 #if defined(BK_PROF) && BK_PROF == 2
     PROF_BEGIN;
 #endif
@@ -63,7 +66,8 @@
     const uint64_t total = (uint64_t)n_act * per_read;
     constexpr uint64_t stride = 256;
     const int k = ix.k;
-  for (uint64_t tile0 = (uint64_t)blockIdx.x * (256 * ILP); tile0 < total; tile0 += (uint64_t)gridDim.x * (256 * ILP)) {
+    ItemCursor cur = item_cursor((uint64_t)blockIdx.x * (256 * ILP), per_read);
+  for (uint64_t tile0 = (uint64_t)blockIdx.x * (256 * ILP); tile0 < total; tile0 += (uint64_t)gridDim.x * (256 * ILP), item_advance(cur, ig)) {
     if (threadIdx.x == 0) s_cnt = 0;
     __syncthreads();
     bool on[ILP], push[ILP], have_code[ILP];
@@ -77,22 +81,20 @@
     uint32_t key0[ILP];
 #pragma unroll
     for (int u = 0; u < ILP; u++) {
-        const uint64_t tid = tile0 + threadIdx.x + (uint64_t)u * stride;
         on[u] = false; push[u] = false; have_code[u] = false; slot[u] = 0; p0[u] = 0; q2raw[u] = 0; first[u] = 0; nval[u] = 0; cl[u] = 1; lo[u] = hi[u] = 0;
         cix[u] = kNoIv32; cv[u] = make_uint2(0, kNoIv32); cached[u] = false;
-        if (tid < total) {
-            const uint64_t a = tid / per_read;
-            const uint32_t rem = (uint32_t)(tid - a * per_read);
-            const int si = (int)(rem / (uint32_t)cmax), c = (int)(rem % (uint32_t)cmax);
+        uint64_t a;
+        int si, c;
+        item_decode(cur, threadIdx.x + (uint32_t)u * (uint32_t)stride, ig, a, si, c);
+        if (a < n_act) {
             const uint32_t r = act[a];
             const uint32_t meta = b.rmeta[r];
             const int len = (int)(meta & kReadLenMask);
             const int strand_c = cfg.align_strand == 2 ? 1 : si;
             if (b.iv32 != nullptr && c == 0 && phase > 0) cv[u] = b.iv32[(uint32_t)strand_c * b.n_reads + r];
-            ReadPlan p = make_plan(len, cfg);
-            int mm, cd, dummy[1];
-            phase_params(p, cfg, phase, mm, cl[u], cd);
-            const int nc = core_offsets(len, cl[u], cd, p.max_slides, dummy, 0);
+            const PlanGeo g = plan_lookup(s_plan, b.plan_n, len);
+            const int cd = g.cd, nc = g.nc;
+            cl[u] = g.cl;
             if (c < nc && nc <= kMaxCoresFast) {
                 on[u] = true;
                 if (b.iv32 != nullptr && c == 0 && cl[u] >= k + kK2Bases) {
@@ -238,9 +240,11 @@
 template <bool WIDE>
 __global__ void __launch_bounds__(256) k_search_b(DevIndex ix, DevAlignCfg cfg, DevBatch b, int phase, int lazy,
                                                   const uint32_t *__restrict__ list, const uint32_t *__restrict__ sorted, uint32_t n_sorted,
-                                                  const uint32_t *__restrict__ p_n_list)
+                                                  const uint32_t *__restrict__ p_n_list, SlotGeo sg)
 {
     __shared__ uint64_t s_lv[kK2Levels + 1];
+    extern __shared__ uint2 s_plan[];
+    plan_stage(s_plan, b, phase, threadIdx.x, 256);
     if (threadIdx.x <= (unsigned)kK2Levels) s_lv[threadIdx.x] = threadIdx.x ? k2s_start(ix.n, (int)threadIdx.x) : 0;
     __syncthreads();
     const uint32_t n_list = *p_n_list;
@@ -250,14 +254,16 @@
     unsigned long long d_k2 = 0, d_deep = 0, d_sa = 0;
     struct Fin { unsigned long long &a, &b, &c; DevBatch &bb; __device__ ~Fin() { if (a + b) atomicAdd(&bb.ctr[ctr_stripe() + 5], a + b); if (c) atomicAdd(&bb.ctr[ctr_stripe() + 6], c); } } fin{d_k2, d_deep, d_sa, b};
 #endif
-    const uint64_t slot = i < n_grouped ? sorted[i] : list[i];
-    const uint32_t r = b.act[(uint32_t)(slot % b.iv_stride)], sc = (uint32_t)(slot / b.iv_stride);
-    const int strand = (int)(sc / b.iv_cores), c = (int)(sc % b.iv_cores);
+    const uint32_t slot32 = i < n_grouped ? sorted[i] : list[i];
+    const uint64_t slot = slot32;
+    uint32_t a;
+    int strand, c;
+    slot_decode(slot32, sg, a, strand, c);
+    const uint32_t r = b.act[a];
     const uint32_t meta = b.rmeta[r];
     const int len = (int)(meta & kReadLenMask);
-    ReadPlan p = make_plan(len, cfg);
-    int mm, cl, cd;
-    phase_params(p, cfg, phase, mm, cl, cd);
+    const PlanGeo g = plan_lookup(s_plan, b.plan_n, len);
+    const int cl = g.cl, cd = g.cd;
     const int my_ofs = c * cd < len - cl ? c * cd : len - cl;
     const RdRow rdw = read_row(b, r, strand, (meta & kReadHasN) != 0);
     uint64_t first;
@@ -402,7 +408,10 @@
     out.cnt = stripe_cnt;
     out.stage[0] = out.stage[1] = out.stage[2] = stage;
     out.cap = stripe_cap((unsigned)tiles, (unsigned)per);
-    hipLaunchKernelGGL(k_search_a_ilp<2>, dim3(blocks), dim3(256), 0, s, ix, cfg, b, act, p_n_act, phase, cmax, nstr, lazy, out);
+    static_assert(256 * ilp <= (int)kItemMaxLaneOfs, "a lane's offset within a tile must stay in item_decode's range");
+    const ItemGeo ig = item_geo_make((uint32_t)(cmax * nstr), (uint32_t)cmax, (uint64_t)blocks * per);
+    const size_t lds = (size_t)b.plan_n * sizeof(uint2);
+    hipLaunchKernelGGL(k_search_a_ilp<ilp>, dim3(blocks), dim3(256), lds, s, ix, cfg, b, act, p_n_act, phase, cmax, nstr, lazy, out, ig);
     launch_compact(out, &list, &list_cnt, 1, nullptr, s);
 }
 
@@ -411,8 +420,10 @@
 {
     if (!n_bound) return;
     unsigned blocks = (unsigned)std::min<uint64_t>((n_bound + 255) / 256, 32768);
-    if (ix.sa_hi) hipLaunchKernelGGL(k_search_b<true>, dim3(blocks), dim3(256), 0, s, ix, cfg, b, phase, lazy, list, sorted, n_sorted, p_n_list);
-    else hipLaunchKernelGGL(k_search_b<false>, dim3(blocks), dim3(256), 0, s, ix, cfg, b, phase, lazy, list, sorted, n_sorted, p_n_list);
+    const SlotGeo sg = slot_geo_make(b.iv_stride, b.iv_cores);
+    const size_t lds = (size_t)b.plan_n * sizeof(uint2);
+    if (ix.sa_hi) hipLaunchKernelGGL(k_search_b<true>, dim3(blocks), dim3(256), lds, s, ix, cfg, b, phase, lazy, list, sorted, n_sorted, p_n_list, sg);
+    else hipLaunchKernelGGL(k_search_b<false>, dim3(blocks), dim3(256), lds, s, ix, cfg, b, phase, lazy, list, sorted, n_sorted, p_n_list, sg);
 }
 
 __global__ void __launch_bounds__(256) k_clear_iv(DevBatch b, const uint32_t *__restrict__ p_n_act, int cmax, int st0, int st1, uint32_t word)
diff --git a/biokanga_amd/csrc/bk_tune.cpp b/biokanga_amd/csrc/bk_tune.cpp
--- a/biokanga_amd/csrc/bk_tune.cpp
+++ b/biokanga_amd/csrc/bk_tune.cpp
@@ -22,6 +22,9 @@
     }
     if (c->sort_lists) { rc = ensure_sort_scratch(c, n, c->stream); if (rc) return rc; }
     if (c->use_wave && c->ix.isa == nullptr) { rc = size_heavy_scratch(c); if (rc) return rc; }
+    rc = plan_table_for(c, max_read_len, c->stream);
+    if (rc) return rc;
+    HIP_TRY(hipStreamSynchronize(c->stream));
     return BK_OK;
 }
 
```

New measurement: 718.8 million, median of 6. +1.4%, better.
